# zichunhao/lgn-autoencoder

Hardware: AMD Instinct MI355X
Metric: jets/sec fwd+bwd, 30-particle maxdim=2 bs=512 (higher is better)
Workload: dtype f64

## Files before the change

include/lgn_amd.h:

```cpp
#ifndef LGN_AMD_H
#define LGN_AMD_H

#include <stddef.h>
#include <stdint.h>

#ifdef __cplusplus
extern "C" {
#endif

#define LGN_AMD_ABI_VERSION 18

int lgn_abi_version(void);
const char* lgn_last_error(void);

int lgn_level_fwd_f64(int B, int N, int C, int CO, int decoder,
                      const double* s_in, const double* v_in, const double* p, const uint8_t* mask,
                      const double* ra, const double* rb, const double* rc,
                      const double* w0, const double* b0, const double* w1, const double* b1,
                      const double* wm0, const double* wm1,
                      double* ag0, double* ag1, double* s_out, double* v_out, void* stream);

int lgn_level_bwd_partial_rows(int B, int N, int decoder, int* rows_mix, int* rows_rad);
int lgn_level_rad_partial_len(int C, int decoder);
int lgn_level_jet_split(int B, int N);

int lgn_level_bwd_f64(int B, int N, int C, int CO, int decoder,
                      const double* s_in, const double* v_in, const double* p, const uint8_t* mask,
                      const double* ra, const double* rb, const double* rc,
                      const double* w0, const double* b0, const double* w1, const double* b1,
                      const double* wm0, const double* wm1, const double* ag0, const double* ag1,
                      const double* g_s_out, const double* g_v_out,
                      double* g_ag, double* g_s_in, double* g_v_in, double* g_p,
                      double* part_mix, double* part_rad, void* stream);

int lgn_cg_product_fwd_f64(int R, int N, int C, int D1, int D2, int DO, int mode, int nnz, const int* row_ptr, const int* col,
                           const double* coef, const double* x1, const double* x2, double* out, void* stream);
int lgn_cg_product_bwd_f64(int R, int N, int C, int D1, int D2, int DO, int mode, int nnz, const int* row_ptr, const int* col,
                           const double* coef, const double* x1, const double* x2, const double* g_out, double* g_x1, double* g_x2,
                           void* stream);

int lgn_reduce_partials_f64(const double* part, int rows, int n, double* out, int accumulate, void* stream);

int lgn_radial_finalize_f64(const double* tot, int C, const double* ra, const double* rb, const double* rc,
                            const double* w0, const double* w1,
                            double* g_a, double* g_b, double* g_c,
                            double* g_w0, double* g_b0, double* g_w1, double* g_b1, void* stream);

#define LGN_ACT_LEAKYRELU 0
#define LGN_ACT_RELU 1
#define LGN_ACT_ELU 2
#define LGN_ACT_SIGMOID 3
#define LGN_ACT_LOGSIGMOID 4
#define LGN_ACT_ATAN 5
#define LGN_ACT_COUNT 6
int lgn_cgmlp_fwd_f64(int M, int C, int H, int nlin, int activation, const double* const* w, const double* const* b,
                      const double* s_in, double* s_out, void* stream);
int lgn_cgmlp_partial_rows(int M, int H);
int lgn_cgmlp_bwd_f64(int M, int C, int H, int nlin, int activation, const double* const* w, const double* const* b,
                      const double* s_in, const double* g_out, double* g_in, double* part, int psize, void* stream);

int lgn_mixreps_fwd_f64(int rows, int Cin, int Cout, int d, const double* w, const double* x, double* y, void* stream);
int lgn_mixreps_partial_rows(int rows);
int lgn_mixreps_bwd_f64(int rows, int Cin, int Cout, int d, const double* w, const double* x, const double* g_y,
                        double* g_x, double* part, void* stream);

int lgn_moments_fwd_f64(int B, int N, int C, int Q, int decoder, const double* X, const double* p, const uint8_t* mask,
                        const double* ra, const double* rb, const double* rc, const double* w0, const double* b0,
                        const double* w1, const double* b1, double* U, void* stream);
long long lgn_moments_scratch_doubles(int B, int N, int C, int decoder);
int lgn_moments_bwd_f64(int B, int N, int C, int Q, int decoder, const double* X, const double* p, const uint8_t* mask,
                        const double* ra, const double* rb, const double* rc, const double* w0, const double* b0,
                        const double* w1, const double* b1, const double* gU, double* gX, double* g_p,
                        double* part_rad, double* scratch, void* stream);

typedef struct lgn_local_tables {
  int n_rows, n_out, n_w;
  int n_terms, n_u, n_x;
  int n_units, static_kind;
  const int *row_ptr, *t_type, *t_a, *t_b;
  const double* t_coef;
  const int *out_dim, *out_nblk, *out_row0, *out_q0, *out_w0;
  const int *u_ptr, *u_row;
  const double* u_coef;
  const int *x_ptr, *x_row, *x_other;
  const double* x_coef;
  int h_out_w0[8];
} lgn_local_tables;

int lgn_local_fwd_f64(int nodes, int C, int CO, int Q, int Qout, const lgn_local_tables* t, const double* X, const double* U,
                      const double* wcat, double* out, void* stream);
int lgn_local_partial_rows(int nodes);
int lgn_local_bwd_f64(int nodes, int C, int CO, int Q, int Qout, const lgn_local_tables* t, const double* X, const double* U,
                      const double* wcat, const double* g_out, double* gU, double* gX, double* part, void* stream);

long long lgn_local_static_packed_doubles(int kind, int C, int CO);
int lgn_local_bwd_static_f64(int kind, int nodes, int C, int CO, const double* XT, const double* UT, const double* wcat,
                             const int* w0, double* wpacked, const double* goT, double* gUT, double* gXT, double* part,
                             double* gpacked, double* g_wcat, void* stream);
int lgn_local_fwd_static_f64(int kind, int nodes, int C, int CO, const double* XT, const double* UT, const double* wcat,
                             const int* w0, double* wpacked, double* outT, double* s_copy, int q_s, void* stream);

typedef struct lgn_net_desc {
  int B, N;
  int n_levels;
  int enc_channels[5];
  int dec_channels[5];
  int tau_s, tau_v;
  int mlp_hidden_mul;
  int mlp_nlin;
  int tau_v_in;
  const lgn_local_tables* enc_tables[4];
  const lgn_local_tables* dec_tables[4];
  int enc_Q[5], enc_qs[5], enc_qv[5];
  int dec_Q[5], dec_qs[5], dec_qv[5];
  int flags;
  int activation;
  int n_in_scalars;
  int latent_pool;
  int dec_N;
  int get_real;
  double jet_loss_scale;
} lgn_net_desc;
#define LGN_REAL_SUM 0
#define LGN_REAL_REAL 1
#define LGN_REAL_IMAG 2
#define LGN_REAL_MEAN 3
#define LGN_REAL_NORM 4
#define LGN_POOL_MIN 0
#define LGN_POOL_MAX 1
#define LGN_POOL_MEAN 2
#define LGN_POOL_MIX 3
#define LGN_POOL(n, avg, o0, o1, o2, o3) ((n) | ((avg) << 3) | ((o0) << 4) | ((o1) << 6) | ((o2) << 8) | ((o3) << 10))
#define LGN_NET_NO_STATIC 1
#define LGN_NET_DEC_PAIRWISE 2
#define LGN_NET_LEVEL_V2 4
#define LGN_NET_MLP_V1 8
#define LGN_NET_MOMENTS_V1 16
#define LGN_NET_BWD_ORDERED 64
#define LGN_NET_DEC_UNFUSED 256
#define LGN_NET_MOMENTS_SPLIT 512
#define LGN_NET_MLP_BWD1 1024
#define LGN_NET_SPLIT_TAIL 128

#define LGN_LDS_LIMIT (160 * 1024)
long long lgn_encoder_end_lds_bytes(int N, int C0, int K, int CL, int Ts, int Tv, int pool);
long long lgn_decoder_end_lds_bytes(int N, int C0, int Tin, int CL);
long long lgn_junction_lds_bytes(int N, int CL, int Ts, int Tv, int pool, int C0);

int lgn_step_param_slots(const lgn_net_desc* d, int decoder);
long long lgn_step_workspace_doubles(const lgn_net_desc* d);
int lgn_step_fwd_bwd_f64(const lgn_net_desc* d, const double* params, double* grads, long long n_params,
                         const int64_t* enc_off, const int64_t* dec_off, const double* p4, const double* target,
                         const uint8_t* mask, const double* in_scalars, double* workspace, long long workspace_doubles,
                         double* recon, double* loss_part, void* stream);
#define LGN_FINALIZE_SCRATCH 2048
int lgn_step_finalize_f64(double* params, double* grads, long long n_params, const double* loss_part, int n_loss,
                          double l1_lambda, double* adam_m, double* adam_v, long long* step_dev,
                          double lr, double beta1, double beta2, double eps, int do_adam, double* loss_out, void* stream);
int lgn_step_train_f64(const lgn_net_desc* d, double* params, double* grads, long long n_params, const int64_t* enc_off,
                       const int64_t* dec_off, const double* p4, const double* target, const uint8_t* mask, const double* in_scalars,
                       double* workspace, long long workspace_doubles, double* recon, double* loss_part, int n_loss, double l1_lambda,
                       double* adam_m, double* adam_v, long long* step_dev, double lr, double beta1, double beta2, double eps,
                       int do_adam, double* loss_out, void* stream);

long long lgn_eval_workspace_doubles(const lgn_net_desc* d);
int lgn_step_eval_f64(const lgn_net_desc* d, const double* params, const int64_t* enc_off, const int64_t* dec_off,
                      const double* p4_scaled, const double* p4_target, const uint8_t* mask, const double* in_scalars,
                      double* workspace, long long workspace_doubles, double* recon_real, double* lat_s ,
                      double* lat_v , double* loss_part, double* loss_out, void* stream);

long long lgn_net_workspace_doubles(const lgn_net_desc* d, int decoder, int which);
int lgn_encoder_fwd_f64(const lgn_net_desc* d, const double* params, const int64_t* off, const double* p4, const uint8_t* mask,
                        const double* in_scalars, double* act, long long act_doubles, double* lat_s, double* lat_v, void* stream);
int lgn_encoder_bwd_f64(const lgn_net_desc* d, const double* params, double* grads, long long n_params, const int64_t* off,
                        const double* p4, const uint8_t* mask, const double* in_scalars, const double* act, long long act_doubles,
                        const double* g_lat_s, const double* g_lat_v, double* scratch, long long scratch_doubles, void* stream);
int lgn_decoder_fwd_f64(const lgn_net_desc* d, const double* params, const int64_t* off, const double* lat_v, double* act,
                        long long act_doubles, double* recon, void* stream);
int lgn_decoder_bwd_f64(const lgn_net_desc* d, const double* params, double* grads, long long n_params, const int64_t* off,
                        const double* lat_v, const double* act, long long act_doubles, const double* g_recon, double* g_lat_v,
                        double* scratch, long long scratch_doubles, void* stream);

int lgn_chamfer_f64(int B, int N, int M, const double* x, const double* y, int jet_features, double* loss_part, double* gx, double* gy,
                    void* stream);

#define LGN_ANOMALY_NMAX 192
#define LGN_ANOMALY_NSCORES 21
#define LGN_ANOMALY_ALL 0x1FFFFF
#define LGN_ANOMALY_HUNGARIAN 0x403E0
#define LGN_ANOMALY_NO_HUNGARIAN (LGN_ANOMALY_ALL & ~LGN_ANOMALY_HUNGARIAN)
int lgn_anomaly_scores_f64(const double* recons, const double* target, const double* recons_n, const double* target_n, int B, int N,
                           int score_mask, double* scores, int* col4row , int* status, void* stream);

int lgn_linear_sum_assignment_f64(const double* cost, int B, int n, int* col4row, int* status, void* stream);

#ifdef __cplusplus
}
#endif
#endif
```

lgn-autoencoder_amd/csrc/api_common.cpp:

```cpp
#include <stdarg.h>
#include <stdlib.h>

#include "level.hpp"
#include "../../include/lgn_amd.h"

namespace lgn {
static thread_local char g_err[512] = "";
void set_error(const char* fmt, ...) {
  va_list ap;
  va_start(ap, fmt);
  vsnprintf(g_err, sizeof(g_err), fmt, ap);
  va_end(ap);
}
int level_flags_from_env() {
  auto on = [](const char* name) { const char* e = getenv(name); return e && e[0] == '1'; };
  return (on("LGN_AMD_DEC_PAIRWISE") ? LVL_DEC_PAIRWISE : 0) | (on("LGN_AMD_LEVEL_V2") ? LVL_LEVEL_V2 : 0) |
         (on("LGN_AMD_MOMENTS_V1") ? LVL_MOMENTS_V1 : 0) | (on("LGN_AMD_MLP_V1") ? LVL_MLP_V1 : 0) | (on("LGN_AMD_BWD_ORDERED") ? LVL_BWD_ORDERED : 0) |
         (on("LGN_AMD_MOMENTS_SPLIT") ? LVL_MOMENTS_SPLIT : 0) | (on("LGN_AMD_MLP_BWD1") ? LVL_MLP_BWD1 : 0);
}
static_assert(LVL_DEC_PAIRWISE == LGN_NET_DEC_PAIRWISE && LVL_LEVEL_V2 == LGN_NET_LEVEL_V2 && LVL_MOMENTS_V1 == LGN_NET_MOMENTS_V1 &&
                  LVL_MLP_V1 == LGN_NET_MLP_V1 && LVL_MLP_BWD1 == LGN_NET_MLP_BWD1 &&
                  LVL_BWD_ORDERED == LGN_NET_BWD_ORDERED && LVL_MOMENTS_SPLIT == LGN_NET_MOMENTS_SPLIT, "LVL_* and LGN_NET_* are the same bits");
}

extern "C" {
const char* lgn_last_error(void) { return lgn::g_err; }
int lgn_abi_version(void) { return LGN_AMD_ABI_VERSION; }
}
```

lgn-autoencoder_amd/csrc/level.hpp:

```cpp
#pragma once
#include "common.hpp"

namespace lgn {

constexpr int LVL_DEC_PAIRWISE = 2;
constexpr int LVL_LEVEL_V2 = 4;
constexpr int LVL_MLP_V1 = 8;
constexpr int LVL_MOMENTS_V1 = 16;
constexpr int LVL_MLP_BWD1 = 1024;
constexpr int LVL_MOMENTS_SPLIT = 512;
constexpr int LVL_BWD_ORDERED = 64;
int level_flags_from_env();

template <typename T>
struct LevelArgs {
  int B, N, C, CO;
  const T* s_in;
  const T* v_in;
  const T* p;
  const uint8_t* mask;
  const T *ra, *rb, *rc, *w0, *b0, *w1, *b1;
  const T *wm0, *wm1;
  T* ag0;
  T* ag1;
  T* s_out;
  T* v_out;
  const T* in_w0 = nullptr;
  const T* in_w1 = nullptr;
  T* in_s = nullptr;
  T* in_v = nullptr;
  T* z1 = nullptr;
  size_t z1n = 0;
  T* z2 = nullptr;
  size_t z2n = 0;
  const T* loss_wo1 = nullptr;
  const T* loss_target = nullptr;
  T loss_scale = T(1);
  int loss_real = 0;
  T loss_jscale = T(0);
  T* loss_recon = nullptr;
  T* loss_part = nullptr;
  T* loss_gv = nullptr;
  T* loss_wpart = nullptr;
  int flags = 0;
};

template <typename T>
struct LevelBwdArgs {
  int B, N, C, CO;
  const T *s_in, *v_in, *p;
  const uint8_t* mask;
  const T *ra, *rb, *rc, *w0, *b0, *w1, *b1;
  const T *wm0, *wm1;
  const T *ag0, *ag1;
  const T* g_s_out;
  const T* g_v_out;
  T* g_ag;
  T* g_s_in;
  T* g_v_in;
  T* g_p;
  T* part_mix;
  T* part_rad;
  T* part_in0 = nullptr;
  int flags = 0;
};

__host__ __device__ constexpr int node_stride(int C) { return 10 * C + 4; }

__host__ __device__ constexpr int rad_partial_size(int C, bool dec) {
  return dec ? 2 * C : (2 * 4 * C * NB + 8 * C);
}

inline int level_jet_split(int B, int N) {
  const int groups = (N + 3) / 4;
  int s = 1;
  while (s * 2 <= groups && B * s * 2 <= 512) s *= 2;
  return s;
}

}
```

lgn-autoencoder_amd/csrc/level_fwd2.hip:

```cpp
#include "level_dev.hpp"
#include "net_dev.hpp"
#include "ops.hpp"
#include "wave_sum.hpp"

namespace lgn {

typedef double v4d __attribute__((ext_vector_type(4)));
LGN_STAMP_DECL
LGN_STAMP_READER(lgn_debug_stamps_fwd2)

__device__ __forceinline__ double dpp_quad(double v, int ctrl_is_xor2) {
  int lo = __double2loint(v), hi = __double2hiint(v);
  if (ctrl_is_xor2) {
    lo = __builtin_amdgcn_mov_dpp(lo, 0x4E, 0xF, 0xF, true);
    hi = __builtin_amdgcn_mov_dpp(hi, 0x4E, 0xF, 0xF, true);
  } else {
    lo = __builtin_amdgcn_mov_dpp(lo, 0xB1, 0xF, 0xF, true);
    hi = __builtin_amdgcn_mov_dpp(hi, 0xB1, 0xF, 0xF, true);
  }
  return __hiloint2double(hi, lo);
}
__device__ __forceinline__ double quad_sum(double v) {
  v += dpp_quad(v, 0);
  v += dpp_quad(v, 1);
  return v;
}

__device__ __forceinline__ double fast_rcp(double u) {
  double r = __builtin_amdgcn_rcp(u);
  double e = __builtin_fma(-u, r, 1.0);
  r = __builtin_fma(r, e, r);
  e = __builtin_fma(-u, r, 1.0);
  return __builtin_fma(r, e, r);
}

template <int C, bool DEC>
struct Fwd2 {
  static constexpr int NG = (C + 3) / 4;
  static constexpr int NS = node_stride(C);
  static constexpr int PS = DEC ? 8 : 4;
  static constexpr int AGS = 20 * C;
  static constexpr int A3 = 0, A4 = 2 * C, A1 = 4 * C, A2 = 12 * C;
};

template <int C, bool DEC, bool SEP, bool TRAIN>
__global__ __launch_bounds__(2 * BLOCK) void level_fwd2_kernel(LevelArgs<double> a, int chunk) {
  using F = Fwd2<C, DEC>;
  constexpr int NG = F::NG;
  const int N = a.N, B = a.B, CO = a.CO;
  const int b = blockIdx.x, tid = threadIdx.x, lane = tid & 63, wave = tid >> 6;
  const int nthr = blockDim.x, nw = nthr >> 6;

  extern __shared__ __align__(16) unsigned char smem_raw[];
  double* nd = reinterpret_cast<double*>(smem_raw);
  double* pj = nd + ((N * F::NS + 1) & ~1);
  double* wm = pj + N * F::PS;
  double* agl = wm + 4 * CO * 5 * C;
  double* sums = agl + chunk * F::AGS;
  uint8_t* mk = reinterpret_cast<uint8_t*>(sums + 20 * C);

  STAMP(0);
  if (!DEC && a.in_w0) {
    {
      const size_t wg = (size_t)blockIdx.y * gridDim.x + blockIdx.x, stride = (size_t)gridDim.x * gridDim.y * nthr;
      for (size_t e = wg * nthr + tid; e < a.z1n; e += stride) a.z1[e] = 0.0;
      for (size_t e = wg * nthr + tid; e < a.z2n; e += stride) a.z2[e] = 0.0;
    }
    const double* p0 = a.p + (size_t)b * N * 4;
    const size_t plane_s = (size_t)B * N * C;
    const int nw2 = 2 * CO * 5 * C;
    for (int e = tid; e < N * 4; e += nthr) pj[e] = p0[e];
    for (int e = tid; e < N; e += nthr) mk[e] = a.mask[(size_t)b * N + e];
    for (int e = tid; e < nw2; e += nthr) {
      wm[e] = a.wm0[e];
      wm[nw2 + e] = a.wm1[e];
    }
    for (int e = tid; e < N * C; e += nthr) {
      const int j = e / C, c = e - j * C;
      const double* p = p0 + j * 4;
      const double pe = p[0], px = p[1], py = p[2], pz = p[3];
      const double q0 = pe * pe, q1 = px * px, q2 = py * py, q3 = pz * pz;
      const double mass = sqrt(fabs(2.0 * q0 - (((q0 + q1) + q2) + q3)));
      constexpr double H = 0.70710678118654752440084436210484903928;
      const cx<double> q[4] = {{pe, 0.0}, {px * H, -py * H}, {pz, 0.0}, {-px * H, -py * H}};
      const double w0r = a.in_w0[c], w0i = a.in_w0[C + c];
      const cx<double> w1 = {a.in_w1[c], a.in_w1[C + c]};
      double* d = nd + j * F::NS + c * 10;
      d[0] = w0r * mass;
      d[1] = w0i * mass;
#pragma unroll
      for (int m = 0; m < 4; ++m) {
        const cx<double> r = cmul(w1, q[m]);
        d[2 + m] = r.r;
        d[6 + m] = r.i;
      }
      if (blockIdx.y == 0) {
        const size_t ge = (size_t)b * N * C + e;
        a.in_s[ge] = d[0];
        a.in_s[plane_s + ge] = d[1];
#pragma unroll
        for (int m = 0; m < 4; ++m) {
          a.in_v[ge * 4 + m] = d[2 + m];
          a.in_v[plane_s * 4 + ge * 4 + m] = d[6 + m];
        }
      }
    }
  } else {
    JetRegs<double> jr;
    load_jet_issue<double, C, DEC>(a.s_in, a.v_in, a.p, a.mask, B, N, b, jr);
    const int nw2 = 2 * CO * 5 * C, ew = tid < nw2 ? tid : 0;
    const double w0v = a.wm0[ew], w1v = a.wm1[ew];
    load_jet_commit<double, C, DEC>(a.s_in, a.v_in, a.p, a.mask, B, N, b, jr, nd, pj, mk);
    if (tid < nw2) {
      wm[tid] = w0v;
      wm[nw2 + tid] = w1v;
    }
    for (int e = tid + nthr; e < nw2; e += nthr) {
      wm[e] = a.wm0[e];
      wm[nw2 + e] = a.wm1[e];
    }
  }

  const int pr = lane & 15, cg = lane >> 4;
  const int ti = pr >> 2, tj = pr & 3;
  double ak[5], bk[5], ck2[5];
  double wf[NG][5];
  double bias[NG][4];
  if (!DEC) {
#pragma unroll
    for (int s = 0; s < 5; ++s) {
      const int k = 4 * s + cg;
      ak[s] = a.ra[k];
      bk[s] = a.rb[k];
      const double c = a.rc[k];
      ck2[s] = c * c;
    }
#pragma unroll
    for (int g = 0; g < NG; ++g) {
      const int rr = lane & 15, q = rr >> 2, ch = 4 * g + (rr & 3);
      const double* w = (q >> 1) ? a.w1 : a.w0;
#pragma unroll
      for (int s = 0; s < 5; ++s) wf[g][s] = ch < C ? w[(2 * ch + (q & 1)) * NB + 4 * s + cg] : 0.0;
    }
  }
#pragma unroll
  for (int g = 0; g < NG; ++g) {
    const int ch = 4 * g + cg;
#pragma unroll
    for (int q = 0; q < 4; ++q) {
      const double* bb = (q >> 1) ? a.b1 : a.b0;
      bias[g][q] = ch < C ? (DEC ? bb[ch] : bb[2 * ch + (q & 1)]) : 0.0;
    }
  }
  __syncthreads();
  STAMP(1);

  if constexpr (DEC && SEP) {
    if (tid < 64) {
      const int k = tid & 7, part = tid >> 3;
      double mean = 0.0;
      for (int n = part; n < N; n += 8) mean += pj[n * 8 + k];
      mean += shfl_xor(mean, 8);
      mean += shfl_xor(mean, 16);
      mean += shfl_xor(mean, 32);
      if (part == 0) sums[k] = mean / N;
    }
    __syncthreads();
    for (int e = tid; e < N * 8; e += nthr) pj[e] -= sums[e & 7];
    __syncthreads();
#define LGN_PUT(k, val)                                           \
  do {                                                            \
    if ((k) < 12) a0[(k) < 12 ? (k) : 0] += (val);                \
    else a1[(k) >= 12 ? (k) - 12 : 0] += (val);                   \
  } while (0)
    for (int c = wave; c < C; c += nw) {
      double a0[12], a1[8];
#pragma unroll
      for (int k = 0; k < 12; ++k) a0[k] = 0.0;
#pragma unroll
      for (int k = 0; k < 8; ++k) a1[k] = 0.0;
      for (int n = lane; n < N; n += 64) {
        const double* ni = nd + n * F::NS + c * 10;
        const double* pn = pj + n * 8;
        const cx<double> sn = {ni[0], ni[1]};
        cx<double> v[4], pc[4];
#pragma unroll
        for (int m = 0; m < 4; ++m) {
          v[m] = {ni[2 + m], ni[6 + m]};
          pc[m] = {pn[m], pn[4 + m]};
        }
        LGN_PUT(0, sn.r);  LGN_PUT(1, sn.i);
#pragma unroll
        for (int m = 0; m < 4; ++m) {
          LGN_PUT(2 + 2 * m, v[m].r);  LGN_PUT(3 + 2 * m, v[m].i);
          const cx<double> sp = cmul(sn, pc[m]);
          LGN_PUT(10 + 2 * m, sp.r);  LGN_PUT(11 + 2 * m, sp.i);
        }
        const cx<double> vp = bil2(v, pc);
        LGN_PUT(18, vp.r);  LGN_PUT(19, vp.i);
      }
      wave_sum_store<12>(a0, sums + c * 20, lane);
      wave_sum_store<8>(a1, sums + c * 20 + 12, lane);
    }
#undef LGN_PUT
    __syncthreads();
  }

  const int ngroups = (N + 3) >> 2, gper = (ngroups + (int)gridDim.y - 1) / (int)gridDim.y;
  const int rlo = min(N, 4 * (int)blockIdx.y * gper), rhi = min(N, rlo + 4 * gper);
  auto catmix = [&](int c0, int c1) {
    constexpr int K = 5 * C;
    const int nr = c1 - c0;
    const size_t plo = (size_t)B * N * CO;
    if (wave == 0) {
      for (int rl = lane; rl < nr; rl += 64) {
// ... 147 lines not shown
#pragma unroll
          for (int s = 0; s < 5; ++s) beta[s] = __builtin_fma(bk[s], rho5[s], ak[s]);
        }
#pragma unroll
        for (int g = 0; g < NG; ++g) {
          T.R[g] = v4d{bias[g][0], bias[g][1], bias[g][2], bias[g][3]};
#pragma unroll
          for (int s = 0; s < 5; ++s) T.R[g] = __builtin_amdgcn_mfma_f64_16x16x4f64(wf[g][s], beta[s], T.R[g], 0, 0, 0);
        }
      }
    };
    auto agg = [&](const Tile& T) {
      if (T.ok) {
        const double* nj = nd + T.jj * F::NS;
#pragma unroll
        for (int g = 0; g < NG; ++g) {
          const int ch = 4 * g + cg;
          if (ch < C) {
            const cx<double> R0 = {T.R[g][0], T.R[g][1]}, R1 = {T.R[g][2], T.R[g][3]};
            const cx<double> e0 = {R0.r - R0.i, R0.r + R0.i};
            const cx<double> sj = {nj[ch * 10], nj[ch * 10 + 1]};
            cx<double> vj[4];
#pragma unroll
            for (int m = 0; m < 4; ++m) {
              vj[m] = {nj[ch * 10 + 2 + m], nj[ch * 10 + 6 + m]};
              cfma(A1[g][m], vj[m], e0);
            }
            cfma(A4[g], sj, e0);
            if (!DEC) {
              const double qd0 = T.qd0, qd3 = T.qd3, qa = T.qa, qb = T.qb;
              const cx<double> Tm = cmul(sj, R1);
              A2[g][0].r = __builtin_fma(Tm.r, qd0, A2[g][0].r);  A2[g][0].i = __builtin_fma(Tm.i, qd0, A2[g][0].i);
              A2[g][2].r = __builtin_fma(Tm.r, qd3, A2[g][2].r);  A2[g][2].i = __builtin_fma(Tm.i, qd3, A2[g][2].i);
              const double aTr = qa * Tm.r, aTi = qa * Tm.i, bTr = qb * Tm.r, bTi = qb * Tm.i;
              A2[g][1].r += aTr + bTi;  A2[g][1].i += aTi - bTr;
              A2[g][3].r += bTi - aTr;  A2[g][3].i -= aTi + bTr;
              const cx<double> dv = {vj[3].r - vj[1].r, vj[3].i - vj[1].i}, sv = {vj[1].r + vj[3].r, vj[1].i + vj[3].i};
              cx<double> V;
              V.r = __builtin_fma(vj[0].r, qd0, __builtin_fma(-vj[2].r, qd3, __builtin_fma(qa, dv.r, qb * sv.i)));
              V.i = __builtin_fma(vj[0].i, qd0, __builtin_fma(-vj[2].i, qd3, __builtin_fma(qa, dv.i, -qb * sv.r)));
              cfma(A3[g], R1, V);
            } else {
              cx<double> e1[4];
#pragma unroll
              for (int m = 0; m < 4; ++m) {
                e1[m] = cmul(R1, T.q[m]);
                cfma(A2[g][m], sj, e1[m]);
              }
              const cx<double> t = bil2(vj, e1);
              A3[g].r += t.r;
              A3[g].i += t.i;
            }
          }
        }
      }
    };
    if (jlo < jhi) {
      Tile ta, tb;
      prep(jlo, ta);
      int j0 = jlo;
      while (true) {
        if (j0 + 4 < jhi) prep(j0 + 4, tb);
        agg(ta);
        j0 += 4;
        if (j0 >= jhi) break;
        if (j0 + 4 < jhi) prep(j0 + 4, ta);
        agg(tb);
        j0 += 4;
        if (j0 >= jhi) break;
      }
    }

    STAMP(3 + ((rg >> 2) & 3) * 4);
#pragma unroll
    for (int g = 0; g < NG; ++g) {
      A3[g].r = quad_sum(A3[g].r) * 0.5;  A3[g].i = quad_sum(A3[g].i) * 0.5;
      A4[g].r = quad_sum(A4[g].r);        A4[g].i = quad_sum(A4[g].i);
#pragma unroll
      for (int m = 0; m < 4; ++m) {
        A1[g][m].r = quad_sum(A1[g][m].r);  A1[g][m].i = quad_sum(A1[g][m].i);
        A2[g][m].r = quad_sum(A2[g][m].r);  A2[g][m].i = quad_sum(A2[g][m].i);
      }
    }
    if (tj == 0) {
      double* st = agl + (slab + i0 + ti - c0) * F::AGS;
#pragma unroll
      for (int g = 0; g < NG; ++g) {
        const int ch = 4 * g + cg;
        if (ch < C) {
          st[F::A3 + 2 * ch] = A3[g].r;  st[F::A3 + 2 * ch + 1] = A3[g].i;
          st[F::A4 + 2 * ch] = A4[g].r;  st[F::A4 + 2 * ch + 1] = A4[g].i;
#pragma unroll
          for (int m = 0; m < 4; ++m) {
            st[F::A1 + (ch * 4 + m) * 2] = A1[g][m].r;  st[F::A1 + (ch * 4 + m) * 2 + 1] = A1[g][m].i;
            st[F::A2 + (ch * 4 + m) * 2] = A2[g][m].r;  st[F::A2 + (ch * 4 + m) * 2 + 1] = A2[g][m].i;
          }
        }
      }
    }
    STAMP(4 + ((rg >> 2) & 3) * 4);
  };
  if (rs > 1) {
    const int rg = (c0 >> 2) + wave / rs;
    if (rg * 4 < c1) row_group(rg, 4 * (rpart * ntl / rs), min(N, 4 * ((rpart + 1) * ntl / rs)), rpart * 4 * ngr);
  } else {
    for (int rg = (c0 >> 2) + wave; rg * 4 < c1; rg += nw) row_group(rg, 0, N, 0);
  }
  if (rs > 1) {
    __syncthreads();
    const int tot = 4 * ngr * F::AGS;
    for (int e = tid; e < tot; e += nthr) {
      double v = agl[e];
      for (int pp = 1; pp < rs; ++pp) v += agl[pp * tot + e];
      agl[e] = v;
    }
  }
  }
  __syncthreads();
  STAMP(20);

  if constexpr (TRAIN) {
    const size_t pl0 = (size_t)B * N * 2 * C;
    for (int e = tid; e < (c1 - c0) * 2 * C; e += nthr) {
      const int n = e / (2 * C), r = e - n * 2 * C, blk = r / C, ch = r - blk * C;
      const double* st = agl + n * F::AGS + (blk ? F::A4 : F::A3) + 2 * ch;
      const size_t ge = ((size_t)b * N + c0) * 2 * C + e;
      a.ag0[ge] = st[0];
      a.ag0[pl0 + ge] = st[1];
    }
    for (int e = tid; e < (c1 - c0) * 2 * C * 4; e += nthr) {
      const int n = e / (8 * C), r = e - n * 8 * C, blk = r / (4 * C), cm = r - blk * 4 * C;
      const double* st = agl + n * F::AGS + (blk ? F::A2 : F::A1) + 2 * cm;
      const size_t ge = ((size_t)b * N + c0) * 8 * C + e;
      a.ag1[ge] = st[0];
      a.ag1[pl0 * 4 + ge] = st[1];
    }
  }
  STAMP(21);

  catmix(c0, c1);
  STAMP(22);
  if (c1 < rhi) __syncthreads();
  }
  STAMP(40);
  if constexpr (DEC) {
    if (a.loss_wo1) {
      __syncthreads();
      dec_output_loss_body<TRAIN>(B, N, CO, a.v_out, a.loss_wo1, a.loss_target, a.loss_scale, a.loss_real, a.loss_jscale,
                                  a.loss_recon, a.loss_part, a.loss_gv, a.loss_wpart, smem_raw);
    }
  }
}

template <int C, bool DEC, bool SEP, bool TRAIN>
static int launch_level_fwd2(const LevelArgs<double>& a, hipStream_t stream) {
  using F = Fwd2<C, DEC>;
  const size_t fixed = sizeof(double) * (((size_t)a.N * F::NS + 1 & ~size_t(1)) + (size_t)a.N * F::PS + 4 * a.CO * 5 * C + 20 * C) + a.N + 16;
  const bool wide = a.B <= 320 && a.N >= 64;
  const size_t row = sizeof(double) * F::AGS, budget1 = 160 * 1024, budget2 = wide ? budget1 : 78 * 1024;
  const int full = (a.N + 15) & ~15;
  int chunk = full;
  if (fixed + full * row > budget2) {
    const size_t room = fixed + 16 * row <= budget2 ? budget2 - fixed : (fixed < budget1 ? budget1 - fixed : 0);
    chunk = (int)(room / row) & ~15;
    if (chunk > full) chunk = full;
    if (chunk < 16) chunk = 16;
  }
  size_t smem = fixed + chunk * row;
  if (a.loss_wo1) {
    LGN_CHECK_ARG(DEC && SEP && a.N <= 40 && !wide && a.loss_target && a.loss_recon && a.loss_part && (!TRAIN || (a.loss_gv && a.loss_wpart)),
                  "level_fwd: the loss rides on the separable decoder forward of jets of <= 40 particles only");
    if (smem < dec_out_loss_bytes(a.N, a.CO)) smem = dec_out_loss_bytes(a.N, a.CO);
  }
  LGN_CHECK_ARG(smem <= 160 * 1024, "level_fwd: N=%d C=%d needs %zu B of LDS (> 160 KiB)", a.N, a.C, smem);
  auto kern = level_fwd2_kernel<C, DEC, SEP, TRAIN>;
  if (smem > 64 * 1024) {
    hipError_t e = hipFuncSetAttribute(reinterpret_cast<const void*>(kern), hipFuncAttributeMaxDynamicSharedMemorySize, (int)smem);
    if (e != hipSuccess) { set_error("hipFuncSetAttribute: %s", hipGetErrorString(e)); return (int)e; }
  }
  const int nthreads = wide ? 2 * BLOCK : BLOCK;
  const int split = (SEP || a.N > 40) ? 1 : level_jet_split(a.B, a.N);
  hipLaunchKernelGGL(kern, dim3(a.B, split), dim3(nthreads), smem, stream, a, chunk);
  LGN_CHECK_LAUNCH();
  return 0;
}

bool level_fwd_carries_loss(int N, int flags) { return N <= 40 && !(flags & LVL_DEC_PAIRWISE); }

template <bool TRAIN>
static int level_fwd_run(const LevelArgs<double>& a, int decoder, hipStream_t stream) {
  LGN_CHECK_ARG(a.B > 0 && a.N > 0, "level_fwd: empty batch (B=%d N=%d)", a.B, a.N);
  LGN_CHECK_ARG(!a.in_w0 || (!decoder && a.in_w1 && a.in_s && a.in_v), "level_fwd: the input stage rides on encoder levels only");
  LGN_CHECK_ARG(a.CO >= 1 && a.CO <= 8, "level_fwd: C_out=%d unsupported (1..8)", a.CO);
  const bool pairwise = (a.flags & LVL_DEC_PAIRWISE) != 0;
#define LGN_CASE(CC)                                                                                         \
  case CC:                                                                                                   \
    if (!decoder) return launch_level_fwd2<CC, false, false, TRAIN>(a, stream);                              \
    return pairwise ? launch_level_fwd2<CC, true, false, TRAIN>(a, stream) : launch_level_fwd2<CC, true, true, TRAIN>(a, stream);
  switch (a.C) {
#ifdef LGN_DEV_ONLY_C4
    LGN_CASE(4)
#else
    LGN_CASE(1) LGN_CASE(2) LGN_CASE(3) LGN_CASE(4) LGN_CASE(5) LGN_CASE(6) LGN_CASE(7) LGN_CASE(8)
#endif
    default:
      set_error("level_fwd: C_in=%d unsupported (1..8)", a.C);
      return -1;
  }
#undef LGN_CASE
}

template <>
int level_fwd_dispatch<double>(const LevelArgs<double>& a, int decoder, hipStream_t stream) {
  return level_fwd_run<true>(a, decoder, stream);
}

int level_fwd_eval(const LevelArgs<double>& a, int decoder, hipStream_t stream) { return level_fwd_run<false>(a, decoder, stream); }

}
```

lgn-autoencoder_amd/csrc/net_kernels.hip:

```cpp
#include "net.hpp"
#include "net_dev.hpp"
#include "tail_dev.hpp"

namespace lgn {

LGN_STAMP_DECL
LGN_STAMP_READER(lgn_debug_stamps_net)

namespace {
constexpr double H = 0.70710678118654752440084436210484903928;

__device__ __forceinline__ double minkowski_sq_ref(const double* p) {
  double q0 = p[0] * p[0], q1 = p[1] * p[1], q2 = p[2] * p[2], q3 = p[3] * p[3];
  return 2.0 * q0 - (((q0 + q1) + q2) + q3);
}
__device__ __forceinline__ void canon_real(const double* p, cx<double> (&q)[4]) {
  q[0] = {p[0], 0.0};
  q[1] = {p[1] * H, -p[2] * H};
  q[2] = {p[3], 0.0};
  q[3] = {-p[1] * H, -p[2] * H};
}
__device__ __forceinline__ void canon_cplx(const cx<double> (&p)[4], cx<double> (&c)[4]) {
  c[0] = p[0];
  c[1] = {(p[1].r + p[2].i) * H, (p[1].i - p[2].r) * H};
  c[2] = p[3];
  c[3] = {(-p[1].r + p[2].i) * H, (-p[1].i - p[2].r) * H};
}
__device__ __forceinline__ void canon_cplx_bwd(const cx<double> (&g)[4], cx<double> (&gp)[4]) {
  gp[0] = g[0];
  gp[1] = {(g[1].r - g[3].r) * H, (g[1].i - g[3].i) * H};
  gp[2] = {-(g[1].i + g[3].i) * H, (g[1].r + g[3].r) * H};
  gp[3] = g[2];
}
__device__ __forceinline__ void cart_from_canon(const cx<double> (&c)[4], cx<double> (&p)[4]) {
  p[0] = c[0];
  p[1] = {(c[1].r - c[3].r) * H, (c[1].i - c[3].i) * H};
  p[2] = {-(c[1].i + c[3].i) * H, (c[1].r + c[3].r) * H};
  p[3] = c[2];
}
}

__global__ void enc_input_fwd_kernel(int B, int N, int C, int K, const double* __restrict__ p4, const double* __restrict__ xs,
                                     const double* __restrict__ w0, const double* __restrict__ w1, double* s, double* v, double* z1,
                                     size_t n1, double* z2, size_t n2) {
  const size_t total = (size_t)B * N * C, pl = total;
  for (size_t e = (size_t)blockIdx.x * blockDim.x + threadIdx.x; e < n1; e += (size_t)gridDim.x * blockDim.x) z1[e] = 0.0;
  for (size_t e = (size_t)blockIdx.x * blockDim.x + threadIdx.x; e < n2; e += (size_t)gridDim.x * blockDim.x) z2[e] = 0.0;
  for (size_t e = (size_t)blockIdx.x * blockDim.x + threadIdx.x; e < total; e += (size_t)gridDim.x * blockDim.x) {
    const int c = e % C;
    const size_t node = e / C;
    const double* p = p4 + node * 4;
    const double mass = sqrt(fabs(minkowski_sq_ref(p)));
    cx<double> q[4];
    canon_real(p, q);
    double sr = w0[c * K] * mass, si = w0[(C + c) * K] * mass;
    for (int k = 1; k < K; ++k) {
      const double x = xs[node * (K - 1) + (k - 1)];
      sr = __builtin_fma(w0[c * K + k], x, sr);
      si = __builtin_fma(w0[(C + c) * K + k], x, si);
    }
    s[e] = sr;
    s[pl + e] = si;
    const cx<double> w = {w1[c], w1[C + c]};
#pragma unroll
    for (int m = 0; m < 4; ++m) {
      cx<double> r = cmul(w, q[m]);
      v[e * 4 + m] = r.r;
      v[pl * 4 + e * 4 + m] = r.i;
    }
  }
}

__global__ __launch_bounds__(BLOCK) void enc_input_bwd_kernel(int B, int N, int C, int K, const double* __restrict__ p4,
                                                             const double* __restrict__ xs, const double* __restrict__ g_s,
                                                             const double* __restrict__ g_v, double* part) {
  extern __shared__ __align__(16) unsigned char smem_raw[];
  double* tmp = reinterpret_cast<double*>(smem_raw);
  const int T = 2 * K + 2;
  const int b = blockIdx.x;
  const size_t pl = (size_t)B * N * C;
  for (int i = threadIdx.x; i < N * C; i += BLOCK) {
    const int n = i / C;
    const double* p = p4 + ((size_t)b * N + n) * 4;
    const double mass = sqrt(fabs(minkowski_sq_ref(p)));
    cx<double> q[4];
    canon_real(p, q);
    const size_t e = (size_t)b * N * C + i;
    cx<double> d1 = {0, 0};
#pragma unroll
    for (int m = 0; m < 4; ++m) cfmac(d1, cx<double>{g_v[e * 4 + m], g_v[pl * 4 + e * 4 + m]}, q[m]);
    const double gr = g_s[e], gi = g_s[pl + e];
    tmp[i * T + 0] = gr * mass;
    tmp[i * T + K] = gi * mass;
    for (int k = 1; k < K; ++k) {
      const double x = xs[((size_t)b * N + n) * (K - 1) + (k - 1)];
      tmp[i * T + k] = gr * x;
      tmp[i * T + K + k] = gi * x;
    }
    tmp[i * T + 2 * K] = d1.r;
    tmp[i * T + 2 * K + 1] = d1.i;
  }
  __syncthreads();
  for (int o = threadIdx.x; o < T * C; o += BLOCK) {
    int c, t;
    if (o < 2 * C * K) {
      const int z = o / (C * K), r = o - z * C * K;
      c = r / K;
      t = z * K + (r - c * K);
    } else {
      const int r = o - 2 * C * K, z = r / C;
      c = r - z * C;
      t = 2 * K + z;
    }
    double acc = 0.0;
    for (int n = 0; n < N; ++n) acc += tmp[(n * C + c) * T + t];
    part[(size_t)b * T * C + o] = acc;
  }
}

__device__ __forceinline__ cx<double> canon_cplx_m(const double* p, int m) {
  if (m == 0) return {p[0], p[4]};
  if (m == 2) return {p[3], p[7]};
  const double sg = m == 1 ? 1.0 : -1.0;
  return {(sg * p[1] + p[6]) * H, (sg * p[5] - p[2]) * H};
}
__device__ __forceinline__ cx<double> canon_cplx_bwd_m(const double* g, int m) {
  if (m == 0) return {g[0], g[4]};
  if (m == 3) return {g[2], g[6]};
  if (m == 1) return {(g[1] - g[3]) * H, (g[5] - g[7]) * H};
  return {-(g[5] + g[7]) * H, (g[1] + g[3]) * H};
}

__host__ __device__ inline size_t lat_y_doubles(int N, int Ts, int Tv, int pool = 0) {
  return (size_t)(pool_is_mix(pool) ? 1 : N) * (2 * Ts + 8 * Tv);
}
__host__ __device__ inline size_t lat_fwd_doubles(int N, int C, int Ts, int Tv, int pool = 0) {
  return lat_y_doubles(N, Ts, Tv, pool) + (size_t)N * C * 10 + 2 * (size_t)(Ts + Tv) * pool_mix_in(pool, N, C);
}
struct LatentStage {
  StageRegs<2> sr, si;
  StageRegs<4> vr, vi;
  StageRegs<1> w0, w1;
  const double *s0, *s1, *v0, *v1, *wl0, *wl1;
  int N, C, Ts, Tv, K, NY, NS;
  __device__ __forceinline__ void issue(int B, int N_, int C_, int Ts_, int Tv_, const double* __restrict__ s, const double* __restrict__ v,
                                        const double* __restrict__ wl0_, const double* __restrict__ wl1_, int pool = 0) {
    N = N_; C = C_; Ts = Ts_; Tv = Tv_; wl0 = wl0_; wl1 = wl1_; K = pool_mix_in(pool, N_, C_); NY = (int)lat_y_doubles(N_, Ts_, Tv_, pool);
    const size_t pl = (size_t)B * N * C, j0 = (size_t)blockIdx.x * N * C;
    NS = s ? N * C : 0;
    s0 = s ? s + j0 : nullptr; s1 = s ? s + pl + j0 : nullptr; v0 = v + j0 * 4; v1 = v + (pl + j0) * 4;
    vr.issue(v0, N * C * 4); vi.issue(v1, N * C * 4);
    sr.issue(s0, NS); si.issue(s1, NS);
    w0.issue(wl0, 2 * Ts * K); w1.issue(wl1, 2 * Tv * K);
  }
  __device__ __forceinline__ void commit(double* lds, bool zero_y) const {
    double* sv = lds + NY;
    double* w0l = sv + N * C * 10;
    double* w1l = w0l + 2 * Ts * K;
    if (zero_y)
      for (int e = threadIdx.x; e < NY; e += BLOCK) lds[e] = 0.0;
    vr.commit(v0, N * C * 4, [&](int e, double x) { sv[(e >> 2) * 10 + 2 + (e & 3)] = x; });
    vi.commit(v1, N * C * 4, [&](int e, double x) { sv[(e >> 2) * 10 + 6 + (e & 3)] = x; });
    if (NS) {
      sr.commit(s0, NS, [&](int e, double x) { sv[e * 10] = x; });
      si.commit(s1, NS, [&](int e, double x) { sv[e * 10 + 1] = x; });
    } else {
      for (int e = threadIdx.x; e < N * C; e += BLOCK) sv[e * 10] = sv[e * 10 + 1] = 0.0;
    }
    w0.commit(wl0, 2 * Ts * K, [&](int e, double x) { w0l[e] = x; });
    w1.commit(wl1, 2 * Tv * K, [&](int e, double x) { w1l[e] = x; });
  }
};
template <bool TO_LDS>
__device__ __forceinline__ void enc_latent_fwd_body(int B, int N, int C, int Ts, int Tv, int pool, double* lat_s, double* lat_v, int* idx,
                                                    double* lds, double* lat_l) {
  const int b = blockIdx.x, TT = Ts + Tv;
  const int P = pool_blocks(pool), PN = pool_n(pool);
  bool need_mean = false;
  for (int i = 0; i < PN; ++i) need_mean |= pool_op(pool, i) == LGN_POOL_MEAN;
  const int YS = 2 * Ts + 8 * Tv;
  double* y = lds;
  const double* sv = y + N * YS;
  const double* w0l = sv + N * C * 10;
  const double* w1l = w0l + 2 * Ts * C;
  STAMP(1);
  for (int e = threadIdx.x; e < N * Tv; e += BLOCK) {
    const int n = e / Tv, tv = e - n * Tv;
    const double* x = sv + n * C * 10;
    cx<double> acc[4] = {{0, 0}, {0, 0}, {0, 0}, {0, 0}}, pc[4];
#pragma unroll 4
    for (int c = 0; c < C; ++c) {
      const cx<double> w = {w1l[tv * C + c], w1l[Tv * C + tv * C + c]};
#pragma unroll
      for (int m = 0; m < 4; ++m) cfma(acc[m], w, cx<double>{x[c * 10 + 2 + m], x[c * 10 + 6 + m]});
    }
    cart_from_canon(acc, pc);
    double* o = y + n * YS + 2 * Ts + 8 * tv;
#pragma unroll
    for (int m = 0; m < 4; ++m) { o[m] = pc[m].r; o[4 + m] = pc[m].i; }
  }
  for (int e = threadIdx.x; e < N * Ts; e += BLOCK) {
    const int n = e / Ts, t = e - n * Ts;
    const double* x = sv + n * C * 10;
    cx<double> acc = {0, 0};
#pragma unroll 4
    for (int c = 0; c < C; ++c) cfma(acc, cx<double>{w0l[t * C + c], w0l[Ts * C + t * C + c]}, cx<double>{x[c * 10], x[c * 10 + 1]});
    y[n * YS + 2 * t] = acc.r;
    y[n * YS + 2 * t + 1] = acc.i;
  }
  __syncthreads();
  STAMP(2);
  const int l8 = threadIdx.x & 7;
  constexpr int NONE = 0x7fffffff;
  for (int it = threadIdx.x >> 3; it < 2 * TT; it += BLOCK / 8) {
    const int z = it / TT, t = it - z * TT;
    int imin = NONE, imax = NONE;
    double smin = 0, smax = 0;
#pragma unroll 4
    for (int n = l8; n < N; n += 8) {
      double lo, hi;
      if (t < Ts) {
        const double val = y[n * YS + 2 * t + z];
        lo = val;
        hi = val * val;
      } else {
        const double* o = y + n * YS + 2 * Ts + 8 * (t - Ts) + 4 * z;
        lo = hi = o[0] * o[0] - ((o[1] * o[1] + o[2] * o[2]) + o[3] * o[3]);
      }
      if (imin == NONE || lo < smin) { smin = lo; imin = n; }
      if (imax == NONE || hi > smax) { smax = hi; imax = n; }
    }
#pragma unroll
    for (int off = 4; off; off >>= 1) {
      const double om = __shfl_xor(smin, off, 8), oM = __shfl_xor(smax, off, 8);
      const int oi = __shfl_xor(imin, off, 8), oI = __shfl_xor(imax, off, 8);
      if (oi != NONE && (imin == NONE || om < smin || (om == smin && oi < imin))) { smin = om; imin = oi; }
      if (oI != NONE && (imax == NONE || oM > smax || (oM == smax && oI < imax))) { smax = oM; imax = oI; }
    }
    imin = __shfl(imin, 0, 8);
    imax = __shfl(imax, 0, 8);
    if (l8 < 2) idx[(((size_t)b * 2 + z) * TT + t) * 2 + l8] = l8 ? imax : imin;
    const int nc = t < Ts ? 1 : 4, y0 = t < Ts ? 2 * t + z : 2 * Ts + 8 * (t - Ts) + 4 * z;
    double mean[4] = {0, 0, 0, 0};
    if (need_mean) {
      for (int n = l8; n < N; n += 8)
#pragma unroll
        for (int m = 0; m < 4; ++m)
          if (m < nc) mean[m] += y[n * YS + y0 + m];
#pragma unroll
      for (int off = 4; off; off >>= 1)
#pragma unroll
        for (int m = 0; m < 4; ++m) mean[m] += __shfl_xor(mean[m], off, 8);
#pragma unroll
      for (int m = 0; m < 4; ++m) mean[m] /= (double)N;
    }
    for (int k = l8; k < P * nc; k += 8) {
      const int pb = k / nc, m = k - pb * nc;
      auto pick = [&](int op) -> double {
        if (op == LGN_POOL_MIN) return y[imin * YS + y0 + m];
        if (op == LGN_POOL_MAX) return y[imax * YS + y0 + m];
        return m == 0 ? mean[0] : (m == 1 ? mean[1] : (m == 2 ? mean[2] : mean[3]));
      };
      double val;
      if (pool_avg(pool)) {
        val = pick(pool_op(pool, 0));
        for (int i = 1; i < PN; ++i) val += pick(pool_op(pool, i));
        val /= (double)PN;
      } else {
        val = pick(pool_op(pool, pb));
      }
      if (t < Ts) {
        lat_s[((size_t)z * B + b) * P * Ts + pb * Ts + t] = val;
      } else {
        const int tv = t - Ts;
        lat_v[(((size_t)z * B + b) * P * Tv + pb * Tv + tv) * 4 + m] = val;
        if constexpr (TO_LDS) lat_l[(pb * Tv + tv) * 8 + 4 * z + m] = val;
      }
    }
  }
}
template <bool TO_LDS>
__device__ __forceinline__ void enc_latent_mix_fwd_body(int B, int N, int C, int Ts, int Tv, double* lat_s, double* lat_v, double* lds,
                                                        double* lat_l) {
  const int b = blockIdx.x, TT = Ts + Tv, K = N * C;
  const double* sv = lds + (2 * Ts + 8 * Tv);
  const double* w0l = sv + K * 10;
  const double* w1l = w0l + 2 * Ts * K;
  const int l8 = threadIdx.x & 7;
  for (int t = threadIdx.x >> 3; t < TT; t += BLOCK / 8) {
    if (t < Ts) {
      cx<double> acc = {0, 0};
      for (int k = l8; k < K; k += 8) cfma(acc, cx<double>{w0l[t * K + k], w0l[Ts * K + t * K + k]}, cx<double>{sv[k * 10], sv[k * 10 + 1]});
#pragma unroll
      for (int off = 4; off; off >>= 1) { acc.r += __shfl_xor(acc.r, off, 8); acc.i += __shfl_xor(acc.i, off, 8); }
      if (l8 < 2) lat_s[((size_t)l8 * B + b) * Ts + t] = l8 ? acc.i : acc.r;
    } else {
      const int tv = t - Ts;
      cx<double> acc[4] = {{0, 0}, {0, 0}, {0, 0}, {0, 0}}, pc[4];
      for (int k = l8; k < K; k += 8) {
        const cx<double> w = {w1l[tv * K + k], w1l[Tv * K + tv * K + k]};
#pragma unroll
        for (int m = 0; m < 4; ++m) cfma(acc[m], w, cx<double>{sv[k * 10 + 2 + m], sv[k * 10 + 6 + m]});
      }
#pragma unroll
      for (int off = 4; off; off >>= 1)
#pragma unroll
        for (int m = 0; m < 4; ++m) { acc[m].r += __shfl_xor(acc[m].r, off, 8); acc[m].i += __shfl_xor(acc[m].i, off, 8); }
      cart_from_canon(acc, pc);
      const int z = l8 >> 2, m = l8 & 3;
      const cx<double> pm = m == 0 ? pc[0] : (m == 1 ? pc[1] : (m == 2 ? pc[2] : pc[3]));
      const double val = z ? pm.i : pm.r;
      lat_v[(((size_t)z * B + b) * Tv + tv) * 4 + m] = val;
      if constexpr (TO_LDS) lat_l[tv * 8 + 4 * z + m] = val;
    }
  }
}
__global__ __launch_bounds__(BLOCK) void enc_latent_fwd_kernel(int B, int N, int C, int Ts, int Tv, int pool,
                                                              const double* __restrict__ s, const double* __restrict__ v,
                                                              const double* __restrict__ wl0, const double* __restrict__ wl1,
                                                              double* lat_s, double* lat_v, int* idx) {
  extern __shared__ __align__(16) unsigned char smem_raw[];
  double* lds = reinterpret_cast<double*>(smem_raw);
  LatentStage st;
  st.issue(B, N, C, Ts, Tv, s, v, wl0, wl1, pool);
  st.commit(lds, false);
  __syncthreads();
  if (pool_is_mix(pool)) enc_latent_mix_fwd_body<false>(B, N, C, Ts, Tv, lat_s, lat_v, lds, nullptr);
  else enc_latent_fwd_body<false>(B, N, C, Ts, Tv, pool, lat_s, lat_v, idx, lds, nullptr);
}

constexpr int LAT_PARTS = 6;
__host__ __device__ inline size_t lat_bwd_doubles(int N, int C, int Ts, int Tv, int pool = 0) {
  return lat_fwd_doubles(N, C, Ts, Tv, pool) + (pool_is_mix(pool) ? 0 : (size_t)LAT_PARTS * (Ts + Tv) * C * 2);
}
struct LatentBwdPrefetch {
  int n[2];
  double gs[4];
  bool valid;
  __device__ __forceinline__ void issue(int B, int Ts, int Tv, int pool, const int* __restrict__ idx, const double* __restrict__ g_lat_s) {
    const int TT = Ts + Tv, e = threadIdx.x, b = blockIdx.x, P = pool_blocks(pool);
    valid = 2 * TT <= BLOCK && !pool_is_mix(pool);
    if (valid && e < 2 * TT) {
      const int z = e / TT, t = e - z * TT;
#pragma unroll
      for (int kind = 0; kind < 2; ++kind) n[kind] = idx[(((size_t)b * 2 + z) * TT + t) * 2 + kind];
#pragma unroll
      for (int pb = 0; pb < 4; ++pb) gs[pb] = (t < Ts && pb < P) ? g_lat_s[((size_t)z * B + b) * P * Ts + pb * Ts + t] : 0.0;
    }
  }
};
template <bool FROM_LDS>
__device__ __forceinline__ void enc_latent_bwd_body(int B, int N, int C, int Ts, int Tv, int pool, const double* __restrict__ g_lat_s,
                                                    const double* __restrict__ g_lat_v, const double* g_lat_l,
                                                    const int* __restrict__ idx, double* g_s, double* g_v, double* part, double* lds,
                                                    const LatentBwdPrefetch& pre) {
  const int b = blockIdx.x, TT = Ts + Tv;
  const int YS = 2 * Ts + 8 * Tv;
  double* gy = lds;
  const double* sv = gy + N * YS;
  const double* w0l = sv + N * C * 10;
  const double* w1l = w0l + 2 * Ts * C;
  double* red = const_cast<double*>(w1l) + 2 * Tv * C;
  const size_t pl = (size_t)B * N * C;
  STAMP(14);
  const int P = pool_blocks(pool), PN = pool_n(pool);
  for (int e = threadIdx.x; e < 2 * TT; e += BLOCK) {
    const int z = e / TT, t = e - z * TT;
    int nmm[2];
#pragma unroll
    for (int kind = 0; kind < 2; ++kind) nmm[kind] = pre.valid ? pre.n[kind] : idx[(((size_t)b * 2 + z) * TT + t) * 2 + kind];
    const int nc = t < Ts ? 1 : 4, y0 = t < Ts ? 2 * t + z : 2 * Ts + 8 * (t - Ts) + 4 * z;
    const int nscat = pool_avg(pool) ? PN : P;
    for (int i = 0; i < nscat; ++i) {
      const int pb = pool_avg(pool) ? 0 : i, op = pool_op(pool, i);
      double g[4] = {0, 0, 0, 0};
      if (t < Ts) {
        g[0] = pre.valid ? (pb == 0 ? pre.gs[0] : (pb == 1 ? pre.gs[1] : (pb == 2 ? pre.gs[2] : pre.gs[3])))
                         : g_lat_s[((size_t)z * B + b) * P * Ts + pb * Ts + t];
      } else {
        const int tv = t - Ts;
#pragma unroll
        for (int m = 0; m < 4; ++m) {
          if constexpr (FROM_LDS) g[m] = g_lat_l[(pb * Tv + tv) * 8 + 4 * z + m];
          else g[m] = g_lat_v[(((size_t)z * B + b) * P * Tv + pb * Tv + tv) * 4 + m];
        }
      }
      if (pool_avg(pool))
#pragma unroll
        for (int m = 0; m < 4; ++m) g[m] /= (double)PN;
      if (op == LGN_POOL_MEAN) {
#pragma unroll
        for (int m = 0; m < 4; ++m) g[m] /= (double)N;
        for (int n = 0; n < N; ++n)
#pragma unroll
          for (int m = 0; m < 4; ++m)
            if (m < nc) gy[n * YS + y0 + m] += g[m];
      } else {
        const int n = nmm[op == LGN_POOL_MAX];
#pragma unroll
        for (int m = 0; m < 4; ++m)
          if (m < nc) gy[n * YS + y0 + m] += g[m];
      }
    }
  }
  __syncthreads();
  STAMP(15);
  for (int e = threadIdx.x; e < N * Tv; e += BLOCK) {
    const int n = e / Tv, tv = e - n * Tv;
    double* o = gy + n * YS + 2 * Ts + 8 * tv;
    cx<double> g[4], gc[4];
    for (int m = 0; m < 4; ++m) g[m] = {o[m], o[4 + m]};
    cart_from_canon_bwd(g, gc);
    for (int m = 0; m < 4; ++m) { o[m] = gc[m].r; o[4 + m] = gc[m].i; }
  }
  __syncthreads();
  STAMP(16);
  for (int e = threadIdx.x; e < N * C; e += BLOCK) {
    const int n = e / C, c = e - n * C;
    const size_t base = ((size_t)b * N + n) * C + c;
    cx<double> as = {0, 0}, av[4] = {{0, 0}, {0, 0}, {0, 0}, {0, 0}};
#pragma unroll 2
    for (int t = 0; t < Ts; ++t)
      cfmac(as, cx<double>{gy[n * YS + 2 * t], gy[n * YS + 2 * t + 1]}, cx<double>{w0l[t * C + c], w0l[Ts * C + t * C + c]});
#pragma unroll 4
    for (int t = 0; t < Tv; ++t) {
      const cx<double> w = {w1l[t * C + c], w1l[Tv * C + t * C + c]};
      const double* o = gy + n * YS + 2 * Ts + 8 * t;
#pragma unroll
      for (int m = 0; m < 4; ++m) cfmac(av[m], cx<double>{o[m], o[4 + m]}, w);
    }
    g_s[base] = as.r;
    g_s[pl + base] = as.i;
#pragma unroll
    for (int m = 0; m < 4; ++m) { g_v[base * 4 + m] = av[m].r; g_v[pl * 4 + base * 4 + m] = av[m].i; }
  }
  STAMP(17);
  const int nper = (N + LAT_PARTS - 1) / LAT_PARTS;
  for (int e = threadIdx.x; e < LAT_PARTS * TT * C; e += BLOCK) {
    const int pi = e / (TT * C), r = e - pi * TT * C, t = r / C, c = r - t * C;
    const int n1 = min(N, (pi + 1) * nper);
    cx<double> acc = {0, 0};
    if (t < Ts) {
#pragma unroll 5
      for (int n = pi * nper; n < n1; ++n)
        cfmac(acc, cx<double>{gy[n * YS + 2 * t], gy[n * YS + 2 * t + 1]}, cx<double>{sv[(n * C + c) * 10], sv[(n * C + c) * 10 + 1]});
    } else {
      const int tv = t - Ts;
#pragma unroll 5
      for (int n = pi * nper; n < n1; ++n) {
        const double* o = gy + n * YS + 2 * Ts + 8 * tv;
        const double* x = sv + (n * C + c) * 10;
#pragma unroll
        for (int m = 0; m < 4; ++m) cfmac(acc, cx<double>{o[m], o[4 + m]}, cx<double>{x[2 + m], x[6 + m]});
      }
    }
    red[e * 2] = acc.r;
    red[e * 2 + 1] = acc.i;
  }
  __syncthreads();
  STAMP(18);
  double* row = part + (size_t)b * 2 * TT * C;
  for (int e = threadIdx.x; e < TT * C; e += BLOCK) {
    const int t = e / C, c = e - t * C;
    double ar = red[e * 2], ai = red[e * 2 + 1];
    for (int pi = 1; pi < LAT_PARTS; ++pi) { ar += red[(pi * TT * C + e) * 2]; ai += red[(pi * TT * C + e) * 2 + 1]; }
    if (t < Ts) {
      row[t * C + c] = ar;
      row[Ts * C + t * C + c] = ai;
    } else {
      row[2 * Ts * C + (t - Ts) * C + c] = ar;
      row[2 * Ts * C + Tv * C + (t - Ts) * C + c] = ai;
    }
  }
}
template <bool FROM_LDS>
__device__ __forceinline__ void enc_latent_mix_bwd_body(int B, int N, int C, int Ts, int Tv, const double* __restrict__ g_lat_s,
                                                        const double* __restrict__ g_lat_v, const double* g_lat_l, double* g_s, double* g_v,
                                                        double* part, double* lds) {
  const int b = blockIdx.x, TT = Ts + Tv, K = N * C;
  double* gy = lds;
  const double* sv = lds + (2 * Ts + 8 * Tv);
  const double* w0l = sv + K * 10;
  const double* w1l = w0l + 2 * Ts * K;
  const size_t pl = (size_t)B * K;
  for (int t = threadIdx.x; t < TT; t += BLOCK) {
    if (t < Ts) {
      gy[2 * t] = g_lat_s ? g_lat_s[((size_t)0 * B + b) * Ts + t] : 0.0;
      gy[2 * t + 1] = g_lat_s ? g_lat_s[((size_t)1 * B + b) * Ts + t] : 0.0;
    } else {
      const int tv = t - Ts;
      cx<double> g[4], gc[4];
      for (int m = 0; m < 4; ++m) {
        if constexpr (FROM_LDS) g[m] = {g_lat_l[tv * 8 + m], g_lat_l[tv * 8 + 4 + m]};
        else g[m] = {g_lat_v[(((size_t)0 * B + b) * Tv + tv) * 4 + m], g_lat_v[(((size_t)1 * B + b) * Tv + tv) * 4 + m]};
      }
      cart_from_canon_bwd(g, gc);
      double* o = gy + 2 * Ts + 8 * tv;
      for (int m = 0; m < 4; ++m) { o[m] = gc[m].r; o[4 + m] = gc[m].i; }
    }
  }
  __syncthreads();
  for (int k = threadIdx.x; k < K; k += BLOCK) {
    cx<double> as = {0, 0}, av[4] = {{0, 0}, {0, 0}, {0, 0}, {0, 0}};
    for (int t = 0; t < Ts; ++t) cfmac(as, cx<double>{gy[2 * t], gy[2 * t + 1]}, cx<double>{w0l[t * K + k], w0l[Ts * K + t * K + k]});
    for (int t = 0; t < Tv; ++t) {
      const cx<double> w = {w1l[t * K + k], w1l[Tv * K + t * K + k]};
      const double* o = gy + 2 * Ts + 8 * t;
#pragma unroll
      for (int m = 0; m < 4; ++m) cfmac(av[m], cx<double>{o[m], o[4 + m]}, w);
    }
    const size_t base = (size_t)b * K + k;
    g_s[base] = as.r;
    g_s[pl + base] = as.i;
#pragma unroll
    for (int m = 0; m < 4; ++m) { g_v[base * 4 + m] = av[m].r; g_v[pl * 4 + base * 4 + m] = av[m].i; }
  }
  double* row = part + (size_t)b * 2 * TT * K;
  for (int e = threadIdx.x; e < TT * K; e += BLOCK) {
    const int t = e / K, k = e - t * K;
    cx<double> acc = {0, 0};
    if (t < Ts) {
      cfmac(acc, cx<double>{gy[2 * t], gy[2 * t + 1]}, cx<double>{sv[k * 10], sv[k * 10 + 1]});
      row[t * K + k] = acc.r;
      row[Ts * K + t * K + k] = acc.i;
    } else {
      const int tv = t - Ts;
      const double* o = gy + 2 * Ts + 8 * tv;
#pragma unroll
      for (int m = 0; m < 4; ++m) cfmac(acc, cx<double>{o[m], o[4 + m]}, cx<double>{sv[k * 10 + 2 + m], sv[k * 10 + 6 + m]});
      row[2 * Ts * K + tv * K + k] = acc.r;
      row[2 * Ts * K + Tv * K + tv * K + k] = acc.i;
    }
  }
}
__global__ __launch_bounds__(BLOCK) void enc_latent_bwd_kernel(int B, int N, int C, int Ts, int Tv, int pool,
                                                              const double* __restrict__ s, const double* __restrict__ v,
                                                              const double* __restrict__ wl0, const double* __restrict__ wl1,
                                                              const double* __restrict__ g_lat_s, const double* __restrict__ g_lat_v,
                                                              const int* __restrict__ idx, double* g_s, double* g_v, double* part) {
  extern __shared__ __align__(16) unsigned char smem_raw[];
  double* lds = reinterpret_cast<double*>(smem_raw);
  LatentStage st;
  LatentBwdPrefetch pre;
  st.issue(B, N, C, Ts, Tv, s, v, wl0, wl1, pool);
  pre.issue(B, Ts, Tv, pool, idx, g_lat_s);
  st.commit(lds, true);
  __syncthreads();
  if (pool_is_mix(pool)) enc_latent_mix_bwd_body<false>(B, N, C, Ts, Tv, g_lat_s, g_lat_v, nullptr, g_s, g_v, part, lds);
  else enc_latent_bwd_body<false>(B, N, C, Ts, Tv, pool, g_lat_s, g_lat_v, nullptr, idx, g_s, g_v, part, lds, pre);
}

__host__ __device__ inline size_t dec_in_fwd_doubles(int N, int C, int Tin) {
  return 2 * (size_t)N * Tin + (size_t)Tin * 8 + (size_t)N * 8 + 4 * (size_t)C;
}
struct DecInFwdStage {
  StageRegs<4> wg;
  StageRegs<1> a0, a1, lr, li;
  const double *wg1, *w0, *w1, *l0, *l1;
  int N, C, Tin;
  bool with_lat;
  __device__ __forceinline__ void issue(int B, int N_, int C_, int Tin_, const double* __restrict__ lat_v, const double* __restrict__ wg1_,
                                        const double* __restrict__ w0_, const double* __restrict__ w1_, bool with_lat_) {
    N = N_; C = C_; Tin = Tin_; wg1 = wg1_; w0 = w0_; w1 = w1_; with_lat = with_lat_;
    wg.issue(wg1, 2 * N * Tin);
    a0.issue(w0, 2 * C); a1.issue(w1, 2 * C);
    if (with_lat) {
      l0 = lat_v + (size_t)blockIdx.x * Tin * 4; l1 = lat_v + ((size_t)B + blockIdx.x) * Tin * 4;
      lr.issue(l0, Tin * 4); li.issue(l1, Tin * 4);
    }
  }
  __device__ __forceinline__ void commit(double* lds) const {
    double* wgl = lds;
    double* latl = wgl + 2 * N * Tin;
    double* w01 = latl + Tin * 8 + N * 8;
    wg.commit(wg1, 2 * N * Tin, [&](int e, double x) { wgl[e] = x; });
    a0.commit(w0, 2 * C, [&](int e, double x) { w01[e] = x; });
    a1.commit(w1, 2 * C, [&](int e, double x) { w01[2 * C + e] = x; });
    if (with_lat) {
      lr.commit(l0, Tin * 4, [&](int e, double x) { latl[(e >> 2) * 8 + (e & 3)] = x; });
      li.commit(l1, Tin * 4, [&](int e, double x) { latl[(e >> 2) * 8 + 4 + (e & 3)] = x; });
    }
  }
};
__device__ __forceinline__ void dec_input_fwd_body(int B, int N, int C, int Tin, double* pdec, double* s0, double* v0, double* lds) {
  const double* wgl = lds;
  const double* latl = wgl + 2 * N * Tin;
  double* cartl = const_cast<double*>(latl) + Tin * 8;
  const double* w01 = cartl + N * 8;
  const int b = blockIdx.x;
  const size_t plp = (size_t)B * N * 4, pl = (size_t)B * N * C;
  STAMP(3);
  for (int e = threadIdx.x; e < N * 4; e += BLOCK) {
    const int n = e >> 2, m = e & 3;
    cx<double> acc = {0, 0};
#pragma unroll 8
    for (int t = 0; t < Tin; ++t)
      cfma(acc, cx<double>{wgl[n * Tin + t], wgl[N * Tin + n * Tin + t]}, cx<double>{latl[t * 8 + m], latl[t * 8 + 4 + m]});
    cartl[n * 8 + m] = acc.r;
    cartl[n * 8 + 4 + m] = acc.i;
  }
  __syncthreads();
  STAMP(4);
  for (int e = threadIdx.x; e < N * 4; e += BLOCK) {
    const cx<double> pc = canon_cplx_m(cartl + (e >> 2) * 8, e & 3);
    pdec[(size_t)b * N * 4 + e] = pc.r;
    pdec[plp + (size_t)b * N * 4 + e] = pc.i;
  }
  for (int e = threadIdx.x; e < N * C; e += BLOCK) {
    const int c = e % C;
    s0[(size_t)b * N * C + e] = w01[c] - w01[C + c];
    s0[pl + (size_t)b * N * C + e] = w01[C + c] + w01[c];
  }
  for (int e = threadIdx.x; e < N * C * 4; e += BLOCK) {
    const int i = e >> 2, m = e & 3, n = i / C, c = i - n * C;
    const cx<double> r = cmul(cx<double>{w01[2 * C + c], w01[3 * C + c]}, canon_cplx_m(cartl + n * 8, m));
    v0[(size_t)b * N * C * 4 + e] = r.r;
    v0[pl * 4 + (size_t)b * N * C * 4 + e] = r.i;
  }
}
__global__ __launch_bounds__(BLOCK) void dec_input_fwd_kernel(int B, int N, int C, int Tin, const double* __restrict__ lat_v,
                                                             const double* __restrict__ wg1, const double* __restrict__ w0,
                                                             const double* __restrict__ w1, double* pdec, double* s0, double* v0) {
  extern __shared__ __align__(16) unsigned char smem_raw[];
  double* lds = reinterpret_cast<double*>(smem_raw);
  DecInFwdStage st;
  st.issue(B, N, C, Tin, lat_v, wg1, w0, w1, true);
  st.commit(lds);
  __syncthreads();
  dec_input_fwd_body(B, N, C, Tin, pdec, s0, v0, lds);
}

__host__ __device__ inline size_t dec_in_bwd_doubles(int N, int C, int Tin) {
  return (size_t)N * 16 + 2 * (size_t)N * Tin + (size_t)Tin * 8 + (size_t)N * 16 + (size_t)N * C * 10 + 2 * (size_t)C;
}
struct DecInBwdStage {
  StageRegs<4> gvr, gvi, wg;
  StageRegs<1> gpr, gpi, pdr, pdi, gsr, gsi, lr, li, a1;
  const double *gv0, *gv1, *wg1, *gp0, *gp1, *pd0, *pd1, *gs0, *gs1, *l0, *l1, *w1;
  int N, C, Tin;
  __device__ __forceinline__ void issue(int B, int N_, int C_, int Tin_, const double* __restrict__ lat_v, const double* __restrict__ wg1_,
                                        const double* __restrict__ w1_, const double* __restrict__ pdec, const double* __restrict__ g_p,
                                        const double* __restrict__ g_s0, const double* __restrict__ g_v0) {
    N = N_; C = C_; Tin = Tin_; wg1 = wg1_; w1 = w1_;
    const int b = blockIdx.x;
    const size_t plp = (size_t)B * N * 4, pl = (size_t)B * N * C, j4 = (size_t)b * N * 4, jc = (size_t)b * N * C;
    gv0 = g_v0 + jc * 4; gv1 = g_v0 + (pl + jc) * 4; gp0 = g_p + j4; gp1 = g_p + plp + j4; pd0 = pdec + j4; pd1 = pdec + plp + j4;
    gs0 = g_s0 + jc; gs1 = g_s0 + pl + jc; l0 = lat_v + (size_t)b * Tin * 4; l1 = lat_v + ((size_t)B + b) * Tin * 4;
    gvr.issue(gv0, N * C * 4); gvi.issue(gv1, N * C * 4); wg.issue(wg1, 2 * N * Tin);
    gpr.issue(gp0, N * 4); gpi.issue(gp1, N * 4); pdr.issue(pd0, N * 4); pdi.issue(pd1, N * 4);
    gsr.issue(gs0, N * C); gsi.issue(gs1, N * C); lr.issue(l0, Tin * 4); li.issue(l1, Tin * 4); a1.issue(w1, 2 * C);
  }
  __device__ __forceinline__ void commit(double* lds) const {
    double* wgl = lds + N * 16;
    double* latl = wgl + 2 * N * Tin;
    double* gp_l = latl + Tin * 8;
    double* pd_l = gp_l + N * 8;
    double* gs_l = pd_l + N * 8;
    double* gv_l = gs_l + N * C * 2;
    double* w1l = gv_l + N * C * 8;
    gvr.commit(gv0, N * C * 4, [&](int e, double x) { gv_l[(e >> 2) * 8 + (e & 3)] = x; });
    gvi.commit(gv1, N * C * 4, [&](int e, double x) { gv_l[(e >> 2) * 8 + 4 + (e & 3)] = x; });
    wg.commit(wg1, 2 * N * Tin, [&](int e, double x) { wgl[e] = x; });
    gpr.commit(gp0, N * 4, [&](int e, double x) { gp_l[(e >> 2) * 8 + (e & 3)] = x; });
    gpi.commit(gp1, N * 4, [&](int e, double x) { gp_l[(e >> 2) * 8 + 4 + (e & 3)] = x; });
    pdr.commit(pd0, N * 4, [&](int e, double x) { pd_l[(e >> 2) * 8 + (e & 3)] = x; });
    pdi.commit(pd1, N * 4, [&](int e, double x) { pd_l[(e >> 2) * 8 + 4 + (e & 3)] = x; });
    gsr.commit(gs0, N * C, [&](int e, double x) { gs_l[e * 2] = x; });
    gsi.commit(gs1, N * C, [&](int e, double x) { gs_l[e * 2 + 1] = x; });
    lr.commit(l0, Tin * 4, [&](int e, double x) { latl[(e >> 2) * 8 + (e & 3)] = x; });
    li.commit(l1, Tin * 4, [&](int e, double x) { latl[(e >> 2) * 8 + 4 + (e & 3)] = x; });
    a1.commit(w1, 2 * C, [&](int e, double x) { w1l[e] = x; });
  }
};
template <bool TO_LDS>
__device__ __forceinline__ void dec_input_bwd_body(int B, int N, int C, int Tin, double* g_lat_v, double* part, double* lds, double* g_lat_l) {
  double* gcan = lds;
  double* gcart = gcan + N * 8;
  const double* wgl = gcart + N * 8;
  const double* latl = wgl + 2 * N * Tin;
  const double* gp_l = latl + Tin * 8;
  const double* pd_l = gp_l + N * 8;
  const double* gs_l = pd_l + N * 8;
  double* gv_l = const_cast<double*>(gs_l) + N * C * 2;
  const double* w1l = gv_l + N * C * 8;
  const int b = blockIdx.x;
  double* row = part + (size_t)b * (4 * C + 2 * N * Tin);
  STAMP(11);
  for (int e = threadIdx.x; e < N * 4; e += BLOCK) {
    const int n = e >> 2, m = e & 3;
    cx<double> g = {gp_l[n * 8 + m], gp_l[n * 8 + 4 + m]};
#pragma unroll 4
    for (int c = 0; c < C; ++c)
      cfmac(g, cx<double>{gv_l[(n * C + c) * 8 + m], gv_l[(n * C + c) * 8 + 4 + m]}, cx<double>{w1l[c], w1l[C + c]});
    gcan[n * 8 + m] = g.r;
    gcan[n * 8 + 4 + m] = g.i;
  }
  __syncthreads();
  for (int i = threadIdx.x; i < N * C; i += BLOCK) {
    const int n = i / C;
    cx<double> d0 = {0, 0}, d1 = {0, 0};
    cfmac(d0, cx<double>{gs_l[i * 2], gs_l[i * 2 + 1]}, cx<double>{1.0, 1.0});
#pragma unroll
    for (int m = 0; m < 4; ++m)
      cfmac(d1, cx<double>{gv_l[i * 8 + m], gv_l[i * 8 + 4 + m]}, cx<double>{pd_l[n * 8 + m], pd_l[n * 8 + 4 + m]});
    gv_l[i * 8 + 0] = d0.r;  gv_l[i * 8 + 1] = d0.i;  gv_l[i * 8 + 2] = d1.r;  gv_l[i * 8 + 3] = d1.i;
  }
  __syncthreads();
  STAMP(12);
  for (int e = threadIdx.x; e < N * 4; e += BLOCK) {
    const cx<double> gc = canon_cplx_bwd_m(gcan + (e >> 2) * 8, e & 3);
    gcart[(e >> 2) * 8 + (e & 3)] = gc.r;
    gcart[(e >> 2) * 8 + 4 + (e & 3)] = gc.i;
  }
  if ((int)threadIdx.x >= BLOCK - 64 && (int)threadIdx.x < BLOCK - 64 + 4 * C) {
    const int k = (threadIdx.x - (BLOCK - 64)) / C, c = (threadIdx.x - (BLOCK - 64)) - k * C;
    double acc = 0.0;
#pragma unroll 6
    for (int n = 0; n < N; ++n) acc += gv_l[(n * C + c) * 8 + k];
    row[k * C + c] = acc;
  }
  __syncthreads();
  STAMP(13);
  for (int e = threadIdx.x; e < Tin * 4; e += BLOCK) {
    const int t = e >> 2, m = e & 3;
    cx<double> acc = {0, 0};
#pragma unroll 6
    for (int n = 0; n < N; ++n)
      cfmac(acc, cx<double>{gcart[n * 8 + m], gcart[n * 8 + 4 + m]}, cx<double>{wgl[n * Tin + t], wgl[N * Tin + n * Tin + t]});
    g_lat_v[((size_t)b * Tin + t) * 4 + m] = acc.r;
    g_lat_v[(((size_t)B + b) * Tin + t) * 4 + m] = acc.i;
    if constexpr (TO_LDS) { g_lat_l[t * 8 + m] = acc.r; g_lat_l[t * 8 + 4 + m] = acc.i; }
  }
  for (int e = threadIdx.x; e < N * Tin; e += BLOCK) {
    const int n = e / Tin, t = e - n * Tin;
    cx<double> acc = {0, 0};
#pragma unroll
    for (int m = 0; m < 4; ++m)
      cfmac(acc, cx<double>{gcart[n * 8 + m], gcart[n * 8 + 4 + m]}, cx<double>{latl[t * 8 + m], latl[t * 8 + 4 + m]});
    row[4 * C + e] = acc.r;
    row[4 * C + N * Tin + e] = acc.i;
  }
}
__global__ __launch_bounds__(BLOCK) void dec_input_bwd_kernel(int B, int N, int C, int Tin, const double* __restrict__ lat_v,
                                                             const double* __restrict__ wg1, const double* __restrict__ w1,
                                                             const double* __restrict__ pdec, const double* __restrict__ g_p,
                                                             const double* __restrict__ g_s0, const double* __restrict__ g_v0,
                                                             double* g_lat_v, double* part) {
  extern __shared__ __align__(16) unsigned char smem_raw[];
  double* lds = reinterpret_cast<double*>(smem_raw);
  DecInBwdStage st;
  st.issue(B, N, C, Tin, lat_v, wg1, w1, pdec, g_p, g_s0, g_v0);
  st.commit(lds);
  __syncthreads();
  dec_input_bwd_body<false>(B, N, C, Tin, g_lat_v, part, lds, nullptr);
}

__global__ __launch_bounds__(BLOCK) void junction_fwd_kernel(int B, int N, int CL, int Ts, int Tv, const double* s, const double* v,
                                                            const double* wl0, const double* wl1, double* lat_s, double* lat_v,
                                                            int* idx, int C0, const double* wg1, const double* w0, const double* w1,
                                                            double* pdec, double* s0, double* v0, int overlap, int pool) {
  extern __shared__ __align__(16) unsigned char smem_raw[];
  double* lat_lds = reinterpret_cast<double*>(smem_raw);
  double* dec_lds = lat_lds + (overlap ? lat_fwd_doubles(N, CL, Ts, Tv, pool) : lat_y_doubles(N, Ts, Tv, pool));
  const int Tin = pool_blocks(pool) * Tv;
  STAMP(0);
  LatentStage ls;
  DecInFwdStage ds;
  ls.issue(B, N, CL, Ts, Tv, s, v, wl0, wl1, pool);
  if (overlap) ds.issue(B, N, C0, Tin, nullptr, wg1, w0, w1, false);
  ls.commit(lat_lds, false);
  if (overlap) ds.commit(dec_lds);
  __syncthreads();
// ... 463 lines not shown
```

lgn-autoencoder_amd/csrc/ops.hpp:

```cpp
#pragma once
#include <cstdlib>
#include <vector>
#include "level.hpp"

namespace lgn {

template <typename T> int level_fwd_dispatch(const LevelArgs<T>&, int decoder, hipStream_t);
int level_fwd_eval(const LevelArgs<double>&, int decoder, hipStream_t);
template <typename T> int level_bwd_dispatch(const LevelBwdArgs<T>&, int decoder, hipStream_t);
template <typename T> int reduce_partials(const T* part, int rows, int n, T* out, int accumulate, hipStream_t);
template <typename T> int reduce_partials_strided(const T* part, int rows, int stride, int col0, int n, T* out, hipStream_t);
constexpr int RED_MAX_SEG = 64;
template <typename T> struct RedSeg { const T* part; int rows, stride, col0, n; T* out; };
template <typename T> struct RedJob {
  int nseg;
  RedSeg<T> seg[RED_MAX_SEG];
  int tile0[RED_MAX_SEG + 1];
  void add(const T* part, int rows, int stride, int col0, int n, T* out) { seg[nseg++] = RedSeg<T>{part, rows, stride, col0, n, out}; }
};
template <typename T> int reduce_segments(RedJob<T>& job, hipStream_t);
template <typename T>
int rad_finalize(const T* tot, int C, const T* ra, const T* rb, const T* rc, const T* w0, const T* w1, T* g_a, T* g_b, T* g_c,
                 T* g_w0, T* g_b0, T* g_w1, T* g_b1, hipStream_t);
struct RadFinJob {
  int n;
  struct Item { const double* tot; int C; const double *ra, *rb, *rc, *w0, *w1; double *g_a, *g_b, *g_c, *g_w0, *g_b0, *g_w1, *g_b1; } it[4];
};
int rad_finalize_batch(const RadFinJob& job, hipStream_t);
struct StepTailArgs {
  double *w, *g;
  long n;
  double *m, *v;
  long* step_dev;
  double lambda, lr, beta1, beta2, eps;
  int do_adam;
  const double* loss_part;
  int nB;
  double* loss_out;
  int reduce_only;
  unsigned long long* counters;
};
int step_tail(const std::vector<RedSeg<double>>& segs, const RadFinJob& fin, const StepTailArgs& ta, hipStream_t st);
void level_bwd_partial_rows(int B, int N, int decoder, int flags, int* rows_mix, int* rows_rad);
bool level_bwd_carries_input(int N, int flags);
bool level_fwd_carries_loss(int N, int flags);

constexpr int MLP_MAX_LIN = 8;
template <typename T>
struct MlpArgs {
  int M;
  int C;
  int H;
  int nlin;
  const T* w[MLP_MAX_LIN];
  const T* b[MLP_MAX_LIN];
  const T* s_in;
  T* s_out;
  const T* g_out;
  T* g_in;
  T* part;
  int psize;
  int ld = 1;
  int tbQ = 0;
  T* h_saved = nullptr;
  int h_rows = 0;
  int act = 0;
  int flags = 0;
};
inline int mlp_saved_rows(int M) { return (M + 63) & ~63; }
inline size_t mlp_saved_doubles(int M, int H, int nlin) {
  return H <= 48 && nlin >= 4 && nlin <= 7 ? (size_t)(nlin - 1) * mlp_saved_rows(M) * ((H + 15) & ~15) : 0;
}
constexpr int MLP_SAVE_MAX_ROWS = 8128;
inline size_t mlp_save_max_rows() {
  static const long v = [] { const char* e = getenv("LGN_AMD_MLP_SAVE_ROWS"); return e ? atol(e) : (long)MLP_SAVE_MAX_ROWS; }();
  return (size_t)(v < 0 ? 0 : v);
}
template <typename T>
__host__ __device__ inline size_t mlp_out_index(const MlpArgs<T>& a, int z, int row, int ch) {
  if (a.tbQ > 0) return ((size_t)((row >> 6) * a.C + ch) * a.tbQ) * 128 + z * 64 + (row & 63);
  return ((size_t)z * a.M * a.C + (size_t)row * a.C + ch) * a.ld;
}
template <typename T> int mlp_dispatch(const MlpArgs<T>&, bool backward, hipStream_t);
int cg_product_fwd(int R, int N, int C, int D1, int D2, int DO, int mode, int nnz, const int* row_ptr, const int* col, const double* coef,
                   const double* x1, const double* x2, double* out, hipStream_t st);
int cg_product_bwd(int R, int N, int C, int D1, int D2, int DO, int mode, int nnz, const int* row_ptr, const int* col, const double* coef,
                   const double* x1, const double* x2, const double* g_out, double* g_x1, double* g_x2, hipStream_t st);
int mlp_mfma_dispatch(const MlpArgs<double>&, bool backward, hipStream_t);
int mlp_chain_dispatch(const MlpArgs<double>&, bool backward, hipStream_t);
int mlp_mfma_wide_dispatch(const MlpArgs<double>&, bool backward, hipStream_t);
inline int mlp_rows_per_workgroup(int M, int H) { return (H <= 48 && (M + 63) / 64 < 128) ? 16 : 64; }
inline int mlp_partial_rows(int M, int H) { const int r = mlp_rows_per_workgroup(M, H); return (M + r - 1) / r; }

template <typename T>
struct MixArgs {
  int rows, Cin, Cout, d;
  const T* w;
  const T* x;
  T* y;
  const T* g_y;
  T* g_x;
  T* part;
};
template <typename T> int mix_fwd(const MixArgs<T>&, hipStream_t);
template <typename T> int mix_bwd(const MixArgs<T>&, hipStream_t);
int mix_partial_rows(int rows);

struct GenArgs {
  int B, N, C, Q;
  const double* X;
  const double* p;
  const uint8_t* mask;
  const double *ra, *rb, *rc, *w0, *b0, *w1, *b1;
  double* U;
  const double* gU;
  double* gX;
  double* g_p;
  double* part_rad;
  double* gbuf;
  int flags;
  int tb;
};
__host__ __device__ inline size_t feat_index(bool tb, size_t plane, int C, int Qx, int n, int c, int q, int z) {
  return tb ? ((size_t)((n >> 6) * C + c) * Qx + q) * 128 + z * 64 + (n & 63) : (size_t)z * plane + ((size_t)n * C + c) * Qx + q;
}
size_t moments2_gbuf_doubles(int B, int N, int C);
int moments_dispatch(const GenArgs& a, int decoder, int which, hipStream_t st);

struct LocalTables {
  int n_rows, n_out, n_w;
  const int *row_ptr, *t_type, *t_a, *t_b;
  const double* t_coef;
  const int *out_dim, *out_nblk, *out_row0, *out_q0, *out_w0;
  const int *u_ptr, *u_row;
  const double* u_coef;
  const int *x_ptr, *x_row, *x_other;
  const double* x_coef;
};
struct LocalArgs {
  int nodes, C, CO, Q, Qout;
  int n_terms, n_u, n_x;
  int n_units;
  LocalTables t;
  const double* X;
  const double* U;
  const double* wcat;
  double* out;
  const double* g_out;
  double* gU;
  double* gX;
  double* part;
  double* s_copy;
  int q_s;
};
int local_fwd(const LocalArgs& a, hipStream_t st);
int local_bwd(const LocalArgs& a, hipStream_t st);
int local_partial_rows(int nodes);
size_t local_static_packed_doubles(int kind, int C, int CO);
int local_bwd_static(int kind, int M, int C, int CO, const double* XT, const double* UT, const double* w, const int* w0, double* wp,
                     const double* goT, double* gUT, double* gXT, double* part, hipStream_t st, bool packed = false,
                     bool param_layout = false);
int local_static_unpack_grads(int kind, int C, int CO, const int* w0, const double* gpacked, double* gw, hipStream_t st);
int local_fwd_static(int kind, int M, int C, int CO, const double* XT, const double* UT, const double* w, const int* w0, double* wp,
                     double* outT, double* s_copy, int q_s, hipStream_t st, bool packed = false);
constexpr int SEP_TBL_STRIDE = 24;
int dec_sep_tab(const GenArgs& a, double* tbl, double* pc, hipStream_t st);
int local_sep_part_rows(int B);
int local_fwd_sep(int kind, int B, int N, int C, int CO, const double* XT, const double* tbl, const double* pc, const double* wp,
                  double* outT, double* s_copy, int q_s, hipStream_t st);
int local_bwd_sep(int kind, int B, int N, int C, int CO, const double* XT, const double* tbl, const double* pc, const double* b0,
                  const double* b1, const double* wp, const int* w0p, const double* goT, double* gXT, double* part, double* gpb,
                  double* part_rad, hipStream_t st);
int local_sep_gp_reduce(const double* const* gpb, const int* C, int n, int M, double* g_p, hipStream_t st);
struct StaticPackJob { int kind, C, CO; int w0[5]; const double* src; double* dst; };
int local_static_pack_batch(const StaticPackJob* jobs, int n, bool unpack, hipStream_t st);
int anomaly_scores(const double* rec, const double* tgt, const double* rec_n, const double* tgt_n, int B, int N, int mask, double* scores,
                   int* col4row, int* status, hipStream_t st);
int linear_sum_assignment(const double* cost, int B, int n, int* col4row, int* status, hipStream_t st);
int gen_pack(size_t nodes_x_C, int Q, int q_s, int q_v, const double* s, const double* v, double* X, hipStream_t st);
int gen_unpack(size_t nodes_x_C, int Q, int q_s, int q_v, const double* X, double* s, double* v, hipStream_t st);
int gen_pack_tb(int M, int C, int Q, int q_s, int q_v, const double* s, const double* v, double* XT, hipStream_t st);
int gen_unpack_tb(int M, int C, int Q, int q_s, int q_v, const double* XT, double* s, double* v, hipStream_t st);

}
```

lgn-autoencoder_amd/csrc/step.hip:

```cpp
#include <stdlib.h>

#include <algorithm>
#include <mutex>
#include <vector>

#include "net.hpp"
#include "../../include/lgn_amd.h"

namespace lgn {
namespace {

struct Bump {
  double* base;
  size_t off = 0;
  double* take(size_t n) {
    n = (n + 15) & ~size_t(15);
    double* p = base ? base + off : nullptr;
    off += n;
    return p;
  }
};

struct NetBuf {
  double *s[5], *v[5], *smix[4], *ag0[4], *ag1[4];
// ... 62 lines not shown
  }
  if (int rc = finish_reductions(dq, fin, grads, n_params, tail ? nullptr : counters, flags, st)) return rc;
  if (!tail) return 0;
  const StepTailArgs& t = *tail;
  return finalize_step(t.w, t.g, t.n, t.loss_part, t.nB, t.lambda, t.m, t.v, t.step_dev, t.lr, t.beta1, t.beta2, t.eps, t.do_adam,
                       t.loss_out, st);
}

inline int in_K(const lgn_net_desc& d) { return d.n_in_scalars > 1 ? d.n_in_scalars : 1; }

int mlp_psize(int C, int H, int nlin) {
  const int D = 2 * C;
  return nlin == 1 ? D * D + D : (H * D + H) + (nlin - 2) * (H * H + H) + (D * H + D);
}

inline int dec_nodes(const lgn_net_desc& d) { return d.dec_N > 0 ? d.dec_N : d.N; }
inline bool step_is_split(const lgn_net_desc& d) { return dec_nodes(d) != d.N || d.n_in_scalars > 1; }
inline int dec_tin(const lgn_net_desc& d) { return d.tau_v_in > 0 ? d.tau_v_in : pool_blocks(d.latent_pool) * d.tau_v; }
int check_latent_match(const lgn_net_desc& d) {
  const int Tin = pool_blocks(d.latent_pool) * d.tau_v;
  LGN_CHECK_ARG(d.tau_v_in == 0 || d.tau_v_in == Tin, "step: the decoder must consume the encoder's %d pooled latent vectors", Tin);
  return 0;
}

struct Slots {
  int L, nlin;
  int in0(bool dec) const { return dec ? 2 : 0; }
  int rad(bool dec, int l, int k) const { return in0(dec) + 2 + 7 * l + k; }
  int mix(bool dec, int l, int k) const { return in0(dec) + 2 + 7 * L + 2 * l + k; }
  int mlp(bool dec, int l, int k) const { return in0(dec) + 2 + 9 * L + 2 * nlin * l + k; }
  int out0(bool dec) const { return in0(dec) + 2 + 9 * L + 2 * nlin * L; }
  int count(bool dec) const { return out0(dec) + 2; }
};

struct RowLayout {
  int width, nseg, col[3], n[3], slot[3];
  void add(Deferred& dq, const double* part, int rows, double* G, const int64_t* off) const {
    for (int i = 0; i < nseg; ++i) dq.add(part, rows, width, col[i], n[i], G + off[slot[i]]);
  }
};
RowLayout enc_latent_rows(const lgn_net_desc& d, int N, int CL) {
  const int KL = pool_mix_in(d.latent_pool, N, CL), o = Slots{d.n_levels, d.mlp_nlin}.out0(false);
  return {2 * (d.tau_s + d.tau_v) * KL, 2, {0, 2 * d.tau_s * KL}, {2 * d.tau_s * KL, 2 * d.tau_v * KL}, {o, o + 1}};
}
RowLayout enc_input_rows(int K, int C0) { return {(2 * K + 2) * C0, 2, {0, 2 * C0 * K}, {2 * C0 * K, 2 * C0}, {0, 1}}; }
RowLayout dec_input_rows(int C0, int N, int Tin) {
  return {4 * C0 + 2 * N * Tin, 3, {0, 2 * C0, 4 * C0}, {2 * C0, 2 * C0, 2 * N * Tin}, {2, 3, 1}};
}
RowLayout dec_output_rows(const lgn_net_desc& d, int CL) {
  return {2 * CL, 1, {0}, {2 * CL}, {Slots{d.n_levels, d.mlp_nlin}.out0(true) + 1}};
}

inline size_t r16(size_t n) { return (n + 15) & ~size_t(15); }
size_t end_parts(const lgn_net_desc& d, bool dec, int N, int in_rows) {
  const int* ch = dec ? d.dec_channels : d.enc_channels;
  const int L = d.n_levels;
  if (dec) return r16((size_t)d.B * dec_output_rows(d, ch[L]).width) + r16((size_t)d.B * dec_input_rows(ch[0], N, dec_tin(d)).width);
  return r16((size_t)d.B * enc_latent_rows(d, N, ch[L]).width) + r16((size_t)in_rows * enc_input_rows(in_K(d), ch[0]).width);
}
size_t net_parts(const lgn_net_desc& d, bool dec, int N) {
  const int* ch = dec ? d.dec_channels : d.enc_channels;
  int rm, rr;
  level_bwd_partial_rows(d.B, N, dec, d.flags, &rm, &rr);
  size_t sum = 0;
  for (int l = 0; l < d.n_levels; ++l) {
    const int H = d.mlp_hidden_mul * 2 * ch[l + 1];
    sum += r16((size_t)rm * 4 * ch[l + 1] * 5 * ch[l]) + r16((size_t)rr * rad_partial_size(ch[l], dec)) +
           r16((size_t)mlp_partial_rows(d.B * (dec ? dec_nodes(d) : N), H) * mlp_psize(ch[l + 1], H, d.mlp_nlin));
  }
  return sum + end_parts(d, dec, N, rm > d.B ? rm : d.B);
}

Work carve(const lgn_net_desc& d, double* base) {
  Work w{};
  Bump b{base};
  const int Nd = dec_nodes(d), Nmax = d.N > Nd ? d.N : Nd;
  const size_t BNe = (size_t)d.B * d.N, BNd = (size_t)d.B * Nd, BN = (size_t)d.B * Nmax;
  const int L = d.n_levels;
  int cmax = 0;
  for (int l = 0; l <= L; ++l) cmax = cmax > d.enc_channels[l] ? cmax : d.enc_channels[l], cmax = cmax > d.dec_channels[l] ? cmax : d.dec_channels[l];
  auto net = [&](NetBuf& n, const int* ch, bool dec) {
    const size_t BN = dec ? BNd : BNe;
    for (int l = 0; l <= L; ++l) {
      n.s[l] = b.take(2 * BN * ch[l]);
      n.v[l] = b.take(8 * BN * ch[l]);
    }
    for (int l = 0; l < L; ++l) {
      n.smix[l] = b.take(2 * BN * ch[l + 1]);
      n.ag0[l] = b.take(4 * BN * ch[l]);
      n.ag1[l] = b.take(16 * BN * ch[l]);
      const size_t hs = l + 1 < L && BN <= mlp_save_max_rows()
                            ? mlp_saved_doubles((int)BN, d.mlp_hidden_mul * 2 * ch[l + 1], d.mlp_nlin) : 0;
      n.hsave[l] = hs ? b.take(hs) : nullptr;
    }
  };
  net(w.enc, d.enc_channels, false);
  net(w.dec, d.dec_channels, true);
  const int Ts = d.tau_s, Tv = d.tau_v, PB = pool_blocks(d.latent_pool);
  w.lat_s = b.take((size_t)2 * d.B * PB * Ts);
  w.lat_v = b.take((size_t)2 * d.B * PB * Tv * 4);
  w.g_lat_v = b.take((size_t)2 * d.B * PB * Tv * 4);
  w.pdec = b.take(8 * BN);
  for (int q = 0; q < 2; ++q) {
    w.gs[q] = b.take(2 * BN * cmax);
    w.gv[q] = b.take(8 * BN * cmax);
  }
  w.gsmix = b.take(2 * BN * cmax);
  w.g_ag = b.take(20 * BN * cmax);
  {
    const size_t z0 = b.off;
    w.zeros_s = b.take(2 * BN * cmax);
    w.g_p = b.take(8 * BN);
    w.g_lat_s = b.take((size_t)2 * d.B * PB * d.tau_s);
    w.tail_cnt = b.take(8);
    w.zero_doubles = b.off - z0;
  }
  w.idx = reinterpret_cast<int*>(b.take(((size_t)d.B * 2 * (Ts + Tv) * 2 + 1) / 2 + 8));
  for (int dec = 0; dec < 2; ++dec)
    for (int l = 0; l < L; ++l) w.tot[dec][l] = b.take(rad_partial_size((dec ? d.dec_channels : d.enc_channels)[l], dec != 0) + 16);
  const size_t psum = net_parts(d, false, d.N) + net_parts(d, true, Nd);
  w.parts = b.take(psum);
  w.parts_size = psum;
  w.total = b.off;
  return w;
}

#define HIPOK(e) do { hipError_t e_ = (e); if (e_ != hipSuccess) { set_error("%s: %s", #e, hipGetErrorString(e_)); return (int)e_; } } while (0)
#define DQ_NEW(var, n) double* var = nullptr; DQ_TAKE(var, n)
#define DQ_TAKE(lhs, n)                                                                                           \
  lhs = dq.take(n);                                                                                             \
  LGN_CHECK_ARG((lhs) != nullptr, "partial-row workspace overflow: %zu + %zu doubles > capacity %zu (carve / take mismatch)", \
                dq.off, (size_t)(n), dq.cap)
#define LGN_TRY(expr)            \
  do {                           \
    int rc_ = (expr);            \
    if (rc_ != 0) return rc_;    \
  } while (0)

struct InputStage {
  const double *w0, *w1;
  double* z1 = nullptr;
  size_t z1n = 0;
  double* z2 = nullptr;
  size_t z2n = 0;
};
struct LossStage {
  const double *wo1, *target;
  double scale;
  int method;
  double jscale;
  double *recon, *loss_part, *g_v, *wpart;
};

MlpArgs<double> level_mlp_args(const lgn_net_desc& d, bool dec, int l, const double* P, const int64_t* off) {
  const Slots S{d.n_levels, d.mlp_nlin};
  const int CO = (dec ? d.dec_channels : d.enc_channels)[l + 1];
  MlpArgs<double> m{};
  m.M = d.B * d.N; m.C = CO; m.H = d.mlp_hidden_mul * 2 * CO; m.nlin = d.mlp_nlin; m.act = d.activation; m.flags = d.flags;
  for (int q = 0; q < d.mlp_nlin; ++q) { m.w[q] = P + off[S.mlp(dec, l, 2 * q)]; m.b[q] = P + off[S.mlp(dec, l, 2 * q + 1)]; }
  return m;
}

int levels_fwd(const lgn_net_desc& d, bool dec, const int* ch, const double* P, const int64_t* off, NetBuf& n, const double* pos,
               const uint8_t* mask, hipStream_t st, const InputStage* in0 = nullptr, const LossStage* loss = nullptr, bool eval = false,
               bool last_scalars = true) {
  const Slots S{d.n_levels, d.mlp_nlin};
  for (int l = 0; l < d.n_levels; ++l) {
    auto p = [&](int slot) { return P + off[slot]; };
    LevelArgs<double> a{d.B, d.N, ch[l], ch[l + 1], n.s[l], n.v[l], pos, mask,
                        p(S.rad(dec, l, 0)), p(S.rad(dec, l, 1)), p(S.rad(dec, l, 2)), p(S.rad(dec, l, 3)), p(S.rad(dec, l, 4)),
                        p(S.rad(dec, l, 5)), p(S.rad(dec, l, 6)), p(S.mix(dec, l, 0)), p(S.mix(dec, l, 1)),
                        n.ag0[l], n.ag1[l], n.smix[l], n.v[l + 1]};
    if (l == 0 && !dec && in0) {
      a.in_w0 = in0->w0; a.in_w1 = in0->w1; a.in_s = n.s[0]; a.in_v = n.v[0];
      a.z1 = in0->z1; a.z1n = in0->z1n; a.z2 = in0->z2; a.z2n = in0->z2n;
    }
    if (l + 1 == d.n_levels && dec && loss) {
      a.loss_wo1 = loss->wo1; a.loss_target = loss->target; a.loss_scale = loss->scale; a.loss_real = loss->method;
      a.loss_jscale = loss->jscale; a.loss_recon = loss->recon;
      a.loss_part = loss->loss_part; a.loss_gv = loss->g_v; a.loss_wpart = loss->wpart;
    }
    a.flags = d.flags;
    LGN_TRY(eval ? level_fwd_eval(a, dec, st) : level_fwd_dispatch<double>(a, dec, st));
    if (l + 1 == d.n_levels && (!last_scalars || (eval && dec))) break;
    MlpArgs<double> m = level_mlp_args(d, dec, l, P, off);
    m.s_in = n.smix[l]; m.s_out = n.s[l + 1];
    m.h_saved = n.hsave[l]; m.h_rows = mlp_saved_rows(m.M);
    LGN_TRY(mlp_dispatch<double>(m, false, st));
  }
  return 0;
}

int levels_bwd(const lgn_net_desc& d, bool dec, const int* ch, const double* P, double* G, const int64_t* off, const NetBuf& n,
               const double* pos, const uint8_t* mask, Work& w, Deferred& dq, RadFinJob& fin, int& cur, bool has_s_grad,
               hipStream_t st, bool* in0_done = nullptr) {
  const Slots S{d.n_levels, d.mlp_nlin};
  const int BN = d.B * d.N;
  for (int l = d.n_levels - 1; l >= 0; --l) {
    auto p = [&](int slot) { return P + off[slot]; };
    auto g = [&](int slot) { return G + off[slot]; };
    const int C = ch[l], CO = ch[l + 1];
    const double* g_smix = w.zeros_s;
    if (has_s_grad) {
      MlpArgs<double> m = level_mlp_args(d, dec, l, P, off);
      m.s_in = n.smix[l]; m.g_out = w.gs[cur]; m.g_in = w.gsmix;
      m.h_saved = n.hsave[l];
      m.h_rows = mlp_saved_rows(BN);
      m.psize = mlp_psize(CO, m.H, m.nlin);
      DQ_TAKE(m.part, (size_t)mlp_partial_rows(BN, m.H) * m.psize);
      LGN_TRY(mlp_dispatch<double>(m, true, st));
      dq.add(m.part, mlp_partial_rows(BN, m.H), m.psize, 0, m.psize, g(S.mlp(dec, l, 0)));
      g_smix = w.gsmix;
    }
    int rm, rr;
    level_bwd_partial_rows(d.B, d.N, dec, d.flags, &rm, &rr);
    const int nmix = 4 * CO * 5 * C, nrad = rad_partial_size(C, dec);
    DQ_NEW(part_mix, (size_t)rm * nmix);
    DQ_NEW(part_rad, (size_t)rr * nrad);
    const int nxt = cur ^ 1;
    LevelBwdArgs<double> a{d.B, d.N, C, CO, n.s[l], n.v[l], pos, mask,
                           p(S.rad(dec, l, 0)), p(S.rad(dec, l, 1)), p(S.rad(dec, l, 2)), p(S.rad(dec, l, 3)), p(S.rad(dec, l, 4)),
                           p(S.rad(dec, l, 5)), p(S.rad(dec, l, 6)), p(S.mix(dec, l, 0)), p(S.mix(dec, l, 1)), n.ag0[l], n.ag1[l],
                           g_smix, w.gv[cur], w.g_ag, w.gs[nxt], w.gv[nxt], dec ? w.g_p : nullptr, part_mix, part_rad};
    const bool carry_in0 = !dec && l == 0 && in0_done && level_bwd_carries_input(d.N, d.flags);
    const RowLayout rin = enc_input_rows(1, C);
    if (carry_in0) { DQ_TAKE(a.part_in0, (size_t)rm * rin.width); }
    a.flags = d.flags;
    LGN_TRY(level_bwd_dispatch<double>(a, dec, st));
    if (carry_in0) {
      rin.add(dq, a.part_in0, rm, G, off);
      *in0_done = true;
    }
    dq.add(part_mix, rm, nmix, 0, nmix / 2, g(S.mix(dec, l, 0)));
    dq.add(part_mix, rm, nmix, nmix / 2, nmix / 2, g(S.mix(dec, l, 1)));
    if (dec) {
      dq.add(part_rad, rr, nrad, 0, C, g(S.rad(dec, l, 4)));
      dq.add(part_rad, rr, nrad, C, C, g(S.rad(dec, l, 6)));
    } else {
      double* tot = w.tot[0][l];
      dq.add(part_rad, rr, nrad, 0, nrad, tot);
      fin.it[fin.n++] = RadFinJob::Item{tot, C, p(S.rad(dec, l, 0)), p(S.rad(dec, l, 1)), p(S.rad(dec, l, 2)), p(S.rad(dec, l, 3)),
                                        p(S.rad(dec, l, 5)), g(S.rad(dec, l, 0)), g(S.rad(dec, l, 1)), g(S.rad(dec, l, 2)),
                                        g(S.rad(dec, l, 3)), g(S.rad(dec, l, 4)), g(S.rad(dec, l, 5)), g(S.rad(dec, l, 6))};
    }
    cur = nxt;
    has_s_grad = true;
  }
  return 0;
}

int check_desc(const lgn_net_desc* d) {
  LGN_CHECK_ARG(d, "step: null descriptor");
  LGN_CHECK_ARG(d->B > 0 && d->N > 0, "step: empty batch (B=%d N=%d)", d->B, d->N);
  LGN_CHECK_ARG(d->n_levels >= 1 && d->n_levels <= 4, "step: n_levels=%d unsupported (1..4)", d->n_levels);
  LGN_CHECK_ARG(d->mlp_nlin >= 4 && d->mlp_nlin <= 7, "step: mlp_depth must be 3 .. 6 (4 .. 7 Linear layers), got %d layers", d->mlp_nlin);
  LGN_CHECK_ARG(d->tau_s >= 1 && d->tau_v >= 1 && d->tau_v_in >= 0, "step: latent multiplicities must be positive");
  LGN_CHECK_ARG(d->n_in_scalars >= 0 && d->n_in_scalars <= 8, "step: n_in_scalars=%d unsupported (0..8)", d->n_in_scalars);
  LGN_CHECK_ARG(pool_valid(d->latent_pool), "step: latent_pool=%d is not an LGN_POOL(...) code", d->latent_pool);
  for (int l = 0; l <= d->n_levels; ++l)
    LGN_CHECK_ARG(d->enc_channels[l] >= 1 && d->enc_channels[l] <= 8 && d->dec_channels[l] >= 1 && d->dec_channels[l] <= 8,
                  "step: channel counts must be in 1..8");
  LGN_CHECK_ARG(d->get_real >= LGN_REAL_SUM && d->get_real <= LGN_REAL_NORM, "step: get_real=%d is not an LGN_REAL_* code", d->get_real);
  LGN_CHECK_ARG(d->jet_loss_scale >= 0.0, "step: jet_loss_scale=%g must be >= 0", d->jet_loss_scale);
  LGN_CHECK_ARG(d->dec_N >= 0, "step: dec_N=%d must be >= 0", d->dec_N);
  if (d->dec_N > 0) {
    const size_t need = decoder_end_lds_bytes(d->dec_N, d->dec_channels[0], dec_tin(*d), d->dec_channels[d->n_levels]);
    LGN_CHECK_ARG(need <= LGN_LDS_LIMIT, "step: dec_N=%d: the decoder end stages need %zu B of LDS (> %d)", d->dec_N, need, LGN_LDS_LIMIT);
  }
  return 0;
}

}

}


namespace lgn {
namespace {
struct ZeroJob { double* p[3]; size_t n[3]; };
__global__ __launch_bounds__(BLOCK) void zero_ranges_kernel(ZeroJob job) {
  const size_t stride = (size_t)gridDim.x * BLOCK;
#pragma unroll
  for (int q = 0; q < 3; ++q)
    for (size_t i = (size_t)blockIdx.x * BLOCK + threadIdx.x; i < job.n[q]; i += stride) job.p[q][i] = 0.0;
}
int zero_ranges(double* a, size_t na, double* b, size_t nb, double* c, size_t nc, hipStream_t st) {
  const ZeroJob job{{a, b, c}, {a ? na : 0, b ? nb : 0, c ? nc : 0}};
  const size_t most = std::max(job.n[0], std::max(job.n[1], job.n[2]));
  if (!most) return 0;
  const int blocks = (int)std::min<size_t>((most + BLOCK - 1) / BLOCK, 1024);
  hipLaunchKernelGGL(zero_ranges_kernel, dim3(blocks), dim3(BLOCK), 0, st, job);
  LGN_CHECK_LAUNCH();
  return 0;
}
int zero_grads_and_block(double* grads, size_t n, double* zeros, size_t nz, hipStream_t st) {
  if (zeros >= grads + n && zeros <= grads + n + 16) return zero_ranges(grads, (size_t)((zeros + nz) - grads), nullptr, 0, nullptr, 0, st);
  return zero_ranges(grads, n, zeros, nz, nullptr, 0, st);
}

int check_mlp_contiguous(const lgn_net_desc& d, bool dec, const int64_t* off) {
  const Slots S{d.n_levels, d.mlp_nlin};
  const int* ch = dec ? d.dec_channels : d.enc_channels;
  for (int l = 0; l < d.n_levels; ++l) {
    const int D = 2 * ch[l + 1], H = d.mlp_hidden_mul * D;
    int64_t expect = off[S.mlp(dec, l, 0)];
    for (int q = 0; q < d.mlp_nlin; ++q) {
      const int hin = q == 0 ? D : H, hout = q == d.mlp_nlin - 1 ? D : H;
      LGN_CHECK_ARG(off[S.mlp(dec, l, 2 * q)] == expect, "MLP weights are not contiguous in the flat parameter buffer");
      expect += (int64_t)hin * hout;
      LGN_CHECK_ARG(off[S.mlp(dec, l, 2 * q + 1)] == expect, "MLP biases are not contiguous in the flat parameter buffer");
      expect += hout;
    }
  }
  return 0;
}

}
}

namespace lgn {
namespace {

inline bool is_generic(const lgn_net_desc& d, bool dec) { return (dec ? d.dec_tables[0] : d.enc_tables[0]) != nullptr; }

struct GenGeom {
  const int *ch, *Q, *qs, *qv;
  const lgn_local_tables* const* tab;
};
inline GenGeom geom(const lgn_net_desc& d, bool dec) {
  return dec ? GenGeom{d.dec_channels, d.dec_Q, d.dec_qs, d.dec_qv, d.dec_tables}
             : GenGeom{d.enc_channels, d.enc_Q, d.enc_qs, d.enc_qv, d.enc_tables};
}

inline bool is_static(const lgn_net_desc& d, bool dec) {
  const GenGeom g = geom(d, dec);
  if (d.N > 32) return false;
  for (int l = 0; l < d.n_levels; ++l)
    if (!g.tab[l] || g.tab[l]->static_kind == 0) return false;
  return !(d.flags & LGN_NET_NO_STATIC);
}
inline bool is_sep_fused(const lgn_net_desc& d, bool dec) {
  return dec && is_static(d, dec) && !(d.flags & (LGN_NET_DEC_PAIRWISE | LGN_NET_DEC_UNFUSED));
}
inline size_t tb_doubles(const lgn_net_desc& d, int C, int Qx) { return (size_t)(((size_t)d.B * d.N + 63) / 64) * C * Qx * 128; }

int check_generic(const lgn_net_desc& d, bool dec) {
  const GenGeom g = geom(d, dec);
  for (int l = 0; l < d.n_levels; ++l) {
    LGN_CHECK_ARG(g.tab[l], "table-driven network: level %d has no tables (every level needs one)", l);
    LGN_CHECK_ARG(g.tab[l]->n_w > 0 && g.tab[l]->n_rows > 0, "table-driven network: empty tables at level %d", l);
  }
  for (int l = 0; l <= d.n_levels; ++l)
    LGN_CHECK_ARG(g.Q[l] >= 5 && g.Q[l] <= 64 && g.qs[l] >= 0 && g.qs[l] < g.Q[l] && g.qv[l] >= 0 && g.qv[l] + 4 <= g.Q[l],
                  "table-driven network: bad component layout at level %d (Q=%d qs=%d qv=%d)", l, g.Q[l], g.qs[l], g.qv[l]);
  LGN_CHECK_ARG(g.Q[0] == 5, "table-driven network: the input level carries (1,1) and (0,0) only (Q=5), got %d", g.Q[0]);
  return 0;
}

struct GenAct {
  double *s0, *v0;
  double *X[5], *U[4], *smix[4];
  double* wp[4];
  double* tbl[4];
  double* pc;
  double *sL, *vL;
  double* pdec;
  int* idx;
  size_t total;
};
GenAct carve_gen_act(const lgn_net_desc& d, bool dec, double* base) {
  GenAct a{};
  Bump b{base};
  const GenGeom g = geom(d, dec);
  const size_t BN = (size_t)d.B * d.N;
  const int L = d.n_levels;
  a.s0 = b.take(2 * BN * g.ch[0]);
  a.v0 = b.take(8 * BN * g.ch[0]);
  const bool tb = is_static(d, dec);
  const bool sep = is_sep_fused(d, dec);
  for (int l = 0; l <= L; ++l) a.X[l] = b.take(tb ? tb_doubles(d, g.ch[l], g.Q[l]) : 2 * BN * g.ch[l] * g.Q[l]);
  a.pc = sep ? b.take(8 * BN) : nullptr;
  for (int l = 0; l < L; ++l) {
    a.U[l] = sep ? nullptr : b.take(tb ? tb_doubles(d, g.ch[l], 5 * g.Q[l]) : 10 * BN * g.ch[l] * g.Q[l]);
    a.tbl[l] = sep ? b.take((size_t)d.B * g.ch[l] * g.Q[l] * SEP_TBL_STRIDE) : nullptr;
    a.smix[l] = b.take(2 * BN * g.ch[l + 1]);
    a.wp[l] = tb ? b.take(local_static_packed_doubles(g.tab[l]->static_kind, g.ch[l], g.ch[l + 1])) : nullptr;
  }
  a.sL = b.take(2 * BN * g.ch[L]);
  a.vL = b.take(8 * BN * g.ch[L]);
  if (dec) a.pdec = b.take(8 * BN);
  else a.idx = reinterpret_cast<int*>(b.take(((size_t)d.B * 2 * (d.tau_s + d.tau_v) * 2 + 1) / 2 + 8));
  a.total = b.off;
  return a;
}

struct GenScratch {
  double *zero0, *g_p, *g_lat_s;
  size_t zero_doubles;
  double *gs, *gv;
  double *gX[2], *gU;
  double* gbuf;
  double* gpk[4];
  double* gpb[4];
  double* tot[4];
  double* parts;
  size_t parts_size, total;
};
size_t gen_net_parts(const lgn_net_desc& d, bool dec) {
  const GenGeom g = geom(d, dec);
  const size_t BN = (size_t)d.B * d.N, tiles = (BN + 63) / 64;
  const bool tb = is_static(d, dec), sep = is_sep_fused(d, dec);
  size_t sum = 0;
  for (int l = 0; l < d.n_levels; ++l) {
    const int H = d.mlp_hidden_mul * 2 * g.ch[l + 1];
    const size_t lrows = tb ? (sep ? (size_t)local_sep_part_rows(d.B) : tiles) * local_static_packed_doubles(g.tab[l]->static_kind, g.ch[l], g.ch[l + 1])
                            : (size_t)local_partial_rows((int)BN) * 2 * g.tab[l]->n_w;
    sum += r16(lrows) + r16((size_t)d.B * rad_partial_size(g.ch[l], dec)) +
           r16((size_t)mlp_partial_rows((int)BN, H) * mlp_psize(g.ch[l + 1], H, d.mlp_nlin));
  }
  return sum + end_parts(d, dec, d.N, d.B);
}

GenScratch carve_gen_scratch(const lgn_net_desc& d, bool dec, double* base) {
  GenScratch s{};
  Bump b{base};
  const GenGeom g = geom(d, dec);
  const size_t BN = (size_t)d.B * d.N;
  const int L = d.n_levels;
  size_t cq = 0, cmax = 0;
  for (int l = 0; l <= L; ++l) {
    cq = cq > (size_t)g.ch[l] * g.Q[l] ? cq : (size_t)g.ch[l] * g.Q[l];
    cmax = cmax > (size_t)g.ch[l] ? cmax : (size_t)g.ch[l];
  }
  {
    const size_t z0 = b.off;
    s.zero0 = b.take(2 * BN * cmax);
    s.g_p = b.take(dec ? 8 * BN : 0);
    s.g_lat_s = b.take(dec ? 0 : (size_t)2 * d.B * pool_blocks(d.latent_pool) * d.tau_s);
    s.zero_doubles = b.off - z0;
  }
  s.gs = b.take(2 * BN * cmax);
  s.gv = b.take(8 * BN * cmax);
  const bool tb = is_static(d, dec), sep = is_sep_fused(d, dec);
  const size_t tiles = (BN + 63) / 64;
  s.gX[0] = b.take(tb ? tiles * cq * 128 : 2 * BN * cq);
  s.gX[1] = b.take(tb ? tiles * cq * 128 : 2 * BN * cq);
  s.gU = sep ? nullptr : b.take(tb ? tiles * cq * 640 : 10 * BN * cq);
  for (int l = 0; l < L; ++l) {
    s.gpk[l] = tb ? b.take(local_static_packed_doubles(g.tab[l]->static_kind, g.ch[l], g.ch[l + 1])) : nullptr;
    s.gpb[l] = sep ? b.take((size_t)g.ch[l] * BN * 8) : nullptr;
  }
  s.gbuf = (!dec && d.N <= 32) ? b.take(moments2_gbuf_doubles(d.B, d.N, (int)cmax)) : nullptr;
  for (int l = 0; l < L; ++l) s.tot[l] = b.take(rad_partial_size(g.ch[l], dec) + 16);
  const size_t psum = gen_net_parts(d, dec);
  s.parts = b.take(psum);
  s.parts_size = psum;
  s.total = b.off;
  return s;
}

GenArgs gen_level_args(const lgn_net_desc& d, bool dec, int l, const double* P, const int64_t* off, const double* X, const double* pos,
                       const uint8_t* mask) {
  const Slots S{d.n_levels, d.mlp_nlin};
  const GenGeom g = geom(d, dec);
  GenArgs a{};
  a.B = d.B; a.N = d.N; a.C = g.ch[l]; a.Q = g.Q[l]; a.X = X; a.p = pos; a.mask = mask;
  a.flags = d.flags;
  a.ra = P + off[S.rad(dec, l, 0)]; a.rb = P + off[S.rad(dec, l, 1)]; a.rc = P + off[S.rad(dec, l, 2)];
  a.w0 = P + off[S.rad(dec, l, 3)]; a.b0 = P + off[S.rad(dec, l, 4)]; a.w1 = P + off[S.rad(dec, l, 5)]; a.b1 = P + off[S.rad(dec, l, 6)];
  return a;
}

int gen_levels_fwd(const lgn_net_desc& d, bool dec, const double* P, const int64_t* off, GenAct& a, const double* pos,
                   const uint8_t* mask, hipStream_t st) {
  const Slots S{d.n_levels, d.mlp_nlin};
  const GenGeom g = geom(d, dec);
// ... 430 lines not shown
  LGN_CHECK_ARG(params && grads && off && p4 && mask && act && g_lat_v && scratch && n_params > 0, "encoder_bwd: null pointer");
  LGN_CHECK_ARG(d->n_in_scalars <= 1 || in_scalars, "encoder_bwd: %d input scalars per node, but in_scalars is NULL", d->n_in_scalars);
  if (is_generic(*d, false)) {
    if (int rc = check_generic(*d, false)) return rc;
    GenAct ga = carve_gen_act(*d, false, const_cast<double*>(act));
    GenScratch gs = carve_gen_scratch(*d, false, scratch);
    LGN_CHECK_ARG((long long)ga.total <= act_doubles && (long long)gs.total <= scratch_doubles,
                  "encoder_bwd: buffers hold %lld / %lld doubles, need %zu / %zu", act_doubles, scratch_doubles, ga.total, gs.total);
    if (int rc = check_mlp_contiguous(*d, false, off)) return rc;
    LGN_TRY(zero_grads_and_block(grads, (size_t)n_params, gs.zero0, gs.zero_doubles, (hipStream_t)stream));
    return gen_encoder_bwd(*d, params, grads, off, p4, mask, ga, g_lat_s, g_lat_v, gs, (hipStream_t)stream, in_scalars);
  }
  NetAct a = carve_act(*d, false, const_cast<double*>(act));
  NetScratch sc = carve_scratch(*d, false, scratch);
  LGN_CHECK_ARG((long long)a.total <= act_doubles && (long long)sc.total <= scratch_doubles,
                "encoder_bwd: buffers hold %lld / %lld doubles, need %zu / %zu", act_doubles, scratch_doubles, a.total, sc.total);
  if (int rc = check_mlp_contiguous(*d, false, off)) return rc;
  hipStream_t st = (hipStream_t)stream;
  Work& w = sc.w;
  const Slots S{d->n_levels, d->mlp_nlin};
  const int L = d->n_levels, B = d->B, N = d->N;
  const int* ce = d->enc_channels;
  LGN_TRY(zero_grads_and_block(grads, (size_t)n_params, w.zero0(), w.zero_doubles, st));
  Deferred dq;
  dq.parts = w.parts;
  dq.cap = w.parts_size;
  RadFinJob fin{};
  int cur = 0;
  {
    const RowLayout rl = enc_latent_rows(*d, N, ce[L]);
    DQ_NEW(parte, (size_t)B * rl.width);
    LGN_TRY(enc_latent_bwd(B, N, ce[L], d->tau_s, d->tau_v, d->latent_pool, a.n.s[L], a.n.v[L], params + off[S.out0(false)],
                           params + off[S.out0(false) + 1], g_lat_s ? g_lat_s : w.g_lat_s, g_lat_v, a.idx, w.gs[cur], w.gv[cur], parte, st));
    rl.add(dq, parte, B, grads, off);
  }
  bool in0_done = false;
  const int K = in_K(*d);
  LGN_TRY(levels_bwd(*d, false, ce, params, grads, off, a.n, p4, mask, w, dq, fin, cur, g_lat_s != nullptr, st,
                     K > 1 ? nullptr : &in0_done));
  if (!in0_done) {
    const RowLayout ri = enc_input_rows(K, ce[0]);
    DQ_NEW(part, (size_t)B * ri.width);
    LGN_TRY(enc_input_bwd(B, N, ce[0], K, p4, in_scalars, w.gs[cur], w.gv[cur], part, st));
    ri.add(dq, part, B, grads, off);
  }
  LGN_CHECK_ARG(dq.off <= dq.cap, "encoder_bwd: partial-row workspace overflow (%zu > %zu)", dq.off, dq.cap);
  LGN_TRY(finish_reductions(dq, fin, grads, n_params, nullptr, d->flags, st));
  return 0;
}

int lgn_decoder_fwd_f64(const lgn_net_desc* d, const double* params, const int64_t* off, const double* lat_v, double* act,
                        long long act_doubles, double* recon, void* stream) {
  if (int rc = check_desc(d)) return rc;
  LGN_CHECK_ARG(params && off && lat_v && act && recon, "decoder_fwd: null pointer");
  if (is_generic(*d, true)) {
    if (int rc = check_generic(*d, true)) return rc;
    GenAct ga = carve_gen_act(*d, true, act);
    LGN_CHECK_ARG((long long)ga.total <= act_doubles, "decoder_fwd: activation buffer holds %lld doubles, needs %zu", act_doubles, ga.total);
    LGN_TRY(gen_decoder_fwd(*d, params, off, lat_v, ga, (hipStream_t)stream));
    const Slots Sg{d->n_levels, d->mlp_nlin};
    return dec_output_fwd(d->B, d->N, d->dec_channels[d->n_levels], ga.vL, params + off[Sg.out0(true) + 1], recon, (hipStream_t)stream);
  }
  NetAct a = carve_act(*d, true, act);
  LGN_CHECK_ARG((long long)a.total <= act_doubles, "decoder_fwd: activation buffer holds %lld doubles, needs %zu", act_doubles, a.total);
  hipStream_t st = (hipStream_t)stream;
  const Slots S{d->n_levels, d->mlp_nlin};
  const int L = d->n_levels;
  const int* cd = d->dec_channels;
  LGN_TRY(dec_input_fwd(d->B, d->N, cd[0], dec_tin(*d), lat_v, params + off[1], params + off[2], params + off[3], a.pdec, a.n.s[0], a.n.v[0], st));
  LGN_TRY(levels_fwd(*d, true, cd, params, off, a.n, a.pdec, nullptr, st));
  LGN_TRY(dec_output_fwd(d->B, d->N, cd[L], a.n.v[L], params + off[S.out0(true) + 1], recon, st));
  return 0;
}

int lgn_decoder_bwd_f64(const lgn_net_desc* d, const double* params, double* grads, long long n_params, const int64_t* off,
                        const double* lat_v, const double* act, long long act_doubles, const double* g_recon, double* g_lat_v,
                        double* scratch, long long scratch_doubles, void* stream) {
  if (int rc = check_desc(d)) return rc;
  LGN_CHECK_ARG(params && grads && off && lat_v && act && g_recon && g_lat_v && scratch && n_params > 0, "decoder_bwd: null pointer");
  if (is_generic(*d, true)) {
    if (int rc = check_generic(*d, true)) return rc;
    hipStream_t gst = (hipStream_t)stream;
    GenAct ga = carve_gen_act(*d, true, const_cast<double*>(act));
    GenScratch gs = carve_gen_scratch(*d, true, scratch);
    LGN_CHECK_ARG((long long)ga.total <= act_doubles && (long long)gs.total <= scratch_doubles,
                  "decoder_bwd: buffers hold %lld / %lld doubles, need %zu / %zu", act_doubles, scratch_doubles, ga.total, gs.total);
    if (int rc = check_mlp_contiguous(*d, true, off)) return rc;
    LGN_TRY(zero_grads_and_block(grads, (size_t)n_params, gs.zero0, gs.zero_doubles, gst));
    const Slots Sg{d->n_levels, d->mlp_nlin};
    const int CL = d->dec_channels[d->n_levels];
    Deferred dq;
    dq.parts = gs.parts;
    dq.cap = gs.parts_size;
    RadFinJob fin{};
    const RowLayout ro = dec_output_rows(*d, CL);
    DQ_NEW(part, (size_t)d->B * ro.width);
    LGN_TRY(dec_output_bwd(d->B, d->N, CL, ga.vL, params + off[Sg.out0(true) + 1], g_recon, gs.gv, part, gst));
    ro.add(dq, part, d->B, grads, off);
    std::vector<UnpackJob> post;
    LGN_TRY(gen_decoder_bwd(*d, params, grads, off, lat_v, ga, g_lat_v, gs, dq, fin, post, gst));
    LGN_CHECK_ARG(dq.off <= dq.cap, "decoder_bwd: partial-row workspace overflow (%zu > %zu)", dq.off, dq.cap);
    LGN_TRY(dq.flush(gst));
    return run_unpack_jobs(post, gst);
  }
  NetAct a = carve_act(*d, true, const_cast<double*>(act));
  NetScratch sc = carve_scratch(*d, true, scratch);
  LGN_CHECK_ARG((long long)a.total <= act_doubles && (long long)sc.total <= scratch_doubles,
                "decoder_bwd: buffers hold %lld / %lld doubles, need %zu / %zu", act_doubles, scratch_doubles, a.total, sc.total);
  if (int rc = check_mlp_contiguous(*d, true, off)) return rc;
  hipStream_t st = (hipStream_t)stream;
  Work& w = sc.w;
  const Slots S{d->n_levels, d->mlp_nlin};
  const int L = d->n_levels, B = d->B, N = d->N, Tin = dec_tin(*d);
  const int* cd = d->dec_channels;
  LGN_TRY(zero_grads_and_block(grads, (size_t)n_params, w.zero0(), w.zero_doubles, st));
  Deferred dq;
  dq.parts = w.parts;
  dq.cap = w.parts_size;
  RadFinJob fin{};
  int cur = 0;
  {
    const RowLayout ro = dec_output_rows(*d, cd[L]);
    DQ_NEW(part, (size_t)B * ro.width);
    LGN_TRY(dec_output_bwd(B, N, cd[L], a.n.v[L], params + off[S.out0(true) + 1], g_recon, w.gv[cur], part, st));
    ro.add(dq, part, B, grads, off);
  }
  LGN_TRY(levels_bwd(*d, true, cd, params, grads, off, a.n, a.pdec, nullptr, w, dq, fin, cur, false, st));
  {
    const RowLayout ri = dec_input_rows(cd[0], N, Tin);
    DQ_NEW(part, (size_t)B * ri.width);
    LGN_TRY(dec_input_bwd(B, N, cd[0], Tin, lat_v, params + off[1], params + off[3], a.pdec, w.g_p, w.gs[cur], w.gv[cur], g_lat_v, part, st));
    ri.add(dq, part, B, grads, off);
  }
  LGN_CHECK_ARG(dq.off <= dq.cap, "decoder_bwd: partial-row workspace overflow (%zu > %zu)", dq.off, dq.cap);
  return finish_reductions(dq, fin, grads, n_params, nullptr, d->flags, st);
}

}

extern "C" {

int lgn_step_param_slots(const lgn_net_desc* d, int decoder) {
  if (check_desc(d)) return -1;
  return Slots{d->n_levels, d->mlp_nlin}.count(decoder != 0);
}

long long lgn_encoder_end_lds_bytes(int N, int C0, int K, int CL, int Ts, int Tv, int pool) {
  return pool_valid(pool) ? (long long)encoder_end_lds_bytes(N, C0, K < 1 ? 1 : K, CL, Ts, Tv, pool) : -1;
}
long long lgn_decoder_end_lds_bytes(int N, int C0, int Tin, int CL) { return (long long)decoder_end_lds_bytes(N, C0, Tin, CL); }
long long lgn_junction_lds_bytes(int N, int CL, int Ts, int Tv, int pool, int C0) {
  return pool_valid(pool) ? (long long)junction_lds_bytes(N, CL, Ts, Tv, pool, C0) : -1;
}

long long lgn_step_workspace_doubles(const lgn_net_desc* d) {
  if (check_desc(d) || check_latent_match(*d)) return -1;
  if (is_generic(*d, false) || is_generic(*d, true)) {
    if (check_generic(*d, false) || check_generic(*d, true)) return -1;
    return (long long)carve_gen_step(*d, nullptr).total;
  }
  return (long long)carve(*d, nullptr).total;
}

}
static int step_fwd_bwd(const lgn_net_desc* dp, const double* params, double* grads, long long n_params, const int64_t* enc_off,
                        const int64_t* dec_off, const double* p4, const double* target, const uint8_t* mask, const double* in_scalars,
                        double* workspace, long long workspace_doubles, double* recon, double* loss_part, void* stream,
                        const StepTailArgs* tail) {
  if (int rc = check_desc(dp)) return rc;
  const lgn_net_desc& d = *dp;
  LGN_CHECK_ARG(params && grads && enc_off && dec_off && p4 && target && mask && workspace && recon && loss_part && n_params > 0,
                "step_fwd_bwd: null pointer");
  LGN_CHECK_ARG(d.n_in_scalars <= 1 || in_scalars, "step_fwd_bwd: %d input scalars per node, but in_scalars is NULL", d.n_in_scalars);
  if (int rc = check_latent_match(d)) return rc;
  hipStream_t st = (hipStream_t)stream;
  const bool split = step_is_split(d);
  if (is_generic(d, false) || is_generic(d, true)) {
    LGN_CHECK_ARG(!split, "step_fwd_bwd: table-driven networks take the mass as the only input scalar and one node count "
                  "for both networks (n_in_scalars=%d, N=%d, dec_N=%d): use the per-network calls", d.n_in_scalars, d.N, d.dec_N);
    return gen_step_fwd_bwd(d, params, grads, n_params, enc_off, dec_off, p4, target, mask, workspace, workspace_doubles, recon,
                            loss_part, st, tail);
  }
  Work w = carve(d, workspace);
  LGN_CHECK_ARG((long long)w.total <= workspace_doubles, "step: workspace holds %lld doubles, this configuration needs %zu",
                workspace_doubles, w.total);
  if (int rc = check_mlp_contiguous(d, false, enc_off)) return rc;
  if (int rc = check_mlp_contiguous(d, true, dec_off)) return rc;
  lgn_net_desc dd = d;
  dd.N = dec_nodes(d);
  const Slots S{d.n_levels, d.mlp_nlin};
  const int L = d.n_levels, B = d.B, Ne = d.N, Nd = dd.N, Ts = d.tau_s, Tv = d.tau_v, K = in_K(d), Tin = dec_tin(d);
  const int* ce = d.enc_channels;
  const int* cd = d.dec_channels;
  const double* wl0 = params + enc_off[S.out0(false)];
  const double* wl1 = params + enc_off[S.out0(false) + 1];
  Deferred dq;
  dq.parts = w.parts;
  dq.cap = w.parts_size;
  RadFinJob fin{};

  if (split) {
    LGN_TRY(zero_ranges(grads, (size_t)n_params, w.zero0(), w.zero_doubles, nullptr, 0, st));
    LGN_TRY(enc_input_fwd(B, Ne, ce[0], K, p4, in_scalars, params + enc_off[0], params + enc_off[1], w.enc.s[0], w.enc.v[0], st));
    LGN_TRY(levels_fwd(d, false, ce, params, enc_off, w.enc, p4, mask, st, nullptr, nullptr, false, false));
    LGN_TRY(enc_latent_fwd(B, Ne, ce[L], Ts, Tv, d.latent_pool, nullptr, w.enc.v[L], wl0, wl1, w.lat_s, w.lat_v, w.idx, st));
    LGN_TRY(dec_input_fwd(B, Nd, cd[0], Tin, w.lat_v, params + dec_off[1], params + dec_off[2], params + dec_off[3], w.pdec, w.dec.s[0],
                          w.dec.v[0], st));
  } else {
    const InputStage in0{params + enc_off[0], params + enc_off[1], grads, (size_t)n_params, w.zeros_s, w.zero_doubles};
    LGN_TRY(levels_fwd(d, false, ce, params, enc_off, w.enc, p4, mask, st, &in0, nullptr, false, false));
    LGN_TRY(junction_fwd(B, Ne, ce[L], Ts, Tv, d.latent_pool, nullptr, w.enc.v[L], wl0, wl1, w.lat_s, w.lat_v, w.idx, cd[0],
                         params + dec_off[1], params + dec_off[2], params + dec_off[3], w.pdec, w.dec.s[0], w.dec.v[0], st));
  }
  int cur = 0;
  {
    const RowLayout ro = dec_output_rows(d, cd[L]);
    DQ_NEW(part, (size_t)B * ro.width);
    const LossStage ls{params + dec_off[S.out0(true) + 1], target, 1.0, d.get_real, d.jet_loss_scale, recon, loss_part, w.gv[cur], part};
    const bool rides = level_fwd_carries_loss(Nd, d.flags);
    LGN_TRY(levels_fwd(dd, true, cd, params, dec_off, w.dec, w.pdec, nullptr, st, nullptr, rides ? &ls : nullptr, false,
                       false));
    if (!rides)
      LGN_TRY(dec_output_loss(B, Nd, cd[L], w.dec.v[L], ls.wo1, target, 1.0, ls.method, ls.jscale, recon, loss_part, w.gv[cur], part, st));
    ro.add(dq, part, B, grads, dec_off);
  }

  LGN_TRY(levels_bwd(dd, true, cd, params, grads, dec_off, w.dec, w.pdec, nullptr, w, dq, fin, cur, false, st));
  {
    const RowLayout ri = dec_input_rows(cd[0], Nd, Tin), rl = enc_latent_rows(d, Ne, ce[L]);
    DQ_NEW(part, (size_t)B * ri.width);
    DQ_NEW(parte, (size_t)B * rl.width);
    const int rd = cur, wr = cur ^ 1;
    cur = wr;
    if (split) {
      LGN_TRY(dec_input_bwd(B, Nd, cd[0], Tin, w.lat_v, params + dec_off[1], params + dec_off[3], w.pdec, w.g_p, w.gs[rd], w.gv[rd],
                            w.g_lat_v, part, st));
      LGN_TRY(enc_latent_bwd(B, Ne, ce[L], Ts, Tv, d.latent_pool, nullptr, w.enc.v[L], wl0, wl1, w.g_lat_s, w.g_lat_v, w.idx, w.gs[wr],
                             w.gv[wr], parte, st));
    } else {
      LGN_TRY(junction_bwd(B, Ne, cd[0], Tin, w.lat_v, params + dec_off[1], params + dec_off[3], w.pdec, w.g_p, w.gs[rd], w.gv[rd], w.g_lat_v,
                           part, ce[L], Ts, Tv, d.latent_pool, nullptr, w.enc.v[L], wl0, wl1, w.g_lat_s, w.idx, w.gs[wr], w.gv[wr], parte, st));
    }
    ri.add(dq, part, B, grads, dec_off);
    rl.add(dq, parte, B, grads, enc_off);
  }
  bool in0_done = false;
  LGN_TRY(levels_bwd(d, false, ce, params, grads, enc_off, w.enc, p4, mask, w, dq, fin, cur, false, st,
                     split ? nullptr : &in0_done));
  if (!in0_done) {
    const RowLayout ri = enc_input_rows(K, ce[0]);
    DQ_NEW(part, (size_t)B * ri.width);
    LGN_TRY(enc_input_bwd(B, Ne, ce[0], K, p4, split ? in_scalars : nullptr, w.gs[cur], w.gv[cur], part, st));
    ri.add(dq, part, B, grads, enc_off);
  }
  return end_step(dq, fin, grads, n_params, w.tail_cnt, d.flags, tail, st);
}
extern "C" {

int lgn_step_fwd_bwd_f64(const lgn_net_desc* d, const double* params, double* grads, long long n_params, const int64_t* enc_off,
                         const int64_t* dec_off, const double* p4, const double* target, const uint8_t* mask, const double* in_scalars,
                         double* workspace, long long workspace_doubles, double* recon, double* loss_part, void* stream) {
  return step_fwd_bwd(d, params, grads, n_params, enc_off, dec_off, p4, target, mask, in_scalars, workspace, workspace_doubles, recon,
                      loss_part, stream, nullptr);
}

int lgn_step_train_f64(const lgn_net_desc* d, double* params, double* grads, long long n_params, const int64_t* enc_off,
                       const int64_t* dec_off, const double* p4, const double* target, const uint8_t* mask, const double* in_scalars,
                       double* workspace, long long workspace_doubles, double* recon, double* loss_part, int n_loss, double l1_lambda, double* adam_m,
                       double* adam_v, long long* step_dev, double lr, double beta1, double beta2, double eps, int do_adam,
                       double* loss_out, void* stream) {
  LGN_CHECK_ARG(loss_out && n_loss > 0, "step_train: null pointer");
  LGN_CHECK_ARG(!do_adam || (adam_m && adam_v && step_dev), "step_train: Adam state missing");
  const StepTailArgs tail{params, grads, (long)n_params, adam_m, adam_v, reinterpret_cast<long*>(step_dev), l1_lambda, lr, beta1, beta2,
                          eps, do_adam, loss_part, n_loss, loss_out, 0, nullptr};
  return step_fwd_bwd(d, params, grads, n_params, enc_off, dec_off, p4, target, mask, in_scalars, workspace, workspace_doubles, recon,
                      loss_part, stream, &tail);
}

int lgn_step_finalize_f64(double* params, double* grads, long long n_params, const double* loss_part, int n_loss, double l1_lambda,
                          double* adam_m, double* adam_v, long long* step_dev, double lr, double beta1, double beta2, double eps,
                          int do_adam, double* loss_out, void* stream) {
  LGN_CHECK_ARG(params && grads && loss_part && loss_out && n_params > 0 && n_loss > 0, "step_finalize: null pointer");
  LGN_CHECK_ARG(!do_adam || (adam_m && adam_v && step_dev), "step_finalize: Adam state missing");
  hipStream_t st = (hipStream_t)stream;
  LGN_TRY(finalize_step(params, grads, (long)n_params, loss_part, n_loss, l1_lambda, adam_m, adam_v, reinterpret_cast<long*>(step_dev),
                        lr, beta1, beta2, eps, do_adam, loss_out, st));
  return 0;
}

}

namespace lgn {
namespace {

struct EvalWork {
  NetBuf enc, dec;
  double *lat_s, *lat_v, *pdec;
  int* idx;
  size_t total;
};

EvalWork carve_eval(const lgn_net_desc& d, double* base) {
  EvalWork w{};
  Bump b{base};
  const int L = d.n_levels, Nd = dec_nodes(d);
  const size_t BNe = (size_t)d.B * d.N, BNd = (size_t)d.B * Nd;
  size_t smix = 0;
  auto net = [&](NetBuf& n, const int* ch, size_t BN) {
    int cmax = 0;
    for (int l = 0; l <= L; ++l) cmax = cmax > ch[l] ? cmax : ch[l];
    double *s[2], *v[2];
    for (int q = 0; q < 2; ++q) {
      s[q] = b.take(2 * BN * cmax);
      v[q] = b.take(8 * BN * cmax);
    }
    for (int l = 0; l <= L; ++l) {
      n.s[l] = s[l & 1];
      n.v[l] = v[l & 1];
    }
    smix = std::max(smix, 2 * BN * cmax);
  };
  net(w.enc, d.enc_channels, BNe);
  net(w.dec, d.dec_channels, BNd);
  double* sm = b.take(smix);
  for (int l = 0; l < L; ++l) w.enc.smix[l] = w.dec.smix[l] = sm;
  const int PB = pool_blocks(d.latent_pool);
  w.lat_s = b.take((size_t)2 * d.B * PB * d.tau_s);
  w.lat_v = b.take((size_t)2 * d.B * PB * d.tau_v * 4);
  w.pdec = b.take(8 * BNd);
  w.idx = reinterpret_cast<int*>(b.take(((size_t)d.B * 2 * (d.tau_s + d.tau_v) * 2 + 1) / 2 + 8));
  w.total = b.off;
  return w;
}

struct GenEval {
  GenAct ea, da;
  double *lat_s, *lat_v;
  size_t total;
};
GenEval carve_gen_eval(const lgn_net_desc& d, double* base) {
  GenEval g{};
  auto at = [&](size_t off) { return base ? base + off : nullptr; };
  size_t off = 0;
  g.ea = carve_gen_act(d, false, at(off)); off += (g.ea.total + 15) & ~size_t(15);
  g.da = carve_gen_act(d, true, at(off)); off += (g.da.total + 15) & ~size_t(15);
  const int P = pool_blocks(d.latent_pool);
  g.lat_s = at(off); off += ((size_t)2 * d.B * P * d.tau_s + 15) & ~size_t(15);
  g.lat_v = at(off); off += ((size_t)2 * d.B * P * d.tau_v * 4 + 15) & ~size_t(15);
  g.total = off;
  return g;
}

long long eval_workspace(const lgn_net_desc& d) {
  if (is_generic(d, false) || is_generic(d, true)) {
    if (check_generic(d, false) || check_generic(d, true)) return -1;
    return (long long)carve_gen_eval(d, nullptr).total;
  }
  return (long long)carve_eval(d, nullptr).total;
}

int step_eval(const lgn_net_desc* dp, const double* params, const int64_t* enc_off, const int64_t* dec_off, const double* p4,
              const double* target, const uint8_t* mask, const double* in_scalars, double* workspace, long long workspace_doubles,
              double* recon_real, double* lat_s_out, double* lat_v_out, double* loss_part, double* loss_out, hipStream_t st) {
  if (int rc = check_desc(dp)) return rc;
  const lgn_net_desc& d = *dp;
  LGN_CHECK_ARG(params && enc_off && dec_off && p4 && target && mask && workspace && recon_real && loss_part && loss_out,
                "step_eval: null pointer");
  LGN_CHECK_ARG(d.n_in_scalars <= 1 || in_scalars, "step_eval: %d input scalars per node, but in_scalars is NULL", d.n_in_scalars);
  LGN_CHECK_ARG(!lat_s_out == !lat_v_out, "step_eval: give both latent outputs or neither");
  if (int rc = check_latent_match(d)) return rc;
  const long long need = eval_workspace(d);
  if (need < 0) return -1;
  LGN_CHECK_ARG(need <= workspace_doubles, "step_eval: workspace holds %lld doubles, this configuration needs %lld", workspace_doubles, need);
  if (int rc = check_mlp_contiguous(d, false, enc_off)) return rc;
  if (int rc = check_mlp_contiguous(d, true, dec_off)) return rc;
  const Slots S{d.n_levels, d.mlp_nlin};
  const int L = d.n_levels, B = d.B, Ne = d.N, Nd = dec_nodes(d), Ts = d.tau_s, Tv = d.tau_v, Tin = dec_tin(d);
  const int* ce = d.enc_channels;
  const int* cd = d.dec_channels;
  const double* wl0 = params + enc_off[S.out0(false)];
  const double* wl1 = params + enc_off[S.out0(false) + 1];
  const double* wo1 = params + dec_off[S.out0(true) + 1];

  if (is_generic(d, false) || is_generic(d, true)) {
    LGN_CHECK_ARG(is_generic(d, false) && is_generic(d, true), "step_eval: encoder and decoder must both be table-driven (or both fused)");
    LGN_CHECK_ARG(!step_is_split(d), "step_eval: table-driven networks take the mass as the only input scalar and one node count for "
                  "both networks (n_in_scalars=%d, N=%d, dec_N=%d)", d.n_in_scalars, d.N, d.dec_N);
    GenEval g = carve_gen_eval(d, workspace);
    double* ls = lat_s_out ? lat_s_out : g.lat_s;
    double* lv = lat_v_out ? lat_v_out : g.lat_v;
    LGN_TRY(gen_encoder_fwd(d, params, enc_off, p4, mask, g.ea, ls, lv, st, nullptr, false));
    LGN_TRY(junction_fwd(B, Ne, ce[L], Ts, Tv, d.latent_pool, g.ea.sL, g.ea.vL, wl0, wl1, ls, lv, g.ea.idx, cd[0], params + dec_off[1],
                         params + dec_off[2], params + dec_off[3], g.da.pdec, g.da.s0, g.da.v0, st));
    LGN_TRY(gen_decoder_fwd(d, params, dec_off, lv, g.da, st, false));
    LGN_TRY(dec_output_eval(B, Ne, cd[L], g.da.vL, wo1, target, d.get_real, d.jet_loss_scale, recon_real, loss_part, st));
    return eval_loss_sum(B, Ne, mask, loss_part, loss_out, st);
  }

  EvalWork w = carve_eval(d, workspace);
  double* ls = lat_s_out ? lat_s_out : w.lat_s;
  double* lv = lat_v_out ? lat_v_out : w.lat_v;
  lgn_net_desc dd = d;
  dd.N = Nd;
  const LossStage loss{wo1, target, 1.0, d.get_real, d.jet_loss_scale, recon_real, loss_part, nullptr, nullptr};
  const bool rides = level_fwd_carries_loss(Nd, d.flags);
  const bool keep_s = lat_s_out != nullptr;
  const double* sL = keep_s ? w.enc.s[L] : nullptr;
  if (step_is_split(d)) {
    LGN_TRY(enc_input_fwd(B, Ne, ce[0], in_K(d), p4, in_scalars, params + enc_off[0], params + enc_off[1], w.enc.s[0], w.enc.v[0], st));
    LGN_TRY(levels_fwd(d, false, ce, params, enc_off, w.enc, p4, mask, st, nullptr, nullptr, true, keep_s));
    LGN_TRY(enc_latent_fwd(B, Ne, ce[L], Ts, Tv, d.latent_pool, sL, w.enc.v[L], wl0, wl1, ls, lv, w.idx, st));
    LGN_TRY(dec_input_fwd(B, Nd, cd[0], Tin, lv, params + dec_off[1], params + dec_off[2], params + dec_off[3], w.pdec, w.dec.s[0],
                          w.dec.v[0], st));
  } else {
    const InputStage in0{params + enc_off[0], params + enc_off[1]};
    LGN_TRY(levels_fwd(d, false, ce, params, enc_off, w.enc, p4, mask, st, &in0, nullptr, true, keep_s));
    LGN_TRY(junction_fwd(B, Ne, ce[L], Ts, Tv, d.latent_pool, sL, w.enc.v[L], wl0, wl1, ls, lv, w.idx, cd[0],
                         params + dec_off[1], params + dec_off[2], params + dec_off[3], w.pdec, w.dec.s[0], w.dec.v[0], st));
  }
  LGN_TRY(levels_fwd(dd, true, cd, params, dec_off, w.dec, w.pdec, nullptr, st, nullptr, rides ? &loss : nullptr, true));
  if (!rides) LGN_TRY(dec_output_eval(B, Nd, cd[L], w.dec.v[L], wo1, target, d.get_real, d.jet_loss_scale, recon_real, loss_part, st));
  return eval_loss_sum(B, Ne, mask, loss_part, loss_out, st);
}

}
}

extern "C" {

long long lgn_eval_workspace_doubles(const lgn_net_desc* d) {
  if (check_desc(d)) return -1;
  return eval_workspace(*d);
}

int lgn_step_eval_f64(const lgn_net_desc* d, const double* params, const int64_t* enc_off, const int64_t* dec_off,
                      const double* p4_scaled, const double* p4_target, const uint8_t* mask, const double* in_scalars,
                      double* workspace, long long workspace_doubles, double* recon_real, double* lat_s, double* lat_v,
                      double* loss_part, double* loss_out, void* stream) {
  return step_eval(d, params, enc_off, dec_off, p4_scaled, p4_target, mask, in_scalars, workspace, workspace_doubles, recon_real, lat_s,
                   lat_v, loss_part, loss_out, (hipStream_t)stream);
}

}
```

lgn-autoencoder_amd/lgn/_native.py:

```python
from __future__ import annotations

import ctypes as C
import os
from typing import Optional, Sequence

import torch

_HERE = os.path.dirname(os.path.abspath(__file__))
LIB_PATH = os.environ.get("LGN_AMD_LIB") or os.path.join(_HERE, "_lib", "liblgn_amd.so")
ABI_VERSION = 18
FINALIZE_SCRATCH = 2048

_lib: Optional[C.CDLL] = None

_vp, _i, _ip = C.c_void_p, C.c_int, C.POINTER(C.c_int)

_SIGNATURES = {
    "lgn_level_fwd_f64": [_i] * 5 + [_vp] * 18,
    "lgn_level_bwd_partial_rows": [_i, _i, _i, _ip, _ip],
    "lgn_level_rad_partial_len": [_i, _i],
    "lgn_level_jet_split": [_i, _i],
    "lgn_cg_product_fwd_f64": [_i] * 8 + [_vp] * 7,
    "lgn_cg_product_bwd_f64": [_i] * 8 + [_vp] * 9,
    "lgn_level_bwd_f64": [_i] * 5 + [_vp] * 24,
    "lgn_reduce_partials_f64": [_vp, _i, _i, _vp, _i, _vp],
    "lgn_radial_finalize_f64": [_vp, _i] + [_vp] * 13,
    "lgn_cgmlp_fwd_f64": [_i] * 5 + [_vp] * 5,
    "lgn_cgmlp_partial_rows": [_i, _i],
    "lgn_cgmlp_bwd_f64": [_i] * 5 + [_vp] * 6 + [_i, _vp],
    "lgn_mixreps_fwd_f64": [_i] * 4 + [_vp] * 4,
    "lgn_chamfer_f64": [_i] * 3 + [_vp] * 2 + [_i] + [_vp] * 4,
    "lgn_mixreps_partial_rows": [_i],
    "lgn_mixreps_bwd_f64": [_i] * 4 + [_vp] * 6,
}


class LocalTables(C.Structure):
    _fields_ = [("n_rows", C.c_int), ("n_out", C.c_int), ("n_w", C.c_int), ("n_terms", C.c_int), ("n_u", C.c_int),
                ("n_x", C.c_int), ("n_units", C.c_int), ("static_kind", C.c_int)] + [
        (name, C.c_void_p) for name in ("row_ptr", "t_type", "t_a", "t_b", "t_coef", "out_dim", "out_nblk", "out_row0", "out_q0",
                                        "out_w0", "u_ptr", "u_row", "u_coef", "x_ptr", "x_row", "x_other", "x_coef")] + [("h_out_w0", C.c_int * 8)]


_tp = C.POINTER(LocalTables)


_POOL_OPS = {"min": 0, "max": 1, "mean": 2, "average": 2}


def pool_code(map_to_latent: str):
    m = map_to_latent.lower()
    if m == "mix":
        return 1 | (3 << 4)
    if "&" in m and "+" in m:
        return None
    avg = "+" in m
    ops = m.split("+") if avg else m.split("&")
    if not 1 <= len(ops) <= 4 or any(o not in _POOL_OPS for o in ops):
        return None
    code = len(ops) | (int(avg) << 3)
    for i, o in enumerate(ops):
        code |= _POOL_OPS[o] << (4 + 2 * i)
    return code


def end_stages_fit(encoder=None, decoder=None, junction: bool = False) -> bool:
    L = lib()
    need = 0
    if encoder is not None:
        code = pool_code(encoder.map_to_latent)
        if code is None:
            return False
        n = encoder.num_input_particles
        ch = encoder.num_channels
        ts, tv = encoder.tau_latent[(0, 0)], encoder.tau_latent[(1, 1)]
        need = max(need, L.lgn_encoder_end_lds_bytes(n, ch[0], max(1, encoder.tau_input_scalars), ch[-1], ts, tv, code))
        if junction and decoder is not None:
            need = max(need, L.lgn_junction_lds_bytes(n, ch[-1], ts, tv, code, decoder.num_channels[0]))
    if decoder is not None:
        ch = decoder.num_channels
        need = max(need, L.lgn_decoder_end_lds_bytes(decoder.num_output_particles, ch[0], decoder.tau_latent_vectors, ch[-1]))
    return 0 <= need <= LDS_LIMIT


def pool_blocks(code: int) -> int:
    if code == 0:
        return 2
    return 1 if (code >> 3) & 1 else code & 7


class NetDesc(C.Structure):
    _fields_ = [("B", C.c_int), ("N", C.c_int), ("n_levels", C.c_int), ("enc_channels", C.c_int * 5),
                ("dec_channels", C.c_int * 5), ("tau_s", C.c_int), ("tau_v", C.c_int), ("mlp_hidden_mul", C.c_int),
                ("mlp_nlin", C.c_int), ("tau_v_in", C.c_int),
                ("enc_tables", _tp * 4), ("dec_tables", _tp * 4),
                ("enc_Q", C.c_int * 5), ("enc_qs", C.c_int * 5), ("enc_qv", C.c_int * 5),
                ("dec_Q", C.c_int * 5), ("dec_qs", C.c_int * 5), ("dec_qv", C.c_int * 5), ("flags", C.c_int),
                ("activation", C.c_int), ("n_in_scalars", C.c_int), ("latent_pool", C.c_int), ("dec_N", C.c_int),
                ("get_real", C.c_int), ("jet_loss_scale", C.c_double)]

    def __init__(self, *a, **kw):
        super().__init__(*a, **kw)
        self.flags = net_flags()


NET_NO_STATIC = 1
_NET_FLAG_ENV = {"LGN_AMD_NO_STATIC": 1, "LGN_AMD_DEC_PAIRWISE": 2, "LGN_AMD_LEVEL_V2": 4, "LGN_AMD_MLP_V1": 8,
                 "LGN_AMD_MOMENTS_V1": 16, "LGN_AMD_BWD_ORDERED": 64, "LGN_AMD_SPLIT_TAIL": 128, "LGN_AMD_DEC_UNFUSED": 256, "LGN_AMD_MOMENTS_SPLIT": 512,
                 "LGN_AMD_MLP_BWD1": 1024}
ACTIVATIONS = {"leakyrelu": 0, "relu": 1, "elu": 2, "sigmoid": 3, "logsigmoid": 4, "atan": 5}


def activation_id(name: str) -> int:
    try:
        return ACTIVATIONS[name.lower()]
    except KeyError:
        raise ValueError(f"Activation function {name} not implemented!") from None


def net_flags() -> int:
    return sum(bit for name, bit in _NET_FLAG_ENV.items() if os.environ.get(name, "") == "1")


_dp = C.POINTER(NetDesc)
_ll = C.c_longlong
_d = C.c_double
_SIGNATURES.update({
    "lgn_moments_fwd_f64": [_i] * 5 + [_vp] * 12,
    "lgn_moments_bwd_f64": [_i] * 5 + [_vp] * 16,
    "lgn_local_fwd_f64": [_i] * 5 + [_tp] + [_vp] * 5,
    "lgn_local_partial_rows": [_i],
    "lgn_local_fwd_static_f64": [_i] * 4 + [_vp] * 3 + [_ip] + [_vp] * 3 + [_i, _vp],
    "lgn_local_bwd_static_f64": [_i] * 4 + [_vp] * 3 + [_ip] + [_vp] * 8,
    "lgn_local_bwd_f64": [_i] * 5 + [_tp] + [_vp] * 8,
    "lgn_step_param_slots": [_dp, _i],
    "lgn_step_fwd_bwd_f64": [_dp, _vp, _vp, _ll, _vp, _vp, _vp, _vp, _vp, _vp, _vp, _ll, _vp, _vp, _vp],
    "lgn_encoder_fwd_f64": [_dp, _vp, _vp, _vp, _vp, _vp, _vp, _ll, _vp, _vp, _vp],
    "lgn_encoder_bwd_f64": [_dp, _vp, _vp, _ll, _vp, _vp, _vp, _vp, _vp, _ll, _vp, _vp, _vp, _ll, _vp],
    "lgn_decoder_fwd_f64": [_dp, _vp, _vp, _vp, _vp, _ll, _vp, _vp],
    "lgn_decoder_bwd_f64": [_dp, _vp, _vp, _ll, _vp, _vp, _vp, _ll, _vp, _vp, _vp, _ll, _vp],
    "lgn_step_finalize_f64": [_vp, _vp, _ll, _vp, _i, _d, _vp, _vp, _vp, _d, _d, _d, _d, _i, _vp, _vp],
    "lgn_step_train_f64": [_dp, _vp, _vp, _ll, _vp, _vp, _vp, _vp, _vp, _vp, _vp, _ll, _vp, _vp, _i, _d, _vp, _vp, _vp, _d, _d, _d, _d, _i,
                           _vp, _vp],
    "lgn_step_eval_f64": [_dp, _vp, _vp, _vp, _vp, _vp, _vp, _vp, _vp, _ll, _vp, _vp, _vp, _vp, _vp, _vp],
    "lgn_anomaly_scores_f64": [_vp] * 4 + [_i] * 3 + [_vp] * 4,
    "lgn_linear_sum_assignment_f64": [_vp, _i, _i, _vp, _vp, _vp],
})
_LL_SIGNATURES = {
    "lgn_step_workspace_doubles": [_dp],
    "lgn_eval_workspace_doubles": [_dp],
    "lgn_net_workspace_doubles": [_dp, _i, _i],
    "lgn_moments_scratch_doubles": [_i, _i, _i, _i],
    "lgn_local_static_packed_doubles": [_i, _i, _i],
    "lgn_encoder_end_lds_bytes": [_i] * 7,
    "lgn_decoder_end_lds_bytes": [_i] * 4,
    "lgn_junction_lds_bytes": [_i] * 6,
}
LDS_LIMIT = 160 * 1024
EXPORTED_SYMBOLS = ["lgn_abi_version", "lgn_last_error"] + list(_LL_SIGNATURES) + list(_SIGNATURES)


def lib() -> C.CDLL:
    global _lib
    if _lib is None:
        if not os.path.exists(LIB_PATH):
            raise RuntimeError(
                f"liblgn_amd.so not found at {LIB_PATH}. Build it with `python -c 'import __graft_entry__ as g; "
                "g.build()'` or `make -C lgn-autoencoder_amd/csrc`. There is no CPU fallback.")
        l = C.CDLL(LIB_PATH)
        l.lgn_abi_version.restype = C.c_int
        l.lgn_last_error.restype = C.c_char_p
        got = l.lgn_abi_version()
        if got != ABI_VERSION:
            raise RuntimeError(f"liblgn_amd.so ABI version {got} != expected {ABI_VERSION}; rebuild the library")
        for name, argtypes in _SIGNATURES.items():
            fn = getattr(l, name)
            fn.argtypes = argtypes
            fn.restype = C.c_int
        for name, argtypes in _LL_SIGNATURES.items():
            fn = getattr(l, name)
            fn.argtypes = argtypes
            fn.restype = C.c_longlong
        _lib = l
    return _lib


def last_error() -> str:
    return lib().lgn_last_error().decode()


def _check(rc: int, what: str):
    if rc != 0:
        raise RuntimeError(f"{what} failed (code {rc}): {last_error()}")


def stream_ptr() -> int:
    return torch.cuda.current_stream().cuda_stream


def ptr(t: Optional[torch.Tensor]):
    if t is None:
        return None
    if not t.is_cuda:
        raise RuntimeError("liblgn_amd.so operates on GPU tensors only (got a CPU tensor); there is no CPU fallback")
    if not t.is_contiguous():
        raise RuntimeError("non-contiguous tensor passed to the native library")
    return t.data_ptr()


def f64(t: torch.Tensor) -> torch.Tensor:
    if t.dtype != torch.float64:
        raise RuntimeError(f"the native path is fp64 (reference precision); got {t.dtype}")
    return t.contiguous()



def level_fwd(decoder, s_in, v_in, p, mask, rad, wm0, wm1):
    _, B, N, Cc = s_in.shape
    CO = wm0.shape[1]
    dev, dt = s_in.device, s_in.dtype
    ag0 = torch.empty(2, B, N, 2 * Cc, device=dev, dtype=dt)
    ag1 = torch.empty(2, B, N, 2 * Cc, 4, device=dev, dtype=dt)
    s_out = torch.empty(2, B, N, CO, device=dev, dtype=dt)
    v_out = torch.empty(2, B, N, CO, 4, device=dev, dtype=dt)
    a, b, c, w0, b0, w1, b1 = rad
    rc = lib().lgn_level_fwd_f64(B, N, Cc, CO, int(decoder), ptr(s_in), ptr(v_in), ptr(p), ptr(mask),
                                 ptr(a), ptr(b), ptr(c), ptr(w0), ptr(b0), ptr(w1), ptr(b1), ptr(wm0), ptr(wm1),
                                 ptr(ag0), ptr(ag1), ptr(s_out), ptr(v_out), stream_ptr())
    _check(rc, "lgn_level_fwd_f64")
    return ag0, ag1, s_out, v_out


def reduce_partials(part: torch.Tensor, out: torch.Tensor, accumulate: bool = False):
    rows, n = part.shape
    _check(lib().lgn_reduce_partials_f64(ptr(part), rows, n, ptr(out), int(accumulate), stream_ptr()),
           "lgn_reduce_partials_f64")
    return out


def level_bwd(decoder, s_in, v_in, p, mask, rad, wm0, wm1, ag0, ag1, g_s_out, g_v_out, g_p=None):
    _, B, N, Cc = s_in.shape
    CO = wm0.shape[1]
    dev, dt = s_in.device, s_in.dtype
    L = lib()
    rm, rr = C.c_int(), C.c_int()
    _check(L.lgn_level_bwd_partial_rows(B, N, int(decoder), C.byref(rm), C.byref(rr)), "lgn_level_bwd_partial_rows")
    nmix = 4 * CO * 5 * Cc
    nrad = L.lgn_level_rad_partial_len(Cc, int(decoder))
    part_mix = torch.empty(rm.value, nmix, device=dev, dtype=dt)
    part_rad = torch.empty(rr.value, nrad, device=dev, dtype=dt)
    g_ag = torch.empty(B, N, 20 * Cc, device=dev, dtype=dt)
    g_s_in = torch.empty_like(s_in)
    g_v_in = torch.empty_like(v_in)
    a, b, c, w0, b0, w1, b1 = rad
    rc = L.lgn_level_bwd_f64(B, N, Cc, CO, int(decoder), ptr(s_in), ptr(v_in), ptr(p), ptr(mask),
                             ptr(a), ptr(b), ptr(c), ptr(w0), ptr(b0), ptr(w1), ptr(b1), ptr(wm0), ptr(wm1),
                             ptr(ag0), ptr(ag1), ptr(g_s_out), ptr(g_v_out), ptr(g_ag), ptr(g_s_in), ptr(g_v_in),
                             ptr(g_p), ptr(part_mix), ptr(part_rad), stream_ptr())
    _check(rc, "lgn_level_bwd_f64")
    g_mix = torch.empty(nmix, device=dev, dtype=dt)
    reduce_partials(part_mix, g_mix)
    g_wm0 = g_mix[: nmix // 2].view(2, CO, 5 * Cc)
    g_wm1 = g_mix[nmix // 2:].view(2, CO, 5 * Cc)
    tot = torch.empty(nrad, device=dev, dtype=dt)
    reduce_partials(part_rad, tot)
    if decoder:
        rad_grads = (tot[:Cc], tot[Cc:])
    else:
        g_a, g_b, g_c = (torch.empty_like(x) for x in (a, b, c))
        g_w0, g_b0, g_w1, g_b1 = (torch.empty_like(x) for x in (w0, b0, w1, b1))
        _check(L.lgn_radial_finalize_f64(ptr(tot), Cc, ptr(a), ptr(b), ptr(c), ptr(w0), ptr(w1), ptr(g_a), ptr(g_b),
                                         ptr(g_c), ptr(g_w0), ptr(g_b0), ptr(g_w1), ptr(g_b1), stream_ptr()),
               "lgn_radial_finalize_f64")
        rad_grads = (g_a, g_b, g_c, g_w0, g_b0, g_w1, g_b1)
    return g_s_in, g_v_in, g_wm0, g_wm1, rad_grads


def _ptr_array(ts: Sequence[torch.Tensor]):
    arr = (C.c_void_p * len(ts))()
    for i, t in enumerate(ts):
        arr[i] = ptr(t)
    return arr


def cgmlp_fwd(s_in, ws, bs, act: int = 0):
    _, B, N, Cc = s_in.shape
    H = ws[0].shape[0]
    s_out = torch.empty_like(s_in)
# ... 137 lines not shown
```

Before: 1.064 million.

## Fuse encoder-decoder junction into the first separable decoder level kernel

After: 1.074 million, median of 6. Within noise of the previous version (+0.9%).

```diff
diff --git a/include/lgn_amd.h b/include/lgn_amd.h
--- a/include/lgn_amd.h
+++ b/include/lgn_amd.h
@@ -140,12 +140,14 @@
 #define LGN_NET_DEC_UNFUSED 256
 #define LGN_NET_MOMENTS_SPLIT 512
 #define LGN_NET_MLP_BWD1 1024
+#define LGN_NET_SPLIT_JUNCTION 2048
 #define LGN_NET_SPLIT_TAIL 128
 
 #define LGN_LDS_LIMIT (160 * 1024)
 long long lgn_encoder_end_lds_bytes(int N, int C0, int K, int CL, int Ts, int Tv, int pool);
 long long lgn_decoder_end_lds_bytes(int N, int C0, int Tin, int CL);
 long long lgn_junction_lds_bytes(int N, int CL, int Ts, int Tv, int pool, int C0);
+int lgn_step_fuses_junction(const lgn_net_desc* d);
 
 int lgn_step_param_slots(const lgn_net_desc* d, int decoder);
 long long lgn_step_workspace_doubles(const lgn_net_desc* d);
diff --git a/lgn-autoencoder_amd/csrc/api_common.cpp b/lgn-autoencoder_amd/csrc/api_common.cpp
--- a/lgn-autoencoder_amd/csrc/api_common.cpp
+++ b/lgn-autoencoder_amd/csrc/api_common.cpp
@@ -16,10 +16,11 @@
   auto on = [](const char* name) { const char* e = getenv(name); return e && e[0] == '1'; };
   return (on("LGN_AMD_DEC_PAIRWISE") ? LVL_DEC_PAIRWISE : 0) | (on("LGN_AMD_LEVEL_V2") ? LVL_LEVEL_V2 : 0) |
          (on("LGN_AMD_MOMENTS_V1") ? LVL_MOMENTS_V1 : 0) | (on("LGN_AMD_MLP_V1") ? LVL_MLP_V1 : 0) | (on("LGN_AMD_BWD_ORDERED") ? LVL_BWD_ORDERED : 0) |
-         (on("LGN_AMD_MOMENTS_SPLIT") ? LVL_MOMENTS_SPLIT : 0) | (on("LGN_AMD_MLP_BWD1") ? LVL_MLP_BWD1 : 0);
+         (on("LGN_AMD_MOMENTS_SPLIT") ? LVL_MOMENTS_SPLIT : 0) | (on("LGN_AMD_MLP_BWD1") ? LVL_MLP_BWD1 : 0) |
+         (on("LGN_AMD_SPLIT_JUNCTION") ? LVL_SPLIT_JUNCTION : 0);
 }
 static_assert(LVL_DEC_PAIRWISE == LGN_NET_DEC_PAIRWISE && LVL_LEVEL_V2 == LGN_NET_LEVEL_V2 && LVL_MOMENTS_V1 == LGN_NET_MOMENTS_V1 &&
-                  LVL_MLP_V1 == LGN_NET_MLP_V1 && LVL_MLP_BWD1 == LGN_NET_MLP_BWD1 &&
+                  LVL_MLP_V1 == LGN_NET_MLP_V1 && LVL_MLP_BWD1 == LGN_NET_MLP_BWD1 && LVL_SPLIT_JUNCTION == LGN_NET_SPLIT_JUNCTION &&
                   LVL_BWD_ORDERED == LGN_NET_BWD_ORDERED && LVL_MOMENTS_SPLIT == LGN_NET_MOMENTS_SPLIT, "LVL_* and LGN_NET_* are the same bits");
 }
 
diff --git a/lgn-autoencoder_amd/csrc/junction_dev.hpp b/lgn-autoencoder_amd/csrc/junction_dev.hpp
--- /dev/null
+++ b/lgn-autoencoder_amd/csrc/junction_dev.hpp
@@ -0,0 +1,290 @@
+#pragma once
+#include "net.hpp"
+#include "net_dev.hpp"
+
+#ifndef JSTAMP
+#define JSTAMP(i) STAMP(i)
+#endif
+
+namespace lgn {
+
+__device__ __forceinline__ void cart_from_canon(const cx<double> (&c)[4], cx<double> (&p)[4]) {
+  p[0] = c[0];
+  p[1] = {(c[1].r - c[3].r) * NET_RSQRT2, (c[1].i - c[3].i) * NET_RSQRT2};
+  p[2] = {-(c[1].i + c[3].i) * NET_RSQRT2, (c[1].r + c[3].r) * NET_RSQRT2};
+  p[3] = c[2];
+}
+
+__device__ __forceinline__ cx<double> canon_cplx_m(const double* p, int m) {
+  if (m == 0) return {p[0], p[4]};
+  if (m == 2) return {p[3], p[7]};
+  const double sg = m == 1 ? 1.0 : -1.0;
+  return {(sg * p[1] + p[6]) * NET_RSQRT2, (sg * p[5] - p[2]) * NET_RSQRT2};
+}
+__device__ __forceinline__ cx<double> canon_cplx_bwd_m(const double* g, int m) {
+  if (m == 0) return {g[0], g[4]};
+  if (m == 3) return {g[2], g[6]};
+  if (m == 1) return {(g[1] - g[3]) * NET_RSQRT2, (g[5] - g[7]) * NET_RSQRT2};
+  return {-(g[5] + g[7]) * NET_RSQRT2, (g[1] + g[3]) * NET_RSQRT2};
+}
+
+__host__ __device__ inline size_t lat_y_doubles(int N, int Ts, int Tv, int pool = 0) {
+  return (size_t)(pool_is_mix(pool) ? 1 : N) * (2 * Ts + 8 * Tv);
+}
+__host__ __device__ inline size_t lat_fwd_doubles(int N, int C, int Ts, int Tv, int pool = 0) {
+  return lat_y_doubles(N, Ts, Tv, pool) + (size_t)N * C * 10 + 2 * (size_t)(Ts + Tv) * pool_mix_in(pool, N, C);
+}
+struct LatentStage {
+  StageRegs<2> sr, si;
+  StageRegs<4> vr, vi;
+  StageRegs<1> w0, w1;
+  const double *s0, *s1, *v0, *v1, *wl0, *wl1;
+  int N, C, Ts, Tv, K, NY, NS;
+  __device__ __forceinline__ void issue(int B, int N_, int C_, int Ts_, int Tv_, const double* __restrict__ s, const double* __restrict__ v,
+                                        const double* __restrict__ wl0_, const double* __restrict__ wl1_, int pool = 0) {
+    N = N_; C = C_; Ts = Ts_; Tv = Tv_; wl0 = wl0_; wl1 = wl1_; K = pool_mix_in(pool, N_, C_); NY = (int)lat_y_doubles(N_, Ts_, Tv_, pool);
+    const size_t pl = (size_t)B * N * C, j0 = (size_t)blockIdx.x * N * C;
+    NS = s ? N * C : 0;
+    s0 = s ? s + j0 : nullptr; s1 = s ? s + pl + j0 : nullptr; v0 = v + j0 * 4; v1 = v + (pl + j0) * 4;
+    vr.issue(v0, N * C * 4); vi.issue(v1, N * C * 4);
+    sr.issue(s0, NS); si.issue(s1, NS);
+    w0.issue(wl0, 2 * Ts * K); w1.issue(wl1, 2 * Tv * K);
+  }
+  __device__ __forceinline__ void commit(double* lds, bool zero_y) const {
+    double* sv = lds + NY;
+    double* w0l = sv + N * C * 10;
+    double* w1l = w0l + 2 * Ts * K;
+    if (zero_y)
+      for (int e = threadIdx.x; e < NY; e += BLOCK) lds[e] = 0.0;
+    vr.commit(v0, N * C * 4, [&](int e, double x) { sv[(e >> 2) * 10 + 2 + (e & 3)] = x; });
+    vi.commit(v1, N * C * 4, [&](int e, double x) { sv[(e >> 2) * 10 + 6 + (e & 3)] = x; });
+    if (NS) {
+      sr.commit(s0, NS, [&](int e, double x) { sv[e * 10] = x; });
+      si.commit(s1, NS, [&](int e, double x) { sv[e * 10 + 1] = x; });
+    } else {
+      for (int e = threadIdx.x; e < N * C; e += BLOCK) sv[e * 10] = sv[e * 10 + 1] = 0.0;
+    }
+    w0.commit(wl0, 2 * Ts * K, [&](int e, double x) { w0l[e] = x; });
+    w1.commit(wl1, 2 * Tv * K, [&](int e, double x) { w1l[e] = x; });
+  }
+};
+template <bool TO_LDS>
+__device__ __forceinline__ void enc_latent_fwd_body(int B, int N, int C, int Ts, int Tv, int pool, double* lat_s, double* lat_v, int* idx,
+                                                    double* lds, double* lat_l) {
+  const int b = blockIdx.x, TT = Ts + Tv;
+  const int P = pool_blocks(pool), PN = pool_n(pool);
+  bool need_mean = false;
+  for (int i = 0; i < PN; ++i) need_mean |= pool_op(pool, i) == LGN_POOL_MEAN;
+  const int YS = 2 * Ts + 8 * Tv;
+  double* y = lds;
+  const double* sv = y + N * YS;
+  const double* w0l = sv + N * C * 10;
+  const double* w1l = w0l + 2 * Ts * C;
+  JSTAMP(1);
+  for (int e = threadIdx.x; e < N * Tv; e += BLOCK) {
+    const int n = e / Tv, tv = e - n * Tv;
+    const double* x = sv + n * C * 10;
+    cx<double> acc[4] = {{0, 0}, {0, 0}, {0, 0}, {0, 0}}, pc[4];
+#pragma unroll 4
+    for (int c = 0; c < C; ++c) {
+      const cx<double> w = {w1l[tv * C + c], w1l[Tv * C + tv * C + c]};
+#pragma unroll
+      for (int m = 0; m < 4; ++m) cfma(acc[m], w, cx<double>{x[c * 10 + 2 + m], x[c * 10 + 6 + m]});
+    }
+    cart_from_canon(acc, pc);
+    double* o = y + n * YS + 2 * Ts + 8 * tv;
+#pragma unroll
+    for (int m = 0; m < 4; ++m) { o[m] = pc[m].r; o[4 + m] = pc[m].i; }
+  }
+  for (int e = threadIdx.x; e < N * Ts; e += BLOCK) {
+    const int n = e / Ts, t = e - n * Ts;
+    const double* x = sv + n * C * 10;
+    cx<double> acc = {0, 0};
+#pragma unroll 4
+    for (int c = 0; c < C; ++c) cfma(acc, cx<double>{w0l[t * C + c], w0l[Ts * C + t * C + c]}, cx<double>{x[c * 10], x[c * 10 + 1]});
+    y[n * YS + 2 * t] = acc.r;
+    y[n * YS + 2 * t + 1] = acc.i;
+  }
+  __syncthreads();
+  JSTAMP(2);
+  const int l8 = threadIdx.x & 7;
+  constexpr int NONE = 0x7fffffff;
+  for (int it = threadIdx.x >> 3; it < 2 * TT; it += BLOCK / 8) {
+    const int z = it / TT, t = it - z * TT;
+    int imin = NONE, imax = NONE;
+    double smin = 0, smax = 0;
+#pragma unroll 4
+    for (int n = l8; n < N; n += 8) {
+      double lo, hi;
+      if (t < Ts) {
+        const double val = y[n * YS + 2 * t + z];
+        lo = val;
+        hi = val * val;
+      } else {
+        const double* o = y + n * YS + 2 * Ts + 8 * (t - Ts) + 4 * z;
+        lo = hi = o[0] * o[0] - ((o[1] * o[1] + o[2] * o[2]) + o[3] * o[3]);
+      }
+      if (imin == NONE || lo < smin) { smin = lo; imin = n; }
+      if (imax == NONE || hi > smax) { smax = hi; imax = n; }
+    }
+#pragma unroll
+    for (int off = 4; off; off >>= 1) {
+      const double om = __shfl_xor(smin, off, 8), oM = __shfl_xor(smax, off, 8);
+      const int oi = __shfl_xor(imin, off, 8), oI = __shfl_xor(imax, off, 8);
+      if (oi != NONE && (imin == NONE || om < smin || (om == smin && oi < imin))) { smin = om; imin = oi; }
+      if (oI != NONE && (imax == NONE || oM > smax || (oM == smax && oI < imax))) { smax = oM; imax = oI; }
+    }
+    imin = __shfl(imin, 0, 8);
+    imax = __shfl(imax, 0, 8);
+    if (l8 < 2) idx[(((size_t)b * 2 + z) * TT + t) * 2 + l8] = l8 ? imax : imin;
+    const int nc = t < Ts ? 1 : 4, y0 = t < Ts ? 2 * t + z : 2 * Ts + 8 * (t - Ts) + 4 * z;
+    double mean[4] = {0, 0, 0, 0};
+    if (need_mean) {
+      for (int n = l8; n < N; n += 8)
+#pragma unroll
+        for (int m = 0; m < 4; ++m)
+          if (m < nc) mean[m] += y[n * YS + y0 + m];
+#pragma unroll
+      for (int off = 4; off; off >>= 1)
+#pragma unroll
+        for (int m = 0; m < 4; ++m) mean[m] += __shfl_xor(mean[m], off, 8);
+#pragma unroll
+      for (int m = 0; m < 4; ++m) mean[m] /= (double)N;
+    }
+    for (int k = l8; k < P * nc; k += 8) {
+      const int pb = k / nc, m = k - pb * nc;
+      auto pick = [&](int op) -> double {
+        if (op == LGN_POOL_MIN) return y[imin * YS + y0 + m];
+        if (op == LGN_POOL_MAX) return y[imax * YS + y0 + m];
+        return m == 0 ? mean[0] : (m == 1 ? mean[1] : (m == 2 ? mean[2] : mean[3]));
+      };
+      double val;
+      if (pool_avg(pool)) {
+        val = pick(pool_op(pool, 0));
+        for (int i = 1; i < PN; ++i) val += pick(pool_op(pool, i));
+        val /= (double)PN;
+      } else {
+        val = pick(pool_op(pool, pb));
+      }
+      if (t < Ts) {
+        lat_s[((size_t)z * B + b) * P * Ts + pb * Ts + t] = val;
+      } else {
+        const int tv = t - Ts;
+        lat_v[(((size_t)z * B + b) * P * Tv + pb * Tv + tv) * 4 + m] = val;
+        if constexpr (TO_LDS) lat_l[(pb * Tv + tv) * 8 + 4 * z + m] = val;
+      }
+    }
+  }
+}
+template <bool TO_LDS>
+__device__ __forceinline__ void enc_latent_mix_fwd_body(int B, int N, int C, int Ts, int Tv, double* lat_s, double* lat_v, double* lds,
+                                                        double* lat_l) {
+  const int b = blockIdx.x, TT = Ts + Tv, K = N * C;
+  const double* sv = lds + (2 * Ts + 8 * Tv);
+  const double* w0l = sv + K * 10;
+  const double* w1l = w0l + 2 * Ts * K;
+  const int l8 = threadIdx.x & 7;
+  for (int t = threadIdx.x >> 3; t < TT; t += BLOCK / 8) {
+    if (t < Ts) {
+      cx<double> acc = {0, 0};
+      for (int k = l8; k < K; k += 8) cfma(acc, cx<double>{w0l[t * K + k], w0l[Ts * K + t * K + k]}, cx<double>{sv[k * 10], sv[k * 10 + 1]});
+#pragma unroll
+      for (int off = 4; off; off >>= 1) { acc.r += __shfl_xor(acc.r, off, 8); acc.i += __shfl_xor(acc.i, off, 8); }
+      if (l8 < 2) lat_s[((size_t)l8 * B + b) * Ts + t] = l8 ? acc.i : acc.r;
+    } else {
+      const int tv = t - Ts;
+      cx<double> acc[4] = {{0, 0}, {0, 0}, {0, 0}, {0, 0}}, pc[4];
+      for (int k = l8; k < K; k += 8) {
+        const cx<double> w = {w1l[tv * K + k], w1l[Tv * K + tv * K + k]};
+#pragma unroll
+        for (int m = 0; m < 4; ++m) cfma(acc[m], w, cx<double>{sv[k * 10 + 2 + m], sv[k * 10 + 6 + m]});
+      }
+#pragma unroll
+      for (int off = 4; off; off >>= 1)
+#pragma unroll
+        for (int m = 0; m < 4; ++m) { acc[m].r += __shfl_xor(acc[m].r, off, 8); acc[m].i += __shfl_xor(acc[m].i, off, 8); }
+      cart_from_canon(acc, pc);
+      const int z = l8 >> 2, m = l8 & 3;
+      const cx<double> pm = m == 0 ? pc[0] : (m == 1 ? pc[1] : (m == 2 ? pc[2] : pc[3]));
+      const double val = z ? pm.i : pm.r;
+      lat_v[(((size_t)z * B + b) * Tv + tv) * 4 + m] = val;
+      if constexpr (TO_LDS) lat_l[tv * 8 + 4 * z + m] = val;
+    }
+  }
+}
+
+__host__ __device__ inline size_t dec_in_fwd_doubles(int N, int C, int Tin) {
+  return 2 * (size_t)N * Tin + (size_t)Tin * 8 + (size_t)N * 8 + 4 * (size_t)C;
+}
+struct DecInFwdStage {
+  StageRegs<4> wg;
+  StageRegs<1> a0, a1, lr, li;
+  const double *wg1, *w0, *w1, *l0, *l1;
+  int N, C, Tin;
+  bool with_lat;
+  __device__ __forceinline__ void issue(int B, int N_, int C_, int Tin_, const double* __restrict__ lat_v, const double* __restrict__ wg1_,
+                                        const double* __restrict__ w0_, const double* __restrict__ w1_, bool with_lat_) {
+    N = N_; C = C_; Tin = Tin_; wg1 = wg1_; w0 = w0_; w1 = w1_; with_lat = with_lat_;
+    wg.issue(wg1, 2 * N * Tin);
+    a0.issue(w0, 2 * C); a1.issue(w1, 2 * C);
+    if (with_lat) {
+      l0 = lat_v + (size_t)blockIdx.x * Tin * 4; l1 = lat_v + ((size_t)B + blockIdx.x) * Tin * 4;
+      lr.issue(l0, Tin * 4); li.issue(l1, Tin * 4);
+    }
+  }
+  __device__ __forceinline__ void commit(double* lds) const {
+    double* wgl = lds;
+    double* latl = wgl + 2 * N * Tin;
+    double* w01 = latl + Tin * 8 + N * 8;
+    wg.commit(wg1, 2 * N * Tin, [&](int e, double x) { wgl[e] = x; });
+    a0.commit(w0, 2 * C, [&](int e, double x) { w01[e] = x; });
+    a1.commit(w1, 2 * C, [&](int e, double x) { w01[2 * C + e] = x; });
+    if (with_lat) {
+      lr.commit(l0, Tin * 4, [&](int e, double x) { latl[(e >> 2) * 8 + (e & 3)] = x; });
+      li.commit(l1, Tin * 4, [&](int e, double x) { latl[(e >> 2) * 8 + 4 + (e & 3)] = x; });
+    }
+  }
+};
+template <bool TILE = false>
+__device__ __forceinline__ void dec_input_fwd_body(int B, int N, int C, int Tin, double* pdec, double* s0, double* v0, double* lds,
+                                                   double* nd = nullptr, double* pj = nullptr, int ns = 0) {
+  const double* wgl = lds;
+  const double* latl = wgl + 2 * N * Tin;
+  double* cartl = const_cast<double*>(latl) + Tin * 8;
+  const double* w01 = cartl + N * 8;
+  const int b = blockIdx.x;
+  const size_t plp = (size_t)B * N * 4, pl = (size_t)B * N * C;
+  JSTAMP(3);
+  for (int e = threadIdx.x; e < N * 4; e += BLOCK) {
+    const int n = e >> 2, m = e & 3;
+    cx<double> acc = {0, 0};
+#pragma unroll 8
+    for (int t = 0; t < Tin; ++t)
+      cfma(acc, cx<double>{wgl[n * Tin + t], wgl[N * Tin + n * Tin + t]}, cx<double>{latl[t * 8 + m], latl[t * 8 + 4 + m]});
+    cartl[n * 8 + m] = acc.r;
+    cartl[n * 8 + 4 + m] = acc.i;
+  }
+  __syncthreads();
+  JSTAMP(4);
+  for (int e = threadIdx.x; e < N * 4; e += BLOCK) {
+    const cx<double> pc = canon_cplx_m(cartl + (e >> 2) * 8, e & 3);
+    pdec[(size_t)b * N * 4 + e] = pc.r;
+    pdec[plp + (size_t)b * N * 4 + e] = pc.i;
+    if constexpr (TILE) { pj[(e >> 2) * 8 + (e & 3)] = pc.r; pj[(e >> 2) * 8 + 4 + (e & 3)] = pc.i; }
+  }
+  for (int e = threadIdx.x; e < N * C; e += BLOCK) {
+    const int c = e % C;
+    s0[(size_t)b * N * C + e] = w01[c] - w01[C + c];
+    s0[pl + (size_t)b * N * C + e] = w01[C + c] + w01[c];
+    if constexpr (TILE) { nd[(e / C) * ns + c * 10] = w01[c] - w01[C + c]; nd[(e / C) * ns + c * 10 + 1] = w01[C + c] + w01[c]; }
+  }
+  for (int e = threadIdx.x; e < N * C * 4; e += BLOCK) {
+    const int i = e >> 2, m = e & 3, n = i / C, c = i - n * C;
+    const cx<double> r = cmul(cx<double>{w01[2 * C + c], w01[3 * C + c]}, canon_cplx_m(cartl + n * 8, m));
+    v0[(size_t)b * N * C * 4 + e] = r.r;
+    v0[pl * 4 + (size_t)b * N * C * 4 + e] = r.i;
+    if constexpr (TILE) { nd[n * ns + c * 10 + 2 + m] = r.r; nd[n * ns + c * 10 + 6 + m] = r.i; }
+  }
+}
+
+}
diff --git a/lgn-autoencoder_amd/csrc/level.hpp b/lgn-autoencoder_amd/csrc/level.hpp
--- a/lgn-autoencoder_amd/csrc/level.hpp
+++ b/lgn-autoencoder_amd/csrc/level.hpp
@@ -10,6 +10,7 @@
 constexpr int LVL_MLP_BWD1 = 1024;
 constexpr int LVL_MOMENTS_SPLIT = 512;
 constexpr int LVL_BWD_ORDERED = 64;
+constexpr int LVL_SPLIT_JUNCTION = 2048;
 int level_flags_from_env();
 
 template <typename T>
@@ -42,6 +43,20 @@
   T* loss_part = nullptr;
   T* loss_gv = nullptr;
   T* loss_wpart = nullptr;
+  const T* jct_s = nullptr;
+  const T* jct_v = nullptr;
+  const T* jct_wl0 = nullptr;
+  const T* jct_wl1 = nullptr;
+  const T* jct_wg1 = nullptr;
+  const T* jct_w0 = nullptr;
+  const T* jct_w1 = nullptr;
+  T* jct_lat_s = nullptr;
+  T* jct_lat_v = nullptr;
+  int* jct_idx = nullptr;
+  T* jct_pdec = nullptr;
+  T* jct_s0 = nullptr;
+  T* jct_v0 = nullptr;
+  int jct_CL = 0, jct_Ts = 0, jct_Tv = 0, jct_pool = 0;
   int flags = 0;
 };
 
diff --git a/lgn-autoencoder_amd/csrc/level_fwd2.hip b/lgn-autoencoder_amd/csrc/level_fwd2.hip
--- a/lgn-autoencoder_amd/csrc/level_fwd2.hip
+++ b/lgn-autoencoder_amd/csrc/level_fwd2.hip
@@ -1,5 +1,6 @@
 #include "level_dev.hpp"
-#include "net_dev.hpp"
+#define JSTAMP(i) STAMP(48 + (i))
+#include "junction_dev.hpp"
 #include "ops.hpp"
 #include "wave_sum.hpp"
 
@@ -43,8 +44,9 @@
   static constexpr int A3 = 0, A4 = 2 * C, A1 = 4 * C, A2 = 12 * C;
 };
 
-template <int C, bool DEC, bool SEP, bool TRAIN>
+template <int C, bool DEC, bool SEP, bool TRAIN, bool JCT = false>
 __global__ __launch_bounds__(2 * BLOCK) void level_fwd2_kernel(LevelArgs<double> a, int chunk) {
+  static_assert(!JCT || (DEC && SEP), "the junction rides on the separable decoder level");
   using F = Fwd2<C, DEC>;
   constexpr int NG = F::NG;
   const int N = a.N, B = a.B, CO = a.CO;
@@ -60,7 +62,33 @@
   uint8_t* mk = reinterpret_cast<uint8_t*>(sums + 20 * C);
 
   STAMP(0);
-  if (!DEC && a.in_w0) {
+  if constexpr (JCT) {
+    const int CL = a.jct_CL, Ts = a.jct_Ts, Tv = a.jct_Tv, pool = a.jct_pool, Tin = pool_blocks(pool) * Tv;
+    double* lat_lds = nd;
+    double* dec_lds = lat_lds + lat_fwd_doubles(N, CL, Ts, Tv, pool);
+    LatentStage ls;
+    DecInFwdStage ds;
+    ls.issue(B, N, CL, Ts, Tv, a.jct_s, a.jct_v, a.jct_wl0, a.jct_wl1, pool);
+    ds.issue(B, N, C, Tin, nullptr, a.jct_wg1, a.jct_w0, a.jct_w1, false);
+    const int nw2 = 2 * CO * 5 * C, ew = tid < nw2 ? tid : 0;
+    const double w0v = a.wm0[ew], w1v = a.wm1[ew];
+    ls.commit(lat_lds, false);
+    ds.commit(dec_lds);
+    __syncthreads();
+    double* lat_l = dec_lds + 2 * N * Tin;
+    if (pool_is_mix(pool)) enc_latent_mix_fwd_body<true>(B, N, CL, Ts, Tv, a.jct_lat_s, a.jct_lat_v, lat_lds, lat_l);
+    else enc_latent_fwd_body<true>(B, N, CL, Ts, Tv, pool, a.jct_lat_s, a.jct_lat_v, a.jct_idx, lat_lds, lat_l);
+    __syncthreads();
+    dec_input_fwd_body<true>(B, N, C, Tin, a.jct_pdec, a.jct_s0, a.jct_v0, dec_lds, nd, pj, F::NS);
+    if (tid < nw2) {
+      wm[tid] = w0v;
+      wm[nw2 + tid] = w1v;
+    }
+    for (int e = tid + nthr; e < nw2; e += nthr) {
+      wm[e] = a.wm0[e];
+      wm[nw2 + e] = a.wm1[e];
+    }
+  } else if (!DEC && a.in_w0) {
     {
       const size_t wg = (size_t)blockIdx.y * gridDim.x + blockIdx.x, stride = (size_t)gridDim.x * gridDim.y * nthr;
       for (size_t e = wg * nthr + tid; e < a.z1n; e += stride) a.z1[e] = 0.0;
@@ -514,7 +542,13 @@
   }
 }
 
-template <int C, bool DEC, bool SEP, bool TRAIN>
+static size_t junction_prologue_bytes(int N, int C, int CO, int CL, int Ts, int Tv, int pool) {
+  const size_t front = (((size_t)N * node_stride(C) + 1) & ~size_t(1)) + (size_t)N * 8 + 4 * (size_t)CO * 5 * C;
+  const size_t nl = lat_fwd_doubles(N, CL, Ts, Tv, pool), ndd = dec_in_fwd_doubles(N, C, pool_blocks(pool) * Tv);
+  return front <= nl ? sizeof(double) * (nl + ndd) : 0;
+}
+
+template <int C, bool DEC, bool SEP, bool TRAIN, bool JCT = false>
 static int launch_level_fwd2(const LevelArgs<double>& a, hipStream_t stream) {
   using F = Fwd2<C, DEC>;
   const size_t fixed = sizeof(double) * (((size_t)a.N * F::NS + 1 & ~size_t(1)) + (size_t)a.N * F::PS + 4 * a.CO * 5 * C + 20 * C) + a.N + 16;
@@ -534,8 +568,15 @@
                   "level_fwd: the loss rides on the separable decoder forward of jets of <= 40 particles only");
     if (smem < dec_out_loss_bytes(a.N, a.CO)) smem = dec_out_loss_bytes(a.N, a.CO);
   }
+  if constexpr (JCT) {
+    const size_t jb = junction_prologue_bytes(a.N, C, a.CO, a.jct_CL, a.jct_Ts, a.jct_Tv, a.jct_pool);
+    LGN_CHECK_ARG(a.N <= 40 && !wide && jb && a.jct_v && a.jct_wl0 && a.jct_wg1 && a.jct_w0 && a.jct_w1 && a.jct_lat_s && a.jct_lat_v &&
+                  a.jct_idx && a.jct_pdec && a.jct_s0 && a.jct_v0,
+                  "level_fwd: the junction rides on the separable decoder forward of jets of <= 40 particles only");
+    if (smem < jb) smem = jb;
+  }
   LGN_CHECK_ARG(smem <= 160 * 1024, "level_fwd: N=%d C=%d needs %zu B of LDS (> 160 KiB)", a.N, a.C, smem);
-  auto kern = level_fwd2_kernel<C, DEC, SEP, TRAIN>;
+  auto kern = level_fwd2_kernel<C, DEC, SEP, TRAIN, JCT>;
   if (smem > 64 * 1024) {
     hipError_t e = hipFuncSetAttribute(reinterpret_cast<const void*>(kern), hipFuncAttributeMaxDynamicSharedMemorySize, (int)smem);
     if (e != hipSuccess) { set_error("hipFuncSetAttribute: %s", hipGetErrorString(e)); return (int)e; }
@@ -548,6 +589,11 @@
 }
 
 bool level_fwd_carries_loss(int N, int flags) { return N <= 40 && !(flags & LVL_DEC_PAIRWISE); }
+bool level_fwd_carries_junction(int N, int C, int CO, int CL, int Ts, int Tv, int pool, int flags) {
+  if (N > 40 || (flags & (LVL_DEC_PAIRWISE | LVL_SPLIT_JUNCTION)) || !pool_valid(pool) || C < 1 || C > 8 || CO < 1 || CO > 8) return false;
+  const size_t jb = junction_prologue_bytes(N, C, CO, CL, Ts, Tv, pool_canon(pool));
+  return jb && jb <= 64 * 1024;
+}
 
 template <bool TRAIN>
 static int level_fwd_run(const LevelArgs<double>& a, int decoder, hipStream_t stream) {
@@ -555,9 +601,13 @@
   LGN_CHECK_ARG(!a.in_w0 || (!decoder && a.in_w1 && a.in_s && a.in_v), "level_fwd: the input stage rides on encoder levels only");
   LGN_CHECK_ARG(a.CO >= 1 && a.CO <= 8, "level_fwd: C_out=%d unsupported (1..8)", a.CO);
   const bool pairwise = (a.flags & LVL_DEC_PAIRWISE) != 0;
+  LGN_CHECK_ARG(!a.jct_wl1 || (decoder && !pairwise), "level_fwd: the junction rides on separable decoder levels only");
+  LevelArgs<double> aj = a;
+  aj.jct_pool = pool_canon(a.jct_pool);
 #define LGN_CASE(CC)                                                                                         \
   case CC:                                                                                                   \
     if (!decoder) return launch_level_fwd2<CC, false, false, TRAIN>(a, stream);                              \
+    if (a.jct_wl1) return launch_level_fwd2<CC, true, true, TRAIN, true>(aj, stream);                        \
     return pairwise ? launch_level_fwd2<CC, true, false, TRAIN>(a, stream) : launch_level_fwd2<CC, true, true, TRAIN>(a, stream);
   switch (a.C) {
 #ifdef LGN_DEV_ONLY_C4
diff --git a/lgn-autoencoder_amd/csrc/net_kernels.hip b/lgn-autoencoder_amd/csrc/net_kernels.hip
--- a/lgn-autoencoder_amd/csrc/net_kernels.hip
+++ b/lgn-autoencoder_amd/csrc/net_kernels.hip
@@ -1,5 +1,6 @@
 #include "net.hpp"
 #include "net_dev.hpp"
+#include "junction_dev.hpp"
 #include "tail_dev.hpp"
 
 namespace lgn {
@@ -31,12 +32,6 @@
   gp[1] = {(g[1].r - g[3].r) * H, (g[1].i - g[3].i) * H};
   gp[2] = {-(g[1].i + g[3].i) * H, (g[1].r + g[3].r) * H};
   gp[3] = g[2];
-}
-__device__ __forceinline__ void cart_from_canon(const cx<double> (&c)[4], cx<double> (&p)[4]) {
-  p[0] = c[0];
-  p[1] = {(c[1].r - c[3].r) * H, (c[1].i - c[3].i) * H};
-  p[2] = {-(c[1].i + c[3].i) * H, (c[1].r + c[3].r) * H};
-  p[3] = c[2];
 }
 }
 
@@ -118,203 +113,6 @@
   }
 }
 
-__device__ __forceinline__ cx<double> canon_cplx_m(const double* p, int m) {
-  if (m == 0) return {p[0], p[4]};
-  if (m == 2) return {p[3], p[7]};
-  const double sg = m == 1 ? 1.0 : -1.0;
-  return {(sg * p[1] + p[6]) * H, (sg * p[5] - p[2]) * H};
-}
-__device__ __forceinline__ cx<double> canon_cplx_bwd_m(const double* g, int m) {
-  if (m == 0) return {g[0], g[4]};
-  if (m == 3) return {g[2], g[6]};
-  if (m == 1) return {(g[1] - g[3]) * H, (g[5] - g[7]) * H};
-  return {-(g[5] + g[7]) * H, (g[1] + g[3]) * H};
-}
-
-__host__ __device__ inline size_t lat_y_doubles(int N, int Ts, int Tv, int pool = 0) {
-  return (size_t)(pool_is_mix(pool) ? 1 : N) * (2 * Ts + 8 * Tv);
-}
-__host__ __device__ inline size_t lat_fwd_doubles(int N, int C, int Ts, int Tv, int pool = 0) {
-  return lat_y_doubles(N, Ts, Tv, pool) + (size_t)N * C * 10 + 2 * (size_t)(Ts + Tv) * pool_mix_in(pool, N, C);
-}
-struct LatentStage {
-  StageRegs<2> sr, si;
-  StageRegs<4> vr, vi;
-  StageRegs<1> w0, w1;
-  const double *s0, *s1, *v0, *v1, *wl0, *wl1;
-  int N, C, Ts, Tv, K, NY, NS;
-  __device__ __forceinline__ void issue(int B, int N_, int C_, int Ts_, int Tv_, const double* __restrict__ s, const double* __restrict__ v,
-                                        const double* __restrict__ wl0_, const double* __restrict__ wl1_, int pool = 0) {
-    N = N_; C = C_; Ts = Ts_; Tv = Tv_; wl0 = wl0_; wl1 = wl1_; K = pool_mix_in(pool, N_, C_); NY = (int)lat_y_doubles(N_, Ts_, Tv_, pool);
-    const size_t pl = (size_t)B * N * C, j0 = (size_t)blockIdx.x * N * C;
-    NS = s ? N * C : 0;
-    s0 = s ? s + j0 : nullptr; s1 = s ? s + pl + j0 : nullptr; v0 = v + j0 * 4; v1 = v + (pl + j0) * 4;
-    vr.issue(v0, N * C * 4); vi.issue(v1, N * C * 4);
-    sr.issue(s0, NS); si.issue(s1, NS);
-    w0.issue(wl0, 2 * Ts * K); w1.issue(wl1, 2 * Tv * K);
-  }
-  __device__ __forceinline__ void commit(double* lds, bool zero_y) const {
-    double* sv = lds + NY;
-    double* w0l = sv + N * C * 10;
-    double* w1l = w0l + 2 * Ts * K;
-    if (zero_y)
-      for (int e = threadIdx.x; e < NY; e += BLOCK) lds[e] = 0.0;
-    vr.commit(v0, N * C * 4, [&](int e, double x) { sv[(e >> 2) * 10 + 2 + (e & 3)] = x; });
-    vi.commit(v1, N * C * 4, [&](int e, double x) { sv[(e >> 2) * 10 + 6 + (e & 3)] = x; });
-    if (NS) {
-      sr.commit(s0, NS, [&](int e, double x) { sv[e * 10] = x; });
-      si.commit(s1, NS, [&](int e, double x) { sv[e * 10 + 1] = x; });
-    } else {
-      for (int e = threadIdx.x; e < N * C; e += BLOCK) sv[e * 10] = sv[e * 10 + 1] = 0.0;
-    }
-    w0.commit(wl0, 2 * Ts * K, [&](int e, double x) { w0l[e] = x; });
-    w1.commit(wl1, 2 * Tv * K, [&](int e, double x) { w1l[e] = x; });
-  }
-};
-template <bool TO_LDS>
-__device__ __forceinline__ void enc_latent_fwd_body(int B, int N, int C, int Ts, int Tv, int pool, double* lat_s, double* lat_v, int* idx,
-                                                    double* lds, double* lat_l) {
-  const int b = blockIdx.x, TT = Ts + Tv;
-  const int P = pool_blocks(pool), PN = pool_n(pool);
-  bool need_mean = false;
-  for (int i = 0; i < PN; ++i) need_mean |= pool_op(pool, i) == LGN_POOL_MEAN;
-  const int YS = 2 * Ts + 8 * Tv;
-  double* y = lds;
-  const double* sv = y + N * YS;
-  const double* w0l = sv + N * C * 10;
-  const double* w1l = w0l + 2 * Ts * C;
-  STAMP(1);
-  for (int e = threadIdx.x; e < N * Tv; e += BLOCK) {
-    const int n = e / Tv, tv = e - n * Tv;
-    const double* x = sv + n * C * 10;
-    cx<double> acc[4] = {{0, 0}, {0, 0}, {0, 0}, {0, 0}}, pc[4];
-#pragma unroll 4
-    for (int c = 0; c < C; ++c) {
-      const cx<double> w = {w1l[tv * C + c], w1l[Tv * C + tv * C + c]};
-#pragma unroll
-      for (int m = 0; m < 4; ++m) cfma(acc[m], w, cx<double>{x[c * 10 + 2 + m], x[c * 10 + 6 + m]});
-    }
-    cart_from_canon(acc, pc);
-    double* o = y + n * YS + 2 * Ts + 8 * tv;
-#pragma unroll
-    for (int m = 0; m < 4; ++m) { o[m] = pc[m].r; o[4 + m] = pc[m].i; }
-  }
-  for (int e = threadIdx.x; e < N * Ts; e += BLOCK) {
-    const int n = e / Ts, t = e - n * Ts;
-    const double* x = sv + n * C * 10;
-    cx<double> acc = {0, 0};
-#pragma unroll 4
-    for (int c = 0; c < C; ++c) cfma(acc, cx<double>{w0l[t * C + c], w0l[Ts * C + t * C + c]}, cx<double>{x[c * 10], x[c * 10 + 1]});
-    y[n * YS + 2 * t] = acc.r;
-    y[n * YS + 2 * t + 1] = acc.i;
-  }
-  __syncthreads();
-  STAMP(2);
-  const int l8 = threadIdx.x & 7;
-  constexpr int NONE = 0x7fffffff;
-  for (int it = threadIdx.x >> 3; it < 2 * TT; it += BLOCK / 8) {
-    const int z = it / TT, t = it - z * TT;
-    int imin = NONE, imax = NONE;
-    double smin = 0, smax = 0;
-#pragma unroll 4
-    for (int n = l8; n < N; n += 8) {
-      double lo, hi;
-      if (t < Ts) {
-        const double val = y[n * YS + 2 * t + z];
-        lo = val;
-        hi = val * val;
-      } else {
-        const double* o = y + n * YS + 2 * Ts + 8 * (t - Ts) + 4 * z;
-        lo = hi = o[0] * o[0] - ((o[1] * o[1] + o[2] * o[2]) + o[3] * o[3]);
-      }
-      if (imin == NONE || lo < smin) { smin = lo; imin = n; }
-      if (imax == NONE || hi > smax) { smax = hi; imax = n; }
-    }
-#pragma unroll
-    for (int off = 4; off; off >>= 1) {
-      const double om = __shfl_xor(smin, off, 8), oM = __shfl_xor(smax, off, 8);
-      const int oi = __shfl_xor(imin, off, 8), oI = __shfl_xor(imax, off, 8);
-      if (oi != NONE && (imin == NONE || om < smin || (om == smin && oi < imin))) { smin = om; imin = oi; }
-      if (oI != NONE && (imax == NONE || oM > smax || (oM == smax && oI < imax))) { smax = oM; imax = oI; }
-    }
-    imin = __shfl(imin, 0, 8);
-    imax = __shfl(imax, 0, 8);
-    if (l8 < 2) idx[(((size_t)b * 2 + z) * TT + t) * 2 + l8] = l8 ? imax : imin;
-    const int nc = t < Ts ? 1 : 4, y0 = t < Ts ? 2 * t + z : 2 * Ts + 8 * (t - Ts) + 4 * z;
-    double mean[4] = {0, 0, 0, 0};
-    if (need_mean) {
-      for (int n = l8; n < N; n += 8)
-#pragma unroll
-        for (int m = 0; m < 4; ++m)
-          if (m < nc) mean[m] += y[n * YS + y0 + m];
-#pragma unroll
-      for (int off = 4; off; off >>= 1)
-#pragma unroll
-        for (int m = 0; m < 4; ++m) mean[m] += __shfl_xor(mean[m], off, 8);
-#pragma unroll
-      for (int m = 0; m < 4; ++m) mean[m] /= (double)N;
-    }
-    for (int k = l8; k < P * nc; k += 8) {
-      const int pb = k / nc, m = k - pb * nc;
-      auto pick = [&](int op) -> double {
-        if (op == LGN_POOL_MIN) return y[imin * YS + y0 + m];
-        if (op == LGN_POOL_MAX) return y[imax * YS + y0 + m];
-        return m == 0 ? mean[0] : (m == 1 ? mean[1] : (m == 2 ? mean[2] : mean[3]));
-      };
-      double val;
-      if (pool_avg(pool)) {
-        val = pick(pool_op(pool, 0));
-        for (int i = 1; i < PN; ++i) val += pick(pool_op(pool, i));
-        val /= (double)PN;
-      } else {
-        val = pick(pool_op(pool, pb));
-      }
-      if (t < Ts) {
-        lat_s[((size_t)z * B + b) * P * Ts + pb * Ts + t] = val;
-      } else {
-        const int tv = t - Ts;
-        lat_v[(((size_t)z * B + b) * P * Tv + pb * Tv + tv) * 4 + m] = val;
-        if constexpr (TO_LDS) lat_l[(pb * Tv + tv) * 8 + 4 * z + m] = val;
-      }
-    }
-  }
-}
-template <bool TO_LDS>
-__device__ __forceinline__ void enc_latent_mix_fwd_body(int B, int N, int C, int Ts, int Tv, double* lat_s, double* lat_v, double* lds,
-                                                        double* lat_l) {
-  const int b = blockIdx.x, TT = Ts + Tv, K = N * C;
-  const double* sv = lds + (2 * Ts + 8 * Tv);
-  const double* w0l = sv + K * 10;
-  const double* w1l = w0l + 2 * Ts * K;
-  const int l8 = threadIdx.x & 7;
-  for (int t = threadIdx.x >> 3; t < TT; t += BLOCK / 8) {
-    if (t < Ts) {
-      cx<double> acc = {0, 0};
-      for (int k = l8; k < K; k += 8) cfma(acc, cx<double>{w0l[t * K + k], w0l[Ts * K + t * K + k]}, cx<double>{sv[k * 10], sv[k * 10 + 1]});
-#pragma unroll
-      for (int off = 4; off; off >>= 1) { acc.r += __shfl_xor(acc.r, off, 8); acc.i += __shfl_xor(acc.i, off, 8); }
-      if (l8 < 2) lat_s[((size_t)l8 * B + b) * Ts + t] = l8 ? acc.i : acc.r;
-    } else {
-      const int tv = t - Ts;
-      cx<double> acc[4] = {{0, 0}, {0, 0}, {0, 0}, {0, 0}}, pc[4];
-      for (int k = l8; k < K; k += 8) {
-        const cx<double> w = {w1l[tv * K + k], w1l[Tv * K + tv * K + k]};
-#pragma unroll
-        for (int m = 0; m < 4; ++m) cfma(acc[m], w, cx<double>{sv[k * 10 + 2 + m], sv[k * 10 + 6 + m]});
-      }
-#pragma unroll
-      for (int off = 4; off; off >>= 1)
-#pragma unroll
-        for (int m = 0; m < 4; ++m) { acc[m].r += __shfl_xor(acc[m].r, off, 8); acc[m].i += __shfl_xor(acc[m].i, off, 8); }
-      cart_from_canon(acc, pc);
-      const int z = l8 >> 2, m = l8 & 3;
-      const cx<double> pm = m == 0 ? pc[0] : (m == 1 ? pc[1] : (m == 2 ? pc[2] : pc[3]));
-      const double val = z ? pm.i : pm.r;
-      lat_v[(((size_t)z * B + b) * Tv + tv) * 4 + m] = val;
-      if constexpr (TO_LDS) lat_l[tv * 8 + 4 * z + m] = val;
-    }
-  }
-}
 __global__ __launch_bounds__(BLOCK) void enc_latent_fwd_kernel(int B, int N, int C, int Ts, int Tv, int pool,
                                                               const double* __restrict__ s, const double* __restrict__ v,
                                                               const double* __restrict__ wl0, const double* __restrict__ wl1,
@@ -550,74 +348,6 @@
   else enc_latent_bwd_body<false>(B, N, C, Ts, Tv, pool, g_lat_s, g_lat_v, nullptr, idx, g_s, g_v, part, lds, pre);
 }
 
-__host__ __device__ inline size_t dec_in_fwd_doubles(int N, int C, int Tin) {
-  return 2 * (size_t)N * Tin + (size_t)Tin * 8 + (size_t)N * 8 + 4 * (size_t)C;
-}
-struct DecInFwdStage {
-  StageRegs<4> wg;
-  StageRegs<1> a0, a1, lr, li;
-  const double *wg1, *w0, *w1, *l0, *l1;
-  int N, C, Tin;
-  bool with_lat;
-  __device__ __forceinline__ void issue(int B, int N_, int C_, int Tin_, const double* __restrict__ lat_v, const double* __restrict__ wg1_,
-                                        const double* __restrict__ w0_, const double* __restrict__ w1_, bool with_lat_) {
-    N = N_; C = C_; Tin = Tin_; wg1 = wg1_; w0 = w0_; w1 = w1_; with_lat = with_lat_;
-    wg.issue(wg1, 2 * N * Tin);
-    a0.issue(w0, 2 * C); a1.issue(w1, 2 * C);
-    if (with_lat) {
-      l0 = lat_v + (size_t)blockIdx.x * Tin * 4; l1 = lat_v + ((size_t)B + blockIdx.x) * Tin * 4;
-      lr.issue(l0, Tin * 4); li.issue(l1, Tin * 4);
-    }
-  }
-  __device__ __forceinline__ void commit(double* lds) const {
-    double* wgl = lds;
-    double* latl = wgl + 2 * N * Tin;
-    double* w01 = latl + Tin * 8 + N * 8;
-    wg.commit(wg1, 2 * N * Tin, [&](int e, double x) { wgl[e] = x; });
-    a0.commit(w0, 2 * C, [&](int e, double x) { w01[e] = x; });
-    a1.commit(w1, 2 * C, [&](int e, double x) { w01[2 * C + e] = x; });
-    if (with_lat) {
-      lr.commit(l0, Tin * 4, [&](int e, double x) { latl[(e >> 2) * 8 + (e & 3)] = x; });
-      li.commit(l1, Tin * 4, [&](int e, double x) { latl[(e >> 2) * 8 + 4 + (e & 3)] = x; });
-    }
-  }
-};
-__device__ __forceinline__ void dec_input_fwd_body(int B, int N, int C, int Tin, double* pdec, double* s0, double* v0, double* lds) {
-  const double* wgl = lds;
-  const double* latl = wgl + 2 * N * Tin;
-  double* cartl = const_cast<double*>(latl) + Tin * 8;
-  const double* w01 = cartl + N * 8;
-  const int b = blockIdx.x;
-  const size_t plp = (size_t)B * N * 4, pl = (size_t)B * N * C;
-  STAMP(3);
-  for (int e = threadIdx.x; e < N * 4; e += BLOCK) {
-    const int n = e >> 2, m = e & 3;
-    cx<double> acc = {0, 0};
-#pragma unroll 8
-    for (int t = 0; t < Tin; ++t)
-      cfma(acc, cx<double>{wgl[n * Tin + t], wgl[N * Tin + n * Tin + t]}, cx<double>{latl[t * 8 + m], latl[t * 8 + 4 + m]});
-    cartl[n * 8 + m] = acc.r;
-    cartl[n * 8 + 4 + m] = acc.i;
-  }
-  __syncthreads();
-  STAMP(4);
-  for (int e = threadIdx.x; e < N * 4; e += BLOCK) {
-    const cx<double> pc = canon_cplx_m(cartl + (e >> 2) * 8, e & 3);
-    pdec[(size_t)b * N * 4 + e] = pc.r;
-    pdec[plp + (size_t)b * N * 4 + e] = pc.i;
-  }
-  for (int e = threadIdx.x; e < N * C; e += BLOCK) {
-    const int c = e % C;
-    s0[(size_t)b * N * C + e] = w01[c] - w01[C + c];
-    s0[pl + (size_t)b * N * C + e] = w01[C + c] + w01[c];
-  }
-  for (int e = threadIdx.x; e < N * C * 4; e += BLOCK) {
-    const int i = e >> 2, m = e & 3, n = i / C, c = i - n * C;
-    const cx<double> r = cmul(cx<double>{w01[2 * C + c], w01[3 * C + c]}, canon_cplx_m(cartl + n * 8, m));
-    v0[(size_t)b * N * C * 4 + e] = r.r;
-    v0[pl * 4 + (size_t)b * N * C * 4 + e] = r.i;
-  }
-}
 __global__ __launch_bounds__(BLOCK) void dec_input_fwd_kernel(int B, int N, int C, int Tin, const double* __restrict__ lat_v,
                                                              const double* __restrict__ wg1, const double* __restrict__ w0,
                                                              const double* __restrict__ w1, double* pdec, double* s0, double* v0) {
diff --git a/lgn-autoencoder_amd/csrc/ops.hpp b/lgn-autoencoder_amd/csrc/ops.hpp
--- a/lgn-autoencoder_amd/csrc/ops.hpp
+++ b/lgn-autoencoder_amd/csrc/ops.hpp
@@ -44,6 +44,7 @@
 void level_bwd_partial_rows(int B, int N, int decoder, int flags, int* rows_mix, int* rows_rad);
 bool level_bwd_carries_input(int N, int flags);
 bool level_fwd_carries_loss(int N, int flags);
+bool level_fwd_carries_junction(int N, int C, int CO, int CL, int Ts, int Tv, int pool, int flags);
 
 constexpr int MLP_MAX_LIN = 8;
 template <typename T>
diff --git a/lgn-autoencoder_amd/csrc/step.hip b/lgn-autoencoder_amd/csrc/step.hip
--- a/lgn-autoencoder_amd/csrc/step.hip
+++ b/lgn-autoencoder_amd/csrc/step.hip
@@ -238,6 +238,15 @@
   double *recon, *loss_part, *g_v, *wpart;
 };
 
+struct JunctionStage {
+  int CL, Ts, Tv, pool;
+  const double *s, *v, *wl0, *wl1;
+  double *lat_s, *lat_v;
+  int* idx;
+  const double *wg1, *w0, *w1;
+  double* pdec;
+};
+
 MlpArgs<double> level_mlp_args(const lgn_net_desc& d, bool dec, int l, const double* P, const int64_t* off) {
   const Slots S{d.n_levels, d.mlp_nlin};
   const int CO = (dec ? d.dec_channels : d.enc_channels)[l + 1];
@@ -249,7 +258,7 @@
 
 int levels_fwd(const lgn_net_desc& d, bool dec, const int* ch, const double* P, const int64_t* off, NetBuf& n, const double* pos,
                const uint8_t* mask, hipStream_t st, const InputStage* in0 = nullptr, const LossStage* loss = nullptr, bool eval = false,
-               bool last_scalars = true) {
+               bool last_scalars = true, const JunctionStage* jct = nullptr) {
   const Slots S{d.n_levels, d.mlp_nlin};
   for (int l = 0; l < d.n_levels; ++l) {
     auto p = [&](int slot) { return P + off[slot]; };
@@ -260,6 +269,13 @@
     if (l == 0 && !dec && in0) {
       a.in_w0 = in0->w0; a.in_w1 = in0->w1; a.in_s = n.s[0]; a.in_v = n.v[0];
       a.z1 = in0->z1; a.z1n = in0->z1n; a.z2 = in0->z2; a.z2n = in0->z2n;
+    }
+    if (l == 0 && dec && jct) {
+      a.jct_CL = jct->CL; a.jct_Ts = jct->Ts; a.jct_Tv = jct->Tv; a.jct_pool = jct->pool;
+      a.jct_s = jct->s; a.jct_v = jct->v; a.jct_wl0 = jct->wl0; a.jct_wl1 = jct->wl1;
+      a.jct_lat_s = jct->lat_s; a.jct_lat_v = jct->lat_v; a.jct_idx = jct->idx;
+      a.jct_wg1 = jct->wg1; a.jct_w0 = jct->w0; a.jct_w1 = jct->w1;
+      a.jct_pdec = jct->pdec; a.jct_s0 = n.s[0]; a.jct_v0 = n.v[0];
     }
     if (l + 1 == d.n_levels && dec && loss) {
       a.loss_wo1 = loss->wo1; a.loss_target = loss->target; a.loss_scale = loss->scale; a.loss_real = loss->method;
@@ -408,6 +424,11 @@
 namespace {
 
 inline bool is_generic(const lgn_net_desc& d, bool dec) { return (dec ? d.dec_tables[0] : d.enc_tables[0]) != nullptr; }
+inline bool step_fuses_junction(const lgn_net_desc& d) {
+  if (is_generic(d, false) || is_generic(d, true) || step_is_split(d)) return false;
+  return level_fwd_carries_junction(d.N, d.dec_channels[0], d.dec_channels[1], d.enc_channels[d.n_levels], d.tau_s, d.tau_v,
+                                    d.latent_pool, d.flags);
+}
 
 struct GenGeom {
   const int *ch, *Q, *qs, *qv;
@@ -1144,6 +1165,10 @@
 long long lgn_junction_lds_bytes(int N, int CL, int Ts, int Tv, int pool, int C0) {
   return pool_valid(pool) ? (long long)junction_lds_bytes(N, CL, Ts, Tv, pool, C0) : -1;
 }
+int lgn_step_fuses_junction(const lgn_net_desc* d) {
+  if (check_desc(d) || check_latent_match(*d)) return -1;
+  return step_fuses_junction(*d) ? 1 : 0;
+}
 
 long long lgn_step_workspace_doubles(const lgn_net_desc* d) {
   if (check_desc(d) || check_latent_match(*d)) return -1;
@@ -1191,6 +1216,9 @@
   dq.cap = w.parts_size;
   RadFinJob fin{};
 
+  const bool fuse_jct = step_fuses_junction(d);
+  const JunctionStage jct{ce[L], Ts, Tv, d.latent_pool, nullptr, w.enc.v[L], wl0, wl1, w.lat_s, w.lat_v, w.idx,
+                          params + dec_off[1], params + dec_off[2], params + dec_off[3], w.pdec};
   if (split) {
     LGN_TRY(zero_ranges(grads, (size_t)n_params, w.zero0(), w.zero_doubles, nullptr, 0, st));
     LGN_TRY(enc_input_fwd(B, Ne, ce[0], K, p4, in_scalars, params + enc_off[0], params + enc_off[1], w.enc.s[0], w.enc.v[0], st));
@@ -1201,8 +1229,9 @@
   } else {
     const InputStage in0{params + enc_off[0], params + enc_off[1], grads, (size_t)n_params, w.zeros_s, w.zero_doubles};
     LGN_TRY(levels_fwd(d, false, ce, params, enc_off, w.enc, p4, mask, st, &in0, nullptr, false, false));
-    LGN_TRY(junction_fwd(B, Ne, ce[L], Ts, Tv, d.latent_pool, nullptr, w.enc.v[L], wl0, wl1, w.lat_s, w.lat_v, w.idx, cd[0],
-                         params + dec_off[1], params + dec_off[2], params + dec_off[3], w.pdec, w.dec.s[0], w.dec.v[0], st));
+    if (!fuse_jct)
+      LGN_TRY(junction_fwd(B, Ne, ce[L], Ts, Tv, d.latent_pool, nullptr, w.enc.v[L], wl0, wl1, w.lat_s, w.lat_v, w.idx, cd[0],
+                           params + dec_off[1], params + dec_off[2], params + dec_off[3], w.pdec, w.dec.s[0], w.dec.v[0], st));
   }
   int cur = 0;
   {
@@ -1211,7 +1240,7 @@
     const LossStage ls{params + dec_off[S.out0(true) + 1], target, 1.0, d.get_real, d.jet_loss_scale, recon, loss_part, w.gv[cur], part};
     const bool rides = level_fwd_carries_loss(Nd, d.flags);
     LGN_TRY(levels_fwd(dd, true, cd, params, dec_off, w.dec, w.pdec, nullptr, st, nullptr, rides ? &ls : nullptr, false,
-                       false));
+                       false, fuse_jct ? &jct : nullptr));
     if (!rides)
       LGN_TRY(dec_output_loss(B, Nd, cd[L], w.dec.v[L], ls.wo1, target, 1.0, ls.method, ls.jscale, recon, loss_part, w.gv[cur], part, st));
     ro.add(dq, part, B, grads, dec_off);
@@ -1398,6 +1427,9 @@
   const bool rides = level_fwd_carries_loss(Nd, d.flags);
   const bool keep_s = lat_s_out != nullptr;
   const double* sL = keep_s ? w.enc.s[L] : nullptr;
+  const bool fuse_jct = step_fuses_junction(d);
+  const JunctionStage jct{ce[L], Ts, Tv, d.latent_pool, sL, w.enc.v[L], wl0, wl1, ls, lv, w.idx,
+                          params + dec_off[1], params + dec_off[2], params + dec_off[3], w.pdec};
   if (step_is_split(d)) {
     LGN_TRY(enc_input_fwd(B, Ne, ce[0], in_K(d), p4, in_scalars, params + enc_off[0], params + enc_off[1], w.enc.s[0], w.enc.v[0], st));
     LGN_TRY(levels_fwd(d, false, ce, params, enc_off, w.enc, p4, mask, st, nullptr, nullptr, true, keep_s));
@@ -1407,10 +1439,12 @@
   } else {
     const InputStage in0{params + enc_off[0], params + enc_off[1]};
     LGN_TRY(levels_fwd(d, false, ce, params, enc_off, w.enc, p4, mask, st, &in0, nullptr, true, keep_s));
-    LGN_TRY(junction_fwd(B, Ne, ce[L], Ts, Tv, d.latent_pool, sL, w.enc.v[L], wl0, wl1, ls, lv, w.idx, cd[0],
-                         params + dec_off[1], params + dec_off[2], params + dec_off[3], w.pdec, w.dec.s[0], w.dec.v[0], st));
-  }
-  LGN_TRY(levels_fwd(dd, true, cd, params, dec_off, w.dec, w.pdec, nullptr, st, nullptr, rides ? &loss : nullptr, true));
+    if (!fuse_jct)
+      LGN_TRY(junction_fwd(B, Ne, ce[L], Ts, Tv, d.latent_pool, sL, w.enc.v[L], wl0, wl1, ls, lv, w.idx, cd[0],
+                           params + dec_off[1], params + dec_off[2], params + dec_off[3], w.pdec, w.dec.s[0], w.dec.v[0], st));
+  }
+  LGN_TRY(levels_fwd(dd, true, cd, params, dec_off, w.dec, w.pdec, nullptr, st, nullptr, rides ? &loss : nullptr, true,
+                     true, fuse_jct ? &jct : nullptr));
   if (!rides) LGN_TRY(dec_output_eval(B, Nd, cd[L], w.dec.v[L], wo1, target, d.get_real, d.jet_loss_scale, recon_real, loss_part, st));
   return eval_loss_sum(B, Ne, mask, loss_part, loss_out, st);
 }
diff --git a/lgn-autoencoder_amd/lgn/_native.py b/lgn-autoencoder_amd/lgn/_native.py
--- a/lgn-autoencoder_amd/lgn/_native.py
+++ b/lgn-autoencoder_amd/lgn/_native.py
@@ -107,7 +107,7 @@
 NET_NO_STATIC = 1
 _NET_FLAG_ENV = {"LGN_AMD_NO_STATIC": 1, "LGN_AMD_DEC_PAIRWISE": 2, "LGN_AMD_LEVEL_V2": 4, "LGN_AMD_MLP_V1": 8,
                  "LGN_AMD_MOMENTS_V1": 16, "LGN_AMD_BWD_ORDERED": 64, "LGN_AMD_SPLIT_TAIL": 128, "LGN_AMD_DEC_UNFUSED": 256, "LGN_AMD_MOMENTS_SPLIT": 512,
-                 "LGN_AMD_MLP_BWD1": 1024}
+                 "LGN_AMD_MLP_BWD1": 1024, "LGN_AMD_SPLIT_JUNCTION": 2048}
 ACTIVATIONS = {"leakyrelu": 0, "relu": 1, "elu": 2, "sigmoid": 3, "logsigmoid": 4, "atan": 5}
 
 
@@ -134,6 +134,7 @@
     "lgn_local_bwd_static_f64": [_i] * 4 + [_vp] * 3 + [_ip] + [_vp] * 8,
     "lgn_local_bwd_f64": [_i] * 5 + [_tp] + [_vp] * 8,
     "lgn_step_param_slots": [_dp, _i],
+    "lgn_step_fuses_junction": [_dp],
     "lgn_step_fwd_bwd_f64": [_dp, _vp, _vp, _ll, _vp, _vp, _vp, _vp, _vp, _vp, _vp, _ll, _vp, _vp, _vp],
     "lgn_encoder_fwd_f64": [_dp, _vp, _vp, _vp, _vp, _vp, _vp, _ll, _vp, _vp, _vp],
     "lgn_encoder_bwd_f64": [_dp, _vp, _vp, _ll, _vp, _vp, _vp, _vp, _vp, _ll, _vp, _vp, _vp, _ll, _vp],
```
